# wolfecameron/GIST

Hardware: AMD Instinct MI355X
Metric: epochs/sec (higher is better)
Workload: dtype f32 (projection products from 3 bf16 pieces per operand = all 24 bits, 6 cross terms, fp32 accumulation)

## Files before the change

### gist_amd/_lib.py

```python
import ctypes
import os

_HERE = os.path.dirname(os.path.abspath(__file__))
LIB_PATH = os.environ.get('GIST_LIB_PATH') or os.path.join(_HERE, 'libgist_hip.so')

ABI_VERSION = 16


class GistLibraryError(RuntimeError):
    pass


class GistError(RuntimeError):
    """A gist_* entry point returned a negative code."""


_p = ctypes.c_void_p
_i64 = ctypes.c_int64
_i32 = ctypes.c_int32
_int = ctypes.c_int
_f = ctypes.c_float
_u64 = ctypes.c_uint64

SIGNATURES = {
    'gist_last_error': (ctypes.c_char_p, []),
    'gist_abi_version': (_int, []),
    'gist_device_count': (_int, []),
    'gist_in_degree_norm_f32': (_int, [_p, _i64, _p, _p]),
    'gist_spmm_csr_f32': (_int, [_p, _p, _p, _i64, _p, _i64, _i64, _i64, _p, _p, _int, _p]),
    'gist_partition_last_stats': (_int, [_p, _i32]),
    'gist_partition_graph': (_int, [_p, _p, _p, _p, _i64, _i32, _u64, _i32, _f, _p]),
    'gist_spmm_csr_blocked_f32': (_int, [_p, _p, _p, _i64, _p, _i64, _i64, _i64, _p, _p, _int, _p, _i64, _p]),
    'gist_spmm_blocks_bytes': (_i64, [_i64]),
    'gist_spmm_blocks_prepare': (_int, [_p, _p, _i64, _p, _i64, _p, _i64, _p]),
    'gist_spmm_csr_prepared_f32': (_int, [_p, _p, _p, _i64, _p, _i64, _i64, _i64, _p, _p, _int, _p, _i64, _p, _p]),
    'gist_gemm_workspace_bytes': (_i64, [_i64, _i64, _i64]),
    'gist_gemm_set_mode': (_int, [_int]),
    'gist_gemm_get_mode': (_int, []),
    'gist_tuning_set': (_int, [_int, ctypes.c_double]),
    'gist_tuning_get': (ctypes.c_double, [_int]),
    'gist_launch_count': (ctypes.c_uint64, []),
    'gist_empty_launches': (_int, [ctypes.c_int32, ctypes.c_int32, ctypes.c_int32, _p]),
    'gist_gemm_nt_f32': (_int, [_p, _i64, _p, _i64, _p, _p, _i64, _i64, _i64, _i64, _p, _i64, _p]),
    'gist_gemm_nn_f32': (_int, [_p, _i64, _p, _i64, _p, _i64, _i64, _i64, _i64, _p, _i64, _p]),
    'gist_gemm_tn_f32': (_int, [_p, _i64, _p, _i64, _p, _i64, _i64, _i64, _i64, _p, _i64, _p]),
    'gist_ln_relu_fwd_f32': (_int, [_p, _i64, _p, _i64, _p, _i64, _i64, _int, _int, _f, _p]),
    'gist_ln_relu_bwd_f32': (_int, [_p, _i64, _p, _i64, _p, _p, _i64, _i64, _i64, _int, _int, _p]),
    'gist_gemm_nn_dropout_f32': (_int, [_p, _i64, _p, _i64, _p, _i64, _i64, _i64, _i64, _f, _u64, _u64, _p, _i64, _p]),
    'gist_dropout_f32': (_int, [_p, _i64, _i64, _i64, _f, _u64, _u64, _p]),
    'gist_colsum_partials': (_i64, [_i64]),
    'gist_colsum_f32': (_int, [_p, _i64, _i64, _i64, _p, _p, _p]),
    'gist_softmax_xent_f32': (_int, [_p, _i64, _p, _p, _i64, _p, _p, _p, _i64, _i64, _i64, _p]),
    'gist_adam_f32': (_int, [_p, _p, _p, _p, _i64, _f, _f, _f, _f, _f, _i64, _p]),
    'gist_argmax_correct_i32': (_int, [_p, _i64, _p, _p, _p, _i64, _i64, _p]),
    'gist_induced_mark': (_int, [_p, _i64, _p, _p]),
    'gist_induced_unmark': (_int, [_p, _i64, _p, _p]),
    'gist_fill_i32': (_int, [_p, _i64, _i32, _p]),
    'gist_copy_i32': (_int, [_p, _p, _i64, _p]),
    'gist_publish_i64': (_int, [_p, _i64, _p, _p]),
    'gist_induced_rowptr': (_int, [_p, _p, _p, _i64, _p, _p, _p]),
    'gist_induced_fill': (_int, [_p, _p, _p, _i64, _p, _p, _p, _i64, _p]),
    'gist_extract_batch': (_int, [_p, _p, _p, _p, _p, _i64, _p, _p, _p, _p, _p, _i64, _p, _p, _i64, _i64, _p, _i64, _p, _p, _p]),
    'gist_gather_rows_f32': (_int, [_p, _i64, _p, _i64, _i64, _p, _i64, _p]),
    'gist_gather_i32': (_int, [_p, _p, _i64, _p, _p]),
    'gist_block_gather_f32': (_int, [_p, _i64, _p, _p, _i64, _i64, _p, _i64, _p]),
    'gist_block_scatter_f32': (_int, [_p, _i64, _p, _p, _i64, _i64, _p, _i64, _p]),
    'gist_mean_rows_f32': (_int, [_p, _i64, _i64, _i64, _p, _p]),
    'gist_standard_scaler_workspace_bytes': (_i64, [_i64, _i64]),
    'gist_standard_scaler_f32': (_int, [_p, _i64, _i64, _i64, _p, _i64, _p, _p, _p, _i64, _p]),
    'gist_timer_create': (_p, [_i64]),
    'gist_timer_destroy': (None, [_p]),
    'gist_timer_reset': (None, [_p]),
    'gist_timer_count': (_i64, [_p]),
    'gist_timer_read': (_int, [_p, _i64, _p, _p, _p, _p, _p]),
    'gist_step_h3_workspace_bytes': (_i64, [_p]),
    'gist_step_h3_workspace_bytes_mode': (_i64, [_p, _int]),
    'gist_step_fused_workspace_bytes': (_i64, [_p]),
    'gist_step_col_partials_floats': (_i64, [_p]),
    'gist_step_fused_slab_bytes': (_i64, [_p, _i32]),
    'gist_spmm_csr_drop_f32': (_int, [_p, _p, _p, _i64, _p, _i64, _i64, _i64, _p, _p, _int, _p, _i64, _int, _f,
                                      _u64, _u64, _u64, _i64, _p]),
    'gist_spmm_csr_drop_prepared_f32': (_int, [_p, _p, _p, _i64, _p, _i64, _i64, _i64, _p, _p, _int, _p, _i64, _int, _f,
                                               _u64, _u64, _u64, _i64, _p, _p]),
    'gist_spmm_csr_drop_lnbwd_f32': (_int, [_p, _p, _p, _i64, _p, _i64, _i64, _i64, _p, _p, _i64, _f, _u64, _u64, _u64, _i64,
                                            _p, _i64, _p, _p, _i64, _p, _i64, _int, _p]),
    'gist_spmm_lnb_units': (_i64, [_i64]),
    'gist_spmm_block_image_bytes': (_i64, []),
    'gist_spmm_pair_min_edges': (ctypes.c_int32, []),
    'gist_spmm_block_units_f32': (_int, [_p, _i64, _p, _p, _i64, _p, _i64, _i64, _i64, _p, _int, _p]),
    'gist_spmm_block_chains_f32': (_int, [_p, _i64, _p, _p, _p, _i64, _p, _i64, _i64, _i64, _p, _int, _p]),
    'gist_spmm_prepared_useful': (_int, [_i64, _i64, _i64, _p, _p]),
    'gist_spmm_drop_takes': (_int, [_int, _i64, _i64, _i64, _p, _p, _int]),
    'gist_gemm_dual_takes': (_int, [_i64, _i64, _i64, _i64, _i64, _i64, _i64, _p, _p, _p, _p]),
    'gist_gemm_nn_tn_dual_f32': (_int, [_p, _i64, _p, _i64, _p, _i64, _p, _i64, _p, _i64, _i64, _i64, _i64, _p, _i64, _p, _p]),
    'gist_gemm_slabs_f32': (_int, [_int, _p, _i64, _p, _i64, _p, _p, _i64, _i64, _i64, _i64, _p, _i64, _p, _p]),
    'gist_ln_relu_fwd_drop_f32': (_int, [_p, _i64, _p, _i64, _p, _i64, _p, _i64, _i64, _int, _int, _f, _f, _u64,
                                         _u64, _i64, _p]),
    'gist_ln_relu_fwd_slabs_f32': (_int, [_p, _i64, _p, _i64, _int, _p, _p, _i64, _p, _i64, _p, _i64, _i64, _int, _int,
                                          _f, _f, _u64, _u64, _i64, _p]),
    'gist_gemm_splits_operands': (_int, [_i64, _i64, _i64]),
    'gist_row_chunks16': (_i64, [_i64]),
    'gist_ln_relu_bwd_colsum_f32': (_int, [_p, _i64, _p, _i64, _p, _p, _i64, _i64, _i64, _int, _int, _p, _p]),
    'gist_colsum_chunks_f32': (_int, [_p, _i64, _i64, _p, _p]),
    'gist_class_layer_takes': (_int, [_i64, _i64, _i64, _i64, _i64, _p, _p]),
    'gist_class_layer_f32': (_int, [_p, _i64, _p, _i64, _p, _p, _i64, _p, _i64, _p, _i64, _p, _p, _i64, _f, _u64, _u64,
                                    _p, _i64, _i64, _i64, _p]),
    'gist_class_dw_slab_bytes': (_i64, [_i64, _i64, _i64]),
    'gist_class_dw_slabs_f32': (_int, [_p, _i64, _p, _i64, _p, _i64, _p, _i64, _i64, _i64, _p]),
    'gist_ln_relu_bwd_colsum_class_dw_f32': (_int, [_p, _i64, _p, _i64, _p, _p, _i64, _i64, _i64, _int, _int, _p,
                                                    _p, _i64, _p, _i64, _p, _i64, _p, _i64, _i64, _i64, _p]),
    'gist_gemm_nn_dropout_colsum_f32': (_int, [_p, _i64, _p, _i64, _p, _i64, _i64, _i64, _i64, _f, _u64, _u64,
                                               _p, _i64, _p, _p]),
    'gist_softmax_xent_slabs_f32': (_int, [_p, _i64, _p, _i64, _i64, _p, _p, _p, _i64, _p, _p, _p, _i64, _i64,
                                           _i64, _p]),
    'gist_adam_segments_f32': (_int, [_p, _p, _p, _p, _i64, _f, _f, _f, _f, _f, _i64, _p, _i64, _p, _i64, _i64,
                                      _p, _p]),
    'gist_grad_segments_finish_f32': (_int, [_p, _i64, _p, _i64, _p]),
    'gist_extract_batch_drop': (_int, [_p, _p, _p, _p, _p, _i64, _p, _p, _p, _p, _p, _i64, _p, _p, _i64, _i64, _p,
                                       _i64, _p, _p, _p, _i64, _f, _u64, _u64, _i64, _p]),
    'gist_extract_parts_scratch_bytes': (_i64, [_i64]),
    'gist_extract_parts_supported': (_int, [_i64]),
    'gist_extract_parts_batch': (_int, [_p, _p, _p, _p, _p, _i64, _i64, _p, _p, _i32, _p, _p, _p, _p, _i64,
                                        _p, _p, _i64, _i64, _p, _i64, _p, _p, _p, _i64, _f, _u64, _u64, _i64, _p,
                                        _p]),
    'gist_sage_step': (_int, [_p, _p, _i64, _u64, _f, _f, _f, _f, _f, _i64, _int, _p]),
    'gist_sage_step_extracts_next': (_int, [_p, _i64, _int]),
    'gist_extract_parts_desc_batch': (_int, [_p, _p]),
    'gist_adam_segments_extract_f32': (_int, [_p, _p, _p, _p, _i64, _f, _f, _f, _f, _f, _i64, _p, _i64, _p, _i64, _i64,
                                              _p, _p, _p]),
    'gist_gat_scores_f32': (_int, [_p, _i64, _p, _i64, _i64, _i64, _p, _p, _p]),
    'gist_gat_aggregate_f32': (_int, [_p, _p, _p, _i64, _p, _p, _i64, _i64, _i64, _int, _p, _i64, _p, _p, _p]),
    'gist_gat_backward_dst_f32': (_int, [_p, _p, _p, _i64, _p, _i64, _p, _i64, _p, _p, _p, _p, _i64, _i64, _i64, _int,
                                         _p, _i64, _p, _p, _p]),
    'gist_gat_backward_src_f32': (_int, [_p, _p, _p, _i64, _p, _i64, _p, _p, _p, _p, _p, _p, _p, _i64, _i64, _i64,
                                         _p, _i64, _p, _p]),
    'gist_gat_attn_grad_workspace_floats': (_i64, [_i64, _i64, _i64]),
    'gist_gat_attn_grad_f32': (_int, [_p, _i64, _p, _p, _i64, _i64, _i64, _p, _i64, _p, _p]),
}

GIST_MAX_LAYERS = 16
TUNE = {'h3_min_gflop': 0, 'h3_min_tiles': 1, 'h3_tm': 2, 'gemm_tile': 3, 'gemm_splits': 4,
        'spmm_chunk': 5, 'spmm_split': 6, 'spmm_kernel': 7, 'b3c': 8, 'class_fused': 9, 'gemm_dual': 10, 'host_threads': 11, 'lnb_fused': 12, 'b3c_splits': 13, 'b3_tail': 14,
        'b3_wide': 15}
GIST_STEP_EXTRACT = 1
GIST_STEP_TRAIN = 2
GIST_STEP_EXTRACT_NEXT = 4
GIST_STEP_PREEXTRACTED = 8
GIST_STEP_PHASE_FORWARD = 16
GIST_STEP_PHASE_BACKWARD = 32
GIST_STEP_PHASE_OPTIMIZER = 64
GIST_STEP_DLOGITS_GIVEN = 128


class LayerDesc(ctypes.Structure):
    _fields_ = [('n_in', _i64), ('n_out', _i64), ('W', _p), ('b', _p), ('dW', _p), ('db', _p),
                ('Z', _p), ('ldz', _i64), ('Y', _p), ('ldy', _i64), ('rstd', _p)]


class StepPlan(ctypes.Structure):
    _fields_ = [('n_layers', _i32), ('use_layernorm', _i32), ('p_drop', _f), ('seed', _u64),
                ('layer', LayerDesc * GIST_MAX_LAYERS),
                ('dlogits', _p), ('ldc', _i64), ('dZ', _p), ('partials', _p),
                ('row_loss', _p), ('loss', _p), ('workspace', _p), ('workspace_bytes', _i64),
                ('workspace2', _p), ('workspace2_bytes', _i64),
                ('params', _p), ('grads', _p), ('exp_avg', _p), ('exp_avg_sq', _p),
                ('n_params', _i64),
                ('g_rowptr', _p), ('g_col', _p), ('g_t_rowptr', _p), ('g_t_col', _p),
                ('feat', _p), ('ld_feat', _i64), ('labels_all', _p), ('remap', _p),
                ('rowptr', _p), ('col', _p), ('t_rowptr', _p), ('t_col', _p),
                ('col_capacity', _i64), ('norm', _p), ('labels', _p), ('timer', _p),
                ('n_max', _i64), ('feat_absmax', _f), ('h3_workspace', _p),
                ('h3_workspace_bytes', _i64), ('row_blocks', _p), ('n_row_blocks', _i64),
                ('spmm_prepared', _p), ('spmm_prepared_bytes', _i64),
                ('fuse', _i32), ('hsrc', _p * GIST_MAX_LAYERS), ('ld_hsrc', _i64 * GIST_MAX_LAYERS),
                ('col_partials', _p), ('fused_workspace', _p), ('fused_workspace_bytes', _i64),
                ('node_part', _p), ('part_slot', _p),
                ('batch_index', _i32), ('extract_scratch', _p),
                ('next_ids', _p), ('next_n', _i64), ('next_batch_index', _i32), ('next_drop_offset', _u64),
                ('feat_intra', _p), ('ld_feat_intra', _i64), ('sibling_parts', ctypes.c_int32)]


class ExtractPartsDesc(ctypes.Structure):
    _fields_ = [('g_rowptr', _p), ('g_col', _p), ('g_t_rowptr', _p), ('g_t_col', _p),
                ('ids', _p), ('n', _i64), ('n_max', _i64),
                ('node_part', _p), ('part_slot', _p), ('batch', _i32),
                ('rowptr', _p), ('col', _p), ('t_rowptr', _p), ('t_col', _p), ('col_capacity', _i64), ('norm', _p),
                ('feat', _p), ('ld_feat', _i64), ('n_feat', _i64), ('z0', _p), ('ldz0', _i64),
                ('labels_all', _p), ('labels', _p),
                ('x0', _p), ('ldx0', _i64), ('p', _f), ('seed', _u64), ('offset', _u64), ('mask_ld', _i64),
                ('scratch', _p), ('feat_intra', _p), ('ld_intra', _i64), ('ah', _p)]


class GradSegment(ctypes.Structure):
    _fields_ = [('begin', _i64), ('end', _i64), ('src', _p), ('stride', _i64), ('n_src', _i32)]


_lib = None


def load():
    global _lib
    if _lib is not None:
        return _lib
    if not os.path.exists(LIB_PATH):
        raise GistLibraryError(
            'gist_amd: %s is missing. Build it with `python gist_amd/build.py` '
            '(hipcc --offload-arch=gfx950). There is no CPU fallback.' % LIB_PATH)
    import torch
    try:
        lib = ctypes.CDLL(LIB_PATH)
    except OSError as e:
        raise GistLibraryError('gist_amd: cannot load %s: %s' % (LIB_PATH, e))
    for name, (res, args) in SIGNATURES.items():
        try:
            fn = getattr(lib, name)
        except AttributeError:
            raise GistLibraryError('gist_amd: %s does not export %s (stale build?)'
                                   % (LIB_PATH, name))
        fn.restype = res
        fn.argtypes = args
    if lib.gist_abi_version() != ABI_VERSION:
        raise GistLibraryError('gist_amd: ABI version mismatch: library %d, binding %d'
                               % (lib.gist_abi_version(), ABI_VERSION))
    _lib = lib
    return lib


def check(rc, name):
    if rc != 0:
        msg = load().gist_last_error()
        raise GistError('%s failed (%d): %s' % (name, rc, msg.decode() if msg else ''))
```

### gist_amd/csrc/adam_body.h

```cpp
#pragma once
#include "common.h"

namespace gist {

constexpr int kAdamMaxSegs = 2 * GIST_MAX_LAYERS;
struct AdamSegs {
    int n;
    int n_src[kAdamMaxSegs];
    int ded_first[kAdamMaxSegs];
    int n_ded;
    int fin_first[kAdamMaxSegs];
    int n_fin;
    int64_t begin[kAdamMaxSegs], end[kAdamMaxSegs], stride[kAdamMaxSegs];
    const float *src[kAdamMaxSegs];
};
struct AdamArgs {
    float *p, *g, *m, *v;
    int64_t n;
    float beta1, beta2, eps, wd, step_size, inv_bc2_sqrt;
    AdamSegs segs;
    const float *row_nll; int n_loss_rows; float inv_count; float *loss;
};
__host__ __device__ inline int64_t adam_arena_blocks(int64_t n) { return (n + 1023) / 1024; }

__device__ __forceinline__ float adam_wave_sum(float v) {
#pragma unroll
    for (int off = 32; off > 0; off >>= 1) v += __shfl_xor(v, off);
    return v;
}

__device__ __forceinline__ void loss_reduce_256(const float *__restrict__ row_nll, int n_rows,
                                                float inv_count, float *__restrict__ loss, float *red) {
    float s = 0.f;
    if (threadIdx.x < 256)
        for (int i = threadIdx.x; i < n_rows; i += 256) s += row_nll[i];
    s = adam_wave_sum(s);
    if (threadIdx.x < 256 && (threadIdx.x & 63) == 0) red[threadIdx.x >> 6] = s;
    __syncthreads();
    if (threadIdx.x == 0) loss[0] = (((red[0] + red[1]) + red[2]) + red[3]) * inv_count;
}

__device__ __forceinline__ float chunk_partial4(const float *__restrict__ src, int64_t stride, int n_src, int q) {
    float acc = 0.f;
    int k = q;
    for (; k + 28 < n_src; k += 32) {
        float t[8];
#pragma unroll
        for (int u = 0; u < 8; ++u) t[u] = src[(int64_t)(k + 4 * u) * stride];
#pragma unroll
        for (int u = 0; u < 8; ++u) acc += t[u];
    }
    for (; k < n_src; k += 4) acc += src[(int64_t)k * stride];
    return acc;
}

__device__ __forceinline__ void adam_update(float *__restrict__ p, float *__restrict__ m, float *__restrict__ v,
                                            int64_t i, float gv, float beta1, float beta2, float eps, float wd,
                                            float step_size, float inv_bc2_sqrt) {
    const float pv = p[i];
    if (wd != 0.f) gv = fmaf(wd, pv, gv);
    const float mv = m[i] + (1.f - beta1) * (gv - m[i]);
    const float vv = beta2 * v[i] + (1.f - beta2) * gv * gv;
    m[i] = mv;
    v[i] = vv;
    const float denom = sqrtf(vv) * inv_bc2_sqrt + eps;
    p[i] = pv - step_size * (mv / denom);
}

template <bool kUpdate = true>
__device__ __forceinline__ void adam_virtual_block(const AdamArgs &A, int64_t vb, int vt, int only_seg = -1) {
    const AdamSegs &segs = A.segs;
    const int64_t n_chunks = adam_arena_blocks(A.n);
    if (vb >= n_chunks) {
        const int idx = (int)(vb - n_chunks);
        if (idx >= segs.n_ded) return;
        int sg = -1;
        for (int s = 0; s < segs.n; ++s)
            if (segs.ded_first[s] >= 0 && segs.ded_first[s] <= idx &&
                (sg < 0 || segs.ded_first[s] > segs.ded_first[sg]))
                sg = s;
        if (sg < 0) return;
        const int lane = vt & 63, w = vt >> 6;
        const int e = 16 * w + (lane & 15), q = lane >> 4;
        const int64_t i = segs.begin[sg] + (int64_t)(idx - segs.ded_first[sg]) * 64 + e;
        const bool live = i < segs.end[sg];
        float acc = 0.f;
        if (live) acc = chunk_partial4(segs.src[sg] + (i - segs.begin[sg]), segs.stride[sg], segs.n_src[sg], q);
        const float a1 = __shfl(acc, (lane & 15) + 16), a2 = __shfl(acc, (lane & 15) + 32), a3 = __shfl(acc, (lane & 15) + 48);
        if (q == 0 && live) {
            const float gv = ((acc + a1) + a2) + a3;
            A.g[i] = gv;
            if (kUpdate) adam_update(A.p, A.m, A.v, i, gv, A.beta1, A.beta2, A.eps, A.wd, A.step_size, A.inv_bc2_sqrt);
        }
        return;
    }
    const int64_t lo = vb * 1024;
    const int64_t hi = lo + 1024 < A.n ? lo + 1024 : A.n;
    unsigned touch = 0;
    for (int s = 0; s < segs.n; ++s)
        if (segs.begin[s] < hi && segs.end[s] > lo && (only_seg < 0 || s == only_seg)) touch |= 1u << s;
#pragma unroll
    for (int u = 0; u < 4; ++u) {
        const int64_t i = lo + vt + 256 * u;
        if (i >= hi) break;
        float gv;
        int sg = -1;
        for (unsigned t = touch; t; t &= t - 1) {
            const int s = __builtin_ctz(t);
            if (i >= segs.begin[s] && i < segs.end[s]) sg = s;
        }
        if (sg >= 0) {
            if (segs.ded_first[sg] >= 0) continue;
            const float *src = segs.src[sg] + (i - segs.begin[sg]);
            const int64_t stride = segs.stride[sg];
            const int ns = segs.n_src[sg];
            float acc = 0.f;
            int k = 0;
            for (; k + 4 <= ns; k += 4) {
                const float t0 = src[(int64_t)k * stride], t1 = src[(int64_t)(k + 1) * stride];
                const float t2 = src[(int64_t)(k + 2) * stride], t3 = src[(int64_t)(k + 3) * stride];
                acc += t0; acc += t1; acc += t2; acc += t3;
            }
            for (; k < ns; ++k) acc += src[(int64_t)k * stride];
            gv = acc;
            A.g[i] = acc;
        } else {
            if (!kUpdate) continue;
            gv = A.g[i];
        }
        if (kUpdate) adam_update(A.p, A.m, A.v, i, gv, A.beta1, A.beta2, A.eps, A.wd, A.step_size, A.inv_bc2_sqrt);
    }
}

int adam_segments_args(const char *name, float *param, float *grad, float *exp_avg, float *exp_avg_sq, int64_t n, float lr,
                       float beta1, float beta2, float eps, float weight_decay, int64_t step,
                       const gist_grad_segment *segments, int64_t n_segments, const float *row_loss,
                       int64_t n_loss_rows, int64_t loss_count, float *loss, AdamArgs *out);

}
```

### gist_amd/csrc/common.h

```cpp
#pragma once
#include <hip/hip_runtime.h>
#include <stdint.h>
#include <stdio.h>
#include <stdlib.h>

#include <atomic>

#include "../../include/gist_hip.h"

namespace gist {

constexpr int kWave = 64;

void set_error(const char *fmt, ...);

static inline hipStream_t as_stream(gist_stream_t s) { return reinterpret_cast<hipStream_t>(s); }

extern std::atomic<uint64_t> g_launches;

static inline int launch_status(const char *what) {
    g_launches.fetch_add(1, std::memory_order_relaxed);
    hipError_t e = hipGetLastError();
    if (e != hipSuccess) {
        set_error("%s: %s", what, hipGetErrorString(e));
        return GIST_ELAUNCH;
    }
    return GIST_OK;
}

#define GIST_REQUIRE(cond, ...)            \
    do {                                   \
        if (!(cond)) {                     \
            gist::set_error(__VA_ARGS__);  \
            return GIST_EINVAL;            \
        }                                  \
    } while (0)

extern thread_local gist_timer *tl_timer;
int64_t timer_begin(gist_timer *t, int kind, int64_t m, int64_t n, int64_t k, hipStream_t s);
void timer_end(gist_timer *t, int64_t slot, hipStream_t s);

__device__ __forceinline__ uint64_t splitmix64(uint64_t z) {
    z = (z ^ (z >> 30)) * 0xBF58476D1CE4E5B9ULL;
    z = (z ^ (z >> 27)) * 0x94D049BB133111EBULL;
    return z ^ (z >> 31);
}

int64_t h3_kpad(int64_t k);
bool h3_eligible(int64_t m, int64_t n, int64_t k);
bool h3_eligible_kept(int64_t m, int64_t n, int64_t k);
struct H3Dual {
    const float *src; int64_t ld; int64_t rows, cols;
    float p; uint64_t seed, offset;
    int fixed_shift;
    const unsigned *amax;
    const float *rowmax, *colmax;
    uint32_t *dst_r; float *inv_r;
    uint32_t *dst_t; float *inv_t;
};
int h3_dual_split(const H3Dual &d, hipStream_t st);
int h3_split_rows(const float *src, int64_t ld, int64_t rows, int64_t k, uint32_t *dst, float *inv,
                  hipStream_t st);
int h3_absmax(const float *src, int64_t ld, int64_t rows, int64_t cols, unsigned *out, hipStream_t st);
int h3_gemm_presplit(const char *name, const uint32_t *sa, const float *inv_a, const uint32_t *sb,
                     const float *inv_b, const float *bias, float *c, int64_t ldc, int64_t m,
                     int64_t n, int64_t k, hipStream_t st);

int h3_mode();
int64_t b3_kpad(int64_t k);
bool b3_eligible(int64_t m, int64_t n, int64_t k);
bool b3_eligible_kept(int64_t m, int64_t n, int64_t k);
struct B3Dual {
    const float *src; int64_t ld; int64_t rows, cols;
    float p; uint64_t seed, offset;
    uint16_t *dst_r;
    uint16_t *dst_t;
    float *col_partials;
    bool vec4;
};
int b3_dual_split(const B3Dual &d, hipStream_t st);
int64_t b3_slab_bytes(int64_t m, int64_t n, int64_t k);
int b3_gemm_presplit(const char *name, const uint16_t *sa, const uint16_t *sb, const float *bias, float *c,
                     int64_t ldc, int64_t m, int64_t n, int64_t k, float *slabs, int64_t slab_bytes,
                     hipStream_t st, int *deferred = nullptr);
int gemm_slabs(int layout, const float *a, int64_t lda, const float *b, int64_t ldb, const float *bias, float *c,
               int64_t ldc, int64_t m, int64_t n, int64_t k, void *slabs, int64_t slab_bytes, int *n_slabs,
               hipStream_t st);
int64_t gemm_f32_slab_bytes(int64_t m, int64_t n, int64_t k, bool tn = false);
bool gemm_dual_takes(int64_t m, int64_t n1, int64_t k1, int64_t lddy, int64_t ldw, int64_t ldz, int64_t lddz,
                     const float *dy, const float *w, const float *z, const float *dz);
int gemm_dual_nn_tn(const char *name, const float *dy, int64_t lddy, const float *w, int64_t ldw, float *dz,
                    int64_t lddz, const float *z, int64_t ldz, float *dw, int64_t lddw, int64_t m, int64_t n1,
                    int64_t k1, void *slabs, int64_t slab_bytes, int *n_slabs, hipStream_t st);
int splitk_reduce(const char *name, const float *slabs, int64_t slab, int splits, const float *bias, float *c,
                  int64_t ldc, int64_t m, int64_t n, hipStream_t st);

struct SpmmDrop {
    int mode;
    float p, scale;
    uint64_t sm, y_base, src_base;
    int64_t ld;
};
struct SpmmLnBwd {
    const float *yhat; int64_t ldy;
    const float *rstd;
    float *dy; int64_t lddy;
    float *col_partials;
    int relu;
};
int spmm_drop(const int32_t *rowptr, const int32_t *col, const float *x, int64_t ldx, float *y, int64_t ldy,
              int64_t n_rows, int64_t d, const float *out_scale, const float *src_scale, int accumulate,
              const int32_t *row_blocks, int64_t n_row_blocks, const SpmmDrop &dr, hipStream_t st,
              const void *prepared = nullptr, bool pairs = true, const SpmmLnBwd *ln = nullptr);
int spmm_prepared(const int32_t *rowptr, const int32_t *col, const float *x, int64_t ldx, float *y, int64_t ldy,
                  int64_t n_rows, int64_t d, const float *out_scale, const float *src_scale, int accumulate,
                  const int32_t *row_blocks, int64_t n_row_blocks, const void *prepared, hipStream_t st, bool pairs);
bool spmm_lnb_takes(int64_t d, int64_t ldx, int64_t ldy, const float *x, const float *y, const int32_t *row_blocks,
                    const void *prepared);
int64_t spmm_lnb_units(int64_t n_row_blocks);
bool spmm_drop_takes(int mode, int64_t d, int64_t ldx, int64_t ldy, const float *x, const float *y,
                     const int32_t *row_blocks);
#ifdef __HIPCC__
template <int CTRL>
__device__ __forceinline__ float dpp_move(float v) {
    return __builtin_bit_cast(float, __builtin_amdgcn_update_dpp(0, __builtin_bit_cast(int, v), CTRL, 0xf, 0xf, true));
}
__device__ __forceinline__ float wave_sum(float v) {
    v += dpp_move<0xB1>(v);
    v += dpp_move<0x4E>(v);
    v += dpp_move<0x141>(v);
    v += dpp_move<0x140>(v);
    const float r0 = __builtin_bit_cast(float, __builtin_amdgcn_readlane(__builtin_bit_cast(int, v), 0));
    const float r1 = __builtin_bit_cast(float, __builtin_amdgcn_readlane(__builtin_bit_cast(int, v), 16));
    const float r2 = __builtin_bit_cast(float, __builtin_amdgcn_readlane(__builtin_bit_cast(int, v), 32));
    const float r3 = __builtin_bit_cast(float, __builtin_amdgcn_readlane(__builtin_bit_cast(int, v), 48));
    return (r0 + r1) + (r2 + r3);
}
__device__ __forceinline__ float drop_keep(uint64_t idx, uint64_t sm, float p, float scale) {
    const uint64_t h = splitmix64((idx >> 1) + sm);
    const uint32_t w = (idx & 1) ? (uint32_t)(h >> 32) : (uint32_t)h;
    return ((float)(w >> 8) * (1.0f / 16777216.0f) >= p) ? scale : 0.f;
}
template <int VEC>
__device__ __forceinline__ void drop_vec(float (&v)[VEC], uint64_t idx0, const SpmmDrop &dr) {
#pragma unroll
    for (int k = 0; k < VEC; ++k) v[k] *= drop_keep(idx0 + k, dr.sm, dr.p, dr.scale);
}
__device__ __forceinline__ void drop_f4(float4 &v, uint64_t idx0, const SpmmDrop &dr) {
    const float inv = 1.0f / 16777216.0f;
    if ((idx0 & 1) == 0) {
        const uint64_t pair = idx0 >> 1;
        const uint64_t h0 = splitmix64(pair + dr.sm), h1 = splitmix64(pair + 1 + dr.sm);
        v.x *= ((float)((uint32_t)h0 >> 8) * inv >= dr.p) ? dr.scale : 0.f;
        v.y *= ((float)((uint32_t)(h0 >> 32) >> 8) * inv >= dr.p) ? dr.scale : 0.f;
        v.z *= ((float)((uint32_t)h1 >> 8) * inv >= dr.p) ? dr.scale : 0.f;
        v.w *= ((float)((uint32_t)(h1 >> 32) >> 8) * inv >= dr.p) ? dr.scale : 0.f;
    } else {
        v.x *= drop_keep(idx0, dr.sm, dr.p, dr.scale); v.y *= drop_keep(idx0 + 1, dr.sm, dr.p, dr.scale);
        v.z *= drop_keep(idx0 + 2, dr.sm, dr.p, dr.scale); v.w *= drop_keep(idx0 + 3, dr.sm, dr.p, dr.scale);
    }
}

#endif
int launch_spmm_mfma(const int32_t *rowptr, const int32_t *col, const float *x, int64_t ldx, float *y,
                     int64_t ldy, int64_t n_rows, int64_t d, const float *out_scale, const float *src_scale,
                     int accumulate, const int32_t *row_blocks, int64_t n_row_blocks, const void *prepared,
                     hipStream_t st, const SpmmDrop *dr = nullptr, bool pairs = true);
int64_t spmm_blocks_bytes(int64_t n_blocks);
bool spmm_dense32_takes(int64_t d, int64_t ldx, int64_t ldy);
int launch_spmm_dense32(const int32_t *rowptr, const int32_t *col, const float *x, int64_t ldx, float *y,
                        int64_t ldy, int64_t n_rows, int64_t d, const float *out_scale, const float *src_scale,
                        int accumulate, const int32_t *row_blocks, int64_t n_row_blocks, const void *prepared,
                        hipStream_t st, const SpmmDrop *dr = nullptr);
bool spmm_prepared_takes(int64_t d, int64_t ldx, int64_t ldy, const float *x, const float *y);
int launch_spmm_blocks_prepare(const int32_t *rowptr, const int32_t *col, const int32_t *rowptr2,
                               const int32_t *col2, int64_t n_rows, const int32_t *row_blocks,
                               int64_t n_row_blocks, void *prepared, void *prepared2, hipStream_t st, bool pairs = true);

int ln_relu_bwd_ex(const float *d_out, int64_t ldg, const float *yhat, int64_t ldy, const float *rstd,
                   float *dy, int64_t lddy, int64_t n_rows, int64_t d, int use_lynorm, int relu,
                   float *rowmax, hipStream_t st);
int colsum_ex(const float *g, int64_t ldg, int64_t n_rows, int64_t d, float *partials, float *out,
              float *pmax, float *outmax, hipStream_t st);
int colsum_finish(const float *partials, int64_t chunks, int64_t d, float *out, hipStream_t st);
int ln_relu_bwd_colsum(const float *d_out, int64_t ldg, const float *yhat, int64_t ldy, const float *rstd,
                       float *dy, int64_t lddy, int64_t n_rows, int64_t d, int use_lynorm, int relu,
                       float *col_partials, hipStream_t st);
struct ClassDwArgs;
int ln_relu_bwd_colsum_class_dw(const float *d_out, int64_t ldg, const float *yhat, int64_t ldy, const float *rstd,
                                float *dy, int64_t lddy, int64_t n_rows, int64_t d, int use_lynorm, int relu,
                                float *col_partials, const ClassDwArgs &dw, hipStream_t st);
int gemm_nn_dropout_ex(const char *name, const float *g, int64_t ldg, const float *w, int64_t ldw, float *z,
                       int64_t ldz, int64_t m, int64_t n, int64_t k, float p, uint64_t seed, uint64_t offset,
                       void *workspace, int64_t workspace_bytes, float *dy_col_partials, hipStream_t st);
int softmax_xent_ex(const char *name, float *logits, int64_t ldl, const float *slabs, int64_t slab_stride,
                    int n_slabs, const float *bias, const int32_t *labels, const uint8_t *mask, int64_t count,
                    float *row_loss, float *loss, float *d_logits, int64_t ldg, int64_t n_rows,
                    int64_t n_classes, hipStream_t st);
int colsum_rows16(const float *g, int64_t ldg, int64_t n_rows, int64_t d, float *partials, bool interleaved,
// ... 24 lines not shown
```

### gist_amd/csrc/gemm_b3.hip

```cpp
#include <stdlib.h>
#include <string.h>

#include <type_traits>

#include "common.h"

namespace gist {

typedef __bf16 bf16x8 __attribute__((ext_vector_type(8)));
typedef float b3_f32x4 __attribute__((ext_vector_type(4)));

constexpr int B3_TM = 256, B3_TN = 128, B3_BK = 32;
constexpr int B3_THREADS = 512;
constexpr int B3_STAGES = 2;
constexpr int B3_SKEW = 16;
constexpr int B3_KT_BYTES = B3_BK * 6;
constexpr int B3_A_BYTES = B3_TM * B3_KT_BYTES;
constexpr int B3_B_BYTES = B3_TN * B3_KT_BYTES;
constexpr int B3_BUF_BYTES = B3_A_BYTES + B3_B_BYTES;

__device__ __forceinline__ uint32_t b3_pack(__bf16 lo, __bf16 hi) {
    return (uint32_t)__builtin_bit_cast(unsigned short, lo) |
           ((uint32_t)__builtin_bit_cast(unsigned short, hi) << 16);
}

__device__ __forceinline__ void b3_emit(const float (&v)[8], uint16_t *__restrict__ dst) {
    uint32_t w[3][4];
#pragma unroll
    for (int j = 0; j < 4; ++j) {
        __bf16 p[2][3];
#pragma unroll
        for (int h = 0; h < 2; ++h) {
            const float x = v[2 * j + h];
            p[h][0] = (__bf16)x;
            const float r1 = x - (float)p[h][0];
            p[h][1] = (__bf16)r1;
            const float r2 = r1 - (float)p[h][1];
            p[h][2] = (__bf16)r2;
        }
#pragma unroll
        for (int q = 0; q < 3; ++q) w[q][j] = b3_pack(p[0][q], p[1][q]);
    }
#pragma unroll
    for (int q = 0; q < 3; ++q)
        *reinterpret_cast<uint4 *>(dst + 8 * q) = make_uint4(w[q][0], w[q][1], w[q][2], w[q][3]);
}

__global__ __launch_bounds__(256) void b3_dual_split_kernel(B3Dual d, int64_t ldd_r, int64_t ldd_t,
                                                            float keep) {
    __shared__ float tile[64][65];
    const int c0 = blockIdx.x * 64, r0 = blockIdx.y * 64;
    const int t = threadIdx.x;
    const int c4 = (t & 15) * 4;
    const uint64_t sm = d.seed * 0x9E3779B97F4A7C15ULL;
    const float inv24 = 1.0f / 16777216.0f;
#pragma unroll
    for (int i = 0; i < 4; ++i) {
        const int rr = (t >> 4) + 16 * i;
        const int64_t r = r0 + rr;
        float v[4] = {0.f, 0.f, 0.f, 0.f};
        if (r < d.rows) {
            const float *p = d.src + r * d.ld + c0 + c4;
            if (c0 + c4 + 3 < d.cols && d.vec4) {
                const float4 q = *reinterpret_cast<const float4 *>(p);
                v[0] = q.x; v[1] = q.y; v[2] = q.z; v[3] = q.w;
            } else {
#pragma unroll
                for (int j = 0; j < 4; ++j)
                    if (c0 + c4 + j < d.cols) v[j] = p[j];
            }
            if (d.p > 0.f) {
                const uint64_t idx0 = d.offset + (uint64_t)r * (uint64_t)d.cols + (uint64_t)(c0 + c4);
#pragma unroll
                for (int j = 0; j < 4; ++j) {
                    const uint64_t idx = idx0 + j;
                    const uint64_t h = splitmix64((idx >> 1) + sm);
                    const uint32_t w = (idx & 1) ? (uint32_t)(h >> 32) : (uint32_t)h;
                    v[j] *= ((float)(w >> 8) * inv24 >= d.p) ? keep : 0.f;
                }
            }
        }
        tile[rr][c4 + 0] = v[0]; tile[rr][c4 + 1] = v[1];
        tile[rr][c4 + 2] = v[2]; tile[rr][c4 + 3] = v[3];
    }
    __syncthreads();
    if (d.col_partials != nullptr && t < 64 && c0 + t < d.cols && r0 < d.rows) {
        float s0 = 0.f, s1 = 0.f, s2 = 0.f, s3 = 0.f;
#pragma unroll
        for (int r = 0; r < 64; r += 4) {
            s0 += tile[r][t]; s1 += tile[r + 1][t]; s2 += tile[r + 2][t]; s3 += tile[r + 3][t];
        }
        d.col_partials[(int64_t)blockIdx.y * d.cols + c0 + t] = (s0 + s1) + (s2 + s3);
    }
    const int kb = t & 7;
#pragma unroll
    for (int i = 0; i < 2; ++i) {
        const int q = (t >> 3) + 32 * i;
        if (d.dst_r != nullptr && r0 + q < d.rows && c0 + kb * 8 < ldd_r) {
            float v[8];
#pragma unroll
            for (int j = 0; j < 8; ++j) v[j] = tile[q][kb * 8 + j];
            b3_emit(v, d.dst_r + ((int64_t)(r0 + q) * ldd_r + c0 + kb * 8) * 3);
        }
        if (d.dst_t != nullptr && c0 + q < d.cols && r0 + kb * 8 < ldd_t) {
            float v[8];
#pragma unroll
            for (int j = 0; j < 8; ++j) v[j] = tile[kb * 8 + j][q];
            b3_emit(v, d.dst_t + ((int64_t)(c0 + q) * ldd_t + r0 + kb * 8) * 3);
        }
    }
}

struct B3Args {
    const uint16_t *a; int64_t lda;
    const uint16_t *b; int64_t ldb;
    const float *bias;
    float *c; int64_t ldc;
    int m, n, kpad;
    int tiles_m, tiles_n;
    int kt_per_split;
    int64_t split_stride;
    int dp_tiles, tail_splits, tail_kt;
    float *tail_partials;
};

template <int NI>
__device__ __forceinline__ void b3_dma_offsets(int64_t ld, int rows, int row0, int first, int lane,
                                                uint32_t (&off)[NI]) {
#pragma unroll
    for (int jj = 0; jj < NI; ++jj) {
        const int inst = first + jj;
        const int slot = (inst % 3) * 64 + lane;
        const int rs = slot / 12;
        const int chunk = (slot % 12) ^ ((rs >> 3) << 1);
        const int r = (inst / 3) * 16 + rs;
        const int dr = min(r, rows - 1 - row0);
        off[jj] = (uint32_t)((int64_t)dr * ld * 6 + chunk * 16);
    }
}

__device__ __forceinline__ void b3_mfma(b3_f32x4 &acc, const bf16x8 &a, const bf16x8 &b) {
    asm volatile("v_mfma_f32_16x16x32_bf16 %0, %1, %2, %0" : "+v"(acc) : "v"(a), "v"(b));
}

template <int NI>
__device__ __forceinline__ void b3_dma_image(const char *base, const uint32_t (&off)[NI], char *image,
                                             int first) {
    __amdgpu_buffer_rsrc_t rsrc = __builtin_amdgcn_make_buffer_rsrc(
        const_cast<char *>(base), 0, 0x7fffffff, 0x00020000);
#pragma unroll
    for (int jj = 0; jj < NI; ++jj)
        __builtin_amdgcn_raw_ptr_buffer_load_lds(
            rsrc, (__attribute__((address_space(3))) void *)(image + (first + jj) * 1024), 16, off[jj],
            0, 0, 0);
}

__global__ __launch_bounds__(B3_THREADS, 2) void gemm_b3_kernel(B3Args g) {
    extern __shared__ __attribute__((aligned(16))) char b3_smem[];
    constexpr int NI = 4, NJ = 4;
    const int nwg = g.dp_tiles;
    const int orig = blockIdx.x;
    const bool tail = orig >= nwg;
    const int tail_tile = tail ? (orig - nwg) / g.tail_splits : 0;
    const int tail_slice = tail ? (orig - nwg) % g.tail_splits : 0;
    const int qd = nwg / kXcds, rm = nwg % kXcds, xcd = orig % kXcds;
    const int L = tail ? nwg + tail_tile
                       : (xcd < rm ? xcd * (qd + 1) : rm * (qd + 1) + (xcd - rm) * qd) + orig / kXcds;
    constexpr int GM = 8;
    const int width = GM * g.tiles_n;
    const int group = L / width;
    const int first_m = group * GM;
    const int gsz = min(g.tiles_m - first_m, GM);
    const int bm = first_m + (L % width) % gsz;
    const int bn = (L % width) / gsz;
    const int row0 = bm * B3_TM, col0 = bn * B3_TN;
    const int kt0 = tail ? tail_slice * g.tail_kt : (int)blockIdx.y * g.kt_per_split;
    const int n_kt = min(g.kpad / B3_BK - kt0, tail ? g.tail_kt : g.kt_per_split);

    const int lane = threadIdx.x & 63;
    const int wave = __builtin_amdgcn_readfirstlane(threadIdx.x >> 6);
    const int wm = wave >> 1, wn = wave & 1;
    const int rr = lane & 15, kg = lane >> 4;

    b3_f32x4 acc[NI][NJ];
#pragma unroll
    for (int i = 0; i < NI; ++i)
#pragma unroll
        for (int j = 0; j < NJ; ++j)
#pragma unroll
            for (int e = 0; e < 4; ++e) acc[i][j][e] = 0.f;

    constexpr int NWAVES = B3_THREADS / 64;
    constexpr int DA = B3_TM / 16 * 3 / NWAVES, DB = B3_TN / 16 * 3 / NWAVES;
    uint32_t offA[DA], offB[DB];
    b3_dma_offsets<DA>(g.lda, g.m, row0, DA * wave, lane, offA);
    b3_dma_offsets<DB>(g.ldb, g.n, col0, DB * wave, lane, offB);
    const char *originA = reinterpret_cast<const char *>(g.a) + (int64_t)row0 * g.lda * 6 + (int64_t)kt0 * B3_KT_BYTES;
    const char *originB = reinterpret_cast<const char *>(g.b) + (int64_t)col0 * g.ldb * 6 + (int64_t)kt0 * B3_KT_BYTES;
    auto dma = [&](int buf, int kt) {
        char *sa = b3_smem + buf * B3_BUF_BYTES;
        b3_dma_image<DA>(originA + (int64_t)kt * B3_KT_BYTES, offA, sa, DA * wave);
        b3_dma_image<DB>(originB + (int64_t)kt * B3_KT_BYTES, offB, sa + B3_A_BYTES, DB * wave);
    };

    const char *fa[B3_STAGES][3], *fb[B3_STAGES][3];
#pragma unroll
    for (int p = 0; p < 3; ++p) {
        const int c = 3 * kg + p;
        const int in_slab = (rr * 12 + (c ^ ((rr >> 3) << 1))) * 16;
#pragma unroll
        for (int st = 0; st < B3_STAGES; ++st) {
            fa[st][p] = b3_smem + st * B3_BUF_BYTES + wm * NI * 3072 + in_slab;
            fb[st][p] = b3_smem + st * B3_BUF_BYTES + B3_A_BYTES + wn * NJ * 3072 + in_slab;
        }
    }

    const bool live = __builtin_amdgcn_readfirstlane(row0 + wm * (16 * NI) < g.m);
    bf16x8 a[NI][3], b[NJ][3];
    auto read_head = [&](auto st_c) {
        constexpr int st = decltype(st_c)::value;
        if (!live) return;
#pragma unroll
        for (int j = 0; j < NJ; ++j) b[j][0] = *reinterpret_cast<const bf16x8 *>(fb[st][0] + j * 3072);
#pragma unroll
        for (int i = 0; i < NI; ++i) a[i][1] = *reinterpret_cast<const bf16x8 *>(fa[st][1] + i * 3072);
#pragma unroll
        for (int i = 0; i < NI; ++i) a[i][2] = *reinterpret_cast<const bf16x8 *>(fa[st][2] + i * 3072);
    };
    auto read_rest = [&](auto st_c) {
        constexpr int st = decltype(st_c)::value;
        if (!live) return;
#pragma unroll
        for (int j = 0; j < NJ; ++j) b[j][1] = *reinterpret_cast<const bf16x8 *>(fb[st][1] + j * 3072);
#pragma unroll
        for (int i = 0; i < NI; ++i) a[i][0] = *reinterpret_cast<const bf16x8 *>(fa[st][0] + i * 3072);
#pragma unroll
        for (int j = 0; j < NJ; ++j) b[j][2] = *reinterpret_cast<const bf16x8 *>(fb[st][2] + j * 3072);
    };
    constexpr int pa[6] = {1, 2, 1, 0, 0, 0};
    constexpr int pb[6] = {0, 0, 1, 0, 1, 2};
    constexpr int B3_MID = 4 * NI * NJ;

    dma(0, 0);
    __builtin_amdgcn_s_waitcnt(0x0f70);
    __syncthreads();
    dma(1, 1);
    read_head(std::integral_constant<int, 0>{});

    auto mfmas = [&](auto t0_c, auto t1_c) {
        constexpr int t0 = decltype(t0_c)::value, t1 = decltype(t1_c)::value;
        if (!live) return;
#pragma unroll
        for (int t = t0; t < t1; ++t) {
            const int term = t / (NI * NJ), i = (t % (NI * NJ)) / NJ, j = t % NJ;
            b3_mfma(acc[i][j], a[i][pa[term]], b[j][pb[term]]);
        }
    };
    const int last_kt = n_kt - 1;
    auto kstep = [&](auto cur_c, auto late_c, int kt) {
        constexpr int cur = decltype(cur_c)::value;
        constexpr int skew = decltype(late_c)::value * B3_SKEW;
        using I = std::integral_constant<int, 0>;
        __builtin_amdgcn_sched_barrier(0);
// ... 462 lines not shown
```

### gist_amd/csrc/rowops.hip

```cpp
#include <stdlib.h>

#include "common.h"
#include "class_dw_body.h"
#include "adam_body.h"

namespace gist {

template <int TPR>
__device__ __forceinline__ float row_sum(float v, float *red) {
    v = wave_sum(v);
    if constexpr (TPR == 64) {
        return v;
    } else {
        const int w = threadIdx.x >> 6;
        __syncthreads();
        if ((threadIdx.x & 63) == 0) red[w] = v;
        __syncthreads();
        return red[0] + red[1] + red[2] + red[3];
    }
}

__device__ __forceinline__ float keep_scale(uint64_t seed, uint64_t idx, float p, float scale) {
    const uint64_t h = splitmix64((idx >> 1) + seed * 0x9E3779B97F4A7C15ULL);
    const uint32_t w = (idx & 1) ? (uint32_t)(h >> 32) : (uint32_t)h;
// ... 553 lines not shown
            const uint64_t pair = (offset + (uint64_t)(r0 + r) * (uint64_t)n_cols + (uint64_t)c0) >> 1;
            const uint64_t h0 = splitmix64(pair + sm), h1 = splitmix64(pair + 1 + sm);
            v.x *= ((float)((uint32_t)h0 >> 8) * inv24 >= p) ? scale : 0.f;
            v.y *= ((float)((uint32_t)(h0 >> 32) >> 8) * inv24 >= p) ? scale : 0.f;
            v.z *= ((float)((uint32_t)h1 >> 8) * inv24 >= p) ? scale : 0.f;
            v.w *= ((float)((uint32_t)(h1 >> 32) >> 8) * inv24 >= p) ? scale : 0.f;
        }
        *reinterpret_cast<float4 *>(dz + (int64_t)(r0 + r) * lddz + c0) = v;
    }
}

constexpr int kColsumRows = 64;

template <bool WITH_MAX>
__global__ __launch_bounds__(256) void colsum_stage1_kernel(const float *__restrict__ g,
                                                            int64_t ldg, int n_rows, int d,
                                                            float *__restrict__ partials,
                                                            float *__restrict__ pmax) {
    __shared__ float red[3][64];
    __shared__ float redm[3][64];
    const int cl = threadIdx.x & 63, rl = threadIdx.x >> 6;
    const int c = blockIdx.x * 64 + cl;
    const int r0 = blockIdx.y * kColsumRows;
    const int r1 = min(n_rows, r0 + kColsumRows);
    float s0 = 0.f, s1 = 0.f, s2 = 0.f, s3 = 0.f, mx = 0.f;
    if (c < d) {
        const float *p = g + c;
        int r = r0 + rl;
        for (; r + 12 < r1; r += 16) {
            const float a0 = p[(int64_t)r * ldg], a1 = p[(int64_t)(r + 4) * ldg];
            const float a2 = p[(int64_t)(r + 8) * ldg], a3 = p[(int64_t)(r + 12) * ldg];
            s0 += a0; s1 += a1; s2 += a2; s3 += a3;
            if constexpr (WITH_MAX)
                mx = fmaxf(mx, fmaxf(fmaxf(fabsf(a0), fabsf(a1)), fmaxf(fabsf(a2), fabsf(a3))));
        }
        for (; r < r1; r += 4) {
            const float a0 = p[(int64_t)r * ldg];
            s0 += a0;
            if constexpr (WITH_MAX) mx = fmaxf(mx, fabsf(a0));
        }
    }
    const float s = (s0 + s1) + (s2 + s3);
    if (rl > 0) {
        red[rl - 1][cl] = s;
        if constexpr (WITH_MAX) redm[rl - 1][cl] = mx;
    }
    __syncthreads();
    if (rl == 0 && c < d) {
        partials[(int64_t)blockIdx.y * d + c] = ((s + red[0][cl]) + red[1][cl]) + red[2][cl];
        if constexpr (WITH_MAX)
            pmax[(int64_t)blockIdx.y * d + c] =
                fmaxf(fmaxf(mx, redm[0][cl]), fmaxf(redm[1][cl], redm[2][cl]));
    }
}

__global__ void colsum_stage2_kernel(const float *__restrict__ partials, int chunks, int d,
                                     float *__restrict__ out, const float *__restrict__ pmax,
                                     float *__restrict__ outmax) {
    const int c = blockIdx.x * blockDim.x + threadIdx.x;
    if (c >= d) return;
    if (outmax != nullptr) {
        float m0 = 0.f, m1 = 0.f, m2 = 0.f, m3 = 0.f;
        int k = 0;
        for (; k + 3 < chunks; k += 4) {
            m0 = fmaxf(m0, pmax[(int64_t)k * d + c]);
            m1 = fmaxf(m1, pmax[(int64_t)(k + 1) * d + c]);
            m2 = fmaxf(m2, pmax[(int64_t)(k + 2) * d + c]);
            m3 = fmaxf(m3, pmax[(int64_t)(k + 3) * d + c]);
        }
        for (; k < chunks; ++k) m0 = fmaxf(m0, pmax[(int64_t)k * d + c]);
        outmax[c] = fmaxf(fmaxf(m0, m1), fmaxf(m2, m3));
    }
    float s0 = 0.f, s1 = 0.f, s2 = 0.f, s3 = 0.f;
    int k = 0;
    for (; k + 3 < chunks; k += 4) {
        s0 += partials[(int64_t)k * d + c];
        s1 += partials[(int64_t)(k + 1) * d + c];
        s2 += partials[(int64_t)(k + 2) * d + c];
        s3 += partials[(int64_t)(k + 3) * d + c];
    }
    for (; k < chunks; ++k) s0 += partials[(int64_t)k * d + c];
    out[c] = (s0 + s1) + (s2 + s3);
}

__device__ __forceinline__ float wave_max(float v) {
#pragma unroll
    for (int off = 32; off > 0; off >>= 1) v = fmaxf(v, __shfl_xor(v, off));
    return v;
}

__global__ __launch_bounds__(256) void xent_grad_kernel(
    float *logits, int64_t ldl, const int32_t *__restrict__ labels,
    const uint8_t *__restrict__ mask, float inv_count, float *__restrict__ d_logits, int64_t ldg,
    float *__restrict__ row_nll, int n_rows, int n_classes, const float *__restrict__ slabs,
    int64_t slab_stride, int n_slabs, const float *__restrict__ bias) {
    const int row = blockIdx.x * 4 + (threadIdx.x >> 6);
    if (row >= n_rows) return;
    const int lane = threadIdx.x & 63;
    float *lr = logits + (int64_t)row * ldl;
    float *gr = d_logits + (int64_t)row * ldg;
    const bool on = mask ? mask[row] != 0 : true;
    if (slabs != nullptr) {
        for (int c = lane; c < n_classes; c += 64) {
            const int64_t i = (int64_t)row * n_classes + c;
            float sacc = 0.f;
            for (int k = 0; k < n_slabs; ++k) sacc += slabs[k * slab_stride + i];
            if (bias) sacc += bias[c];
            lr[c] = sacc;
        }
    }
    float mx = -INFINITY;
    for (int c = lane; c < n_classes; c += 64) mx = fmaxf(mx, lr[c]);
    mx = wave_max(mx);
    float se = 0.f;
    for (int c = lane; c < n_classes; c += 64) se += expf(lr[c] - mx);
    se = wave_sum(se);
    const int lab = labels[row];
    const float inv = 1.f / se;
    for (int c = lane; c < ldg; c += 64) {
        float gval = 0.f;
        if (on && c < n_classes) gval = (expf(lr[c] - mx) * inv - (c == lab ? 1.f : 0.f)) * inv_count;
        gr[c] = gval;
    }
    if (lane == 0) row_nll[row] = on ? -((lr[lab] - mx) - logf(se)) : 0.f;
}

__global__ __launch_bounds__(256) void xent_loss_kernel(const float *__restrict__ row_nll,
                                                        int n_rows, float inv_count,
                                                        float *__restrict__ loss) {
    __shared__ float red[4];
    loss_reduce_256(row_nll, n_rows, inv_count, loss, red);
}

__global__ void adam_kernel(float *__restrict__ p, const float *__restrict__ g,
                            float *__restrict__ m, float *__restrict__ v, int64_t n, float beta1,
                            float beta2, float eps, float wd, float step_size,
                            float inv_bc2_sqrt) {
    for (int64_t i = (int64_t)blockIdx.x * blockDim.x + threadIdx.x; i < n;
         i += (int64_t)gridDim.x * blockDim.x) {
        const float pv = p[i];
        float gv = g[i];
        if (wd != 0.f) gv = fmaf(wd, pv, gv);
        const float mv = m[i] + (1.f - beta1) * (gv - m[i]);
        const float vv = beta2 * v[i] + (1.f - beta2) * gv * gv;
        m[i] = mv;
        v[i] = vv;
        const float denom = sqrtf(vv) * inv_bc2_sqrt + eps;
        p[i] = pv - step_size * (mv / denom);
    }
}

__global__ __launch_bounds__(256) void adam_segments_kernel(AdamArgs A) {
    __shared__ float red[4];
    const int64_t n_blocks = adam_arena_blocks(A.n) + A.segs.n_ded;
    if ((int64_t)blockIdx.x >= n_blocks) {
        if (A.row_nll != nullptr) loss_reduce_256(A.row_nll, A.n_loss_rows, A.inv_count, A.loss, red);
        return;
    }
    adam_virtual_block(A, blockIdx.x, threadIdx.x);
}

__global__ __launch_bounds__(256) void grad_finish_kernel(AdamArgs A) {
    const int b = (int)blockIdx.x;
    if (b >= A.segs.n_fin) {
        adam_virtual_block<false>(A, adam_arena_blocks(A.n) + (b - A.segs.n_fin), threadIdx.x);
        return;
    }
    int sg = -1;
    for (int s = 0; s < A.segs.n; ++s)
        if (A.segs.fin_first[s] >= 0 && A.segs.fin_first[s] <= b && (sg < 0 || A.segs.fin_first[s] > A.segs.fin_first[sg]))
            sg = s;
    if (sg < 0) return;
    adam_virtual_block<false>(A, A.segs.begin[sg] / 1024 + (b - A.segs.fin_first[sg]), threadIdx.x, sg);
}

__global__ __launch_bounds__(256) void argmax_correct_kernel(
    const float *__restrict__ logits, int64_t ldl, const int32_t *__restrict__ labels,
    const uint8_t *__restrict__ mask, int32_t *__restrict__ correct, int n_rows, int n_classes) {
    const int row = blockIdx.x * 4 + (threadIdx.x >> 6);
    if (row >= n_rows) return;
    if (mask && !mask[row]) return;
    const int lane = threadIdx.x & 63;
    const float *lr = logits + (int64_t)row * ldl;
    float best = -INFINITY;
    int arg = 0x7fffffff;
    for (int c = lane; c < n_classes; c += 64) {
        const float v = lr[c];
        if (v > best) { best = v; arg = c; }
    }
#pragma unroll
    for (int off = 32; off > 0; off >>= 1) {
        const float ob = __shfl_xor(best, off);
        const int oa = __shfl_xor(arg, off);
        if (ob > best || (ob == best && oa < arg)) { best = ob; arg = oa; }
    }
    if (lane == 0 && arg == labels[row]) atomicAdd(correct, 1);
}

}

using namespace gist;

namespace gist {
static int ln_relu_fwd_ex(const char *name, float *y, int64_t ldy, float *out, int64_t ldo, float *rstd,
                          int64_t n_rows, int64_t d, int use_lynorm, int relu, float eps,
                          const DropOut *drop, hipStream_t st) {
    if (n_rows < 0 || d < 0) { set_error("%s: negative size", name); return GIST_EINVAL; }
    if (n_rows == 0 || d == 0) return GIST_OK;
    if (!y || !out) { set_error("%s: null pointer", name); return GIST_EINVAL; }
    if (ldy < d || ldo < d) { set_error("%s: leading dimension < d", name); return GIST_EINVAL; }
    if (n_rows >= (1LL << 31) || d >= (1LL << 31)) { set_error("%s: size >= 2^31", name); return GIST_EINVAL; }
    bool v4 = d % 4 == 0 && ldy % 4 == 0 && ldo % 4 == 0 && aligned16(y) && aligned16(out);
    DropOut dr{};
    const bool dropping = drop != nullptr && (drop->p > 0.f || drop->out2 != nullptr);
    if (drop != nullptr && drop->n_slabs > 0) {
        if (drop->slabs == nullptr || drop->slab_stride < n_rows * d) { set_error("%s: bad slabs", name); return GIST_EINVAL; }
        dr.slabs = drop->slabs; dr.slab_stride = drop->slab_stride; dr.n_slabs = drop->n_slabs; dr.bias = drop->bias;
        v4 = v4 && aligned16(drop->slabs) && drop->slab_stride % 4 == 0;
    }
    if (dropping) {
        const DropOut keep = dr;
        dr = *drop;
        dr.slabs = keep.slabs; dr.slab_stride = keep.slab_stride; dr.n_slabs = keep.n_slabs; dr.bias = keep.bias;
        if (dr.out2 != nullptr) {
            if (dr.ldo2 < d) { set_error("%s: leading dimension < d", name); return GIST_EINVAL; }
            v4 = v4 && dr.ldo2 % 4 == 0 && aligned16(dr.out2);
        }
    }
    const bool wide = d > 1024;
    const unsigned grid = (unsigned)(wide ? n_rows : ceil_div(n_rows, 4));
#define L(TPR, V)                                                                                   \
    do {                                                                                            \
        if (dropping)                                                                               \
            hipLaunchKernelGGL((ln_relu_fwd_kernel<TPR, V, true>), dim3(grid), dim3(256), 0, st, y, \
                               ldy, out, ldo, rstd, (int)n_rows, (int)d, use_lynorm, relu, eps, dr); \
        else                                                                                        \
            hipLaunchKernelGGL((ln_relu_fwd_kernel<TPR, V, false>), dim3(grid), dim3(256), 0, st, y, \
                               ldy, out, ldo, rstd, (int)n_rows, (int)d, use_lynorm, relu, eps, dr); \
    } while (0)
    if (wide) { if (v4) L(256, 4); else L(256, 1); }
    else { if (v4) L(64, 4); else L(64, 1); }
#undef L
    return launch_status(name);
}
}

extern "C" int gist_ln_relu_fwd_f32(float *y, int64_t ldy, float *out, int64_t ldo, float *rstd,
                                    int64_t n_rows, int64_t d, int use_lynorm, int relu,
                                    float eps, gist_stream_t stream) {
    return gist::ln_relu_fwd_ex("gist_ln_relu_fwd_f32", y, ldy, out, ldo, rstd, n_rows, d, use_lynorm, relu,
                                eps, nullptr, gist::as_stream(stream));
}

extern "C" int gist_ln_relu_fwd_drop_f32(float *y, int64_t ldy, float *out, int64_t ldo, float *out2,
                                         int64_t ldo2, float *rstd, int64_t n_rows, int64_t d,
                                         int use_lynorm, int relu, float eps, float p, uint64_t seed,
                                         uint64_t offset, int64_t mask_ld, gist_stream_t stream) {
    GIST_REQUIRE(p >= 0.f && p < 1.f, "gist_ln_relu_fwd_drop_f32: p must be in [0,1)");
    GIST_REQUIRE(mask_ld >= d || p == 0.f, "gist_ln_relu_fwd_drop_f32: mask_ld < d");
    gist::DropOut dr{};
    dr.out2 = out2; dr.ldo2 = ldo2; dr.p = p; dr.scale = p > 0.f ? 1.0f / (1.0f - p) : 1.f;
    dr.sm = seed * 0x9E3779B97F4A7C15ULL; dr.offset = offset; dr.mask_ld = mask_ld;
    return gist::ln_relu_fwd_ex("gist_ln_relu_fwd_drop_f32", y, ldy, out, ldo, rstd, n_rows, d, use_lynorm,
                                relu, eps, &dr, gist::as_stream(stream));
}

extern "C" int gist_ln_relu_fwd_slabs_f32(float *y, int64_t ldy, const float *slabs, int64_t slab_stride,
                                          int32_t n_slabs, const float *bias, float *out, int64_t ldo, float *out2,
                                          int64_t ldo2, float *rstd, int64_t n_rows, int64_t d, int use_lynorm,
                                          int relu, float eps, float p, uint64_t seed, uint64_t offset,
                                          int64_t mask_ld, gist_stream_t stream) {
    GIST_REQUIRE(p >= 0.f && p < 1.f, "gist_ln_relu_fwd_slabs_f32: p must be in [0,1)");
    GIST_REQUIRE(mask_ld >= d || p == 0.f, "gist_ln_relu_fwd_slabs_f32: mask_ld < d");
    GIST_REQUIRE(n_slabs >= 0 && n_slabs < 4096, "gist_ln_relu_fwd_slabs_f32: bad n_slabs");
    GIST_REQUIRE(n_slabs == 0 || slabs != nullptr, "gist_ln_relu_fwd_slabs_f32: null slabs");
    gist::DropOut dr{};
    dr.out2 = out2; dr.ldo2 = ldo2; dr.p = p; dr.scale = p > 0.f ? 1.0f / (1.0f - p) : 1.f;
    dr.sm = seed * 0x9E3779B97F4A7C15ULL; dr.offset = offset; dr.mask_ld = mask_ld;
    dr.slabs = slabs; dr.slab_stride = slab_stride; dr.n_slabs = n_slabs; dr.bias = n_slabs > 0 ? bias : nullptr;
    return gist::ln_relu_fwd_ex("gist_ln_relu_fwd_slabs_f32", y, ldy, out, ldo, rstd, n_rows, d, use_lynorm,
                                relu, eps, &dr, gist::as_stream(stream));
}

namespace gist {
int ln_relu_bwd_ex(const float *d_out, int64_t ldg, const float *yhat, int64_t ldy, const float *rstd,
                   float *dy, int64_t lddy, int64_t n_rows, int64_t d, int use_lynorm, int relu,
                   float *rowmax, hipStream_t st) {
    GIST_REQUIRE(n_rows >= 0 && d >= 0, "gist_ln_relu_bwd_f32: negative size");
    if (n_rows == 0 || d == 0) return GIST_OK;
    GIST_REQUIRE(d_out && yhat && dy, "gist_ln_relu_bwd_f32: null pointer");
    GIST_REQUIRE(!use_lynorm || rstd, "gist_ln_relu_bwd_f32: rstd is NULL with use_lynorm");
    GIST_REQUIRE(ldg >= d && ldy >= d && lddy >= d, "gist_ln_relu_bwd_f32: leading dimension < d");
    GIST_REQUIRE(n_rows < (1LL << 31) && d < (1LL << 31), "gist_ln_relu_bwd_f32: size >= 2^31");
    const bool v4 = d % 4 == 0 && ldg % 4 == 0 && ldy % 4 == 0 && lddy % 4 == 0 &&
                    aligned16(d_out) && aligned16(yhat) && aligned16(dy);
    const bool wide = d > 1024;
    const unsigned grid = (unsigned)(wide ? n_rows : ceil_div(n_rows, 4));
#define L(TPR, V)                                                                               \
    hipLaunchKernelGGL((ln_relu_bwd_kernel<TPR, V>), dim3(grid), dim3(256), 0, st, d_out, ldg,   \
                       yhat, ldy, rstd, dy, lddy, (int)n_rows, (int)d, use_lynorm, relu, rowmax)
    if (wide) { if (v4) L(256, 4); else L(256, 1); }
    else { if (v4) L(64, 4); else L(64, 1); }
#undef L
    return launch_status("gist_ln_relu_bwd_f32");
}
}

extern "C" int gist_ln_relu_bwd_f32(const float *d_out, int64_t ldg, const float *yhat,
                                    int64_t ldy, const float *rstd, float *dy, int64_t lddy,
                                    int64_t n_rows, int64_t d, int use_lynorm, int relu,
                                    gist_stream_t stream) {
    return gist::ln_relu_bwd_ex(d_out, ldg, yhat, ldy, rstd, dy, lddy, n_rows, d, use_lynorm, relu,
// ... 118 lines not shown
    GIST_REQUIRE(n_rows >= 0 && d >= 0, "gist_dropout_f32: negative size");
    GIST_REQUIRE(p >= 0.f && p < 1.f, "gist_dropout_f32: p must be in [0,1)");
    if (n_rows == 0 || d == 0 || p == 0.f) return GIST_OK;
    GIST_REQUIRE(z && ldz >= d, "gist_dropout_f32: bad buffer");
    const int64_t total = n_rows * d;
    if (d % 4 == 0 && ldz % 4 == 0 && aligned16(z) && (offset & 1) == 0) {
        const int64_t quads = total / 4;
        const unsigned grid = (unsigned)(ceil_div(quads, 256) < 16384 ? ceil_div(quads, 256) : 16384);
        hipLaunchKernelGGL(dropout_vec4_kernel, dim3(grid), dim3(256), 0, as_stream(stream), z, ldz,
                           n_rows, d, p, 1.0f / (1.0f - p), seed, offset);
        return launch_status("gist_dropout_f32");
    }
    const unsigned grid = (unsigned)(ceil_div(total, 256) < 8192 ? ceil_div(total, 256) : 8192);
    hipLaunchKernelGGL(dropout_kernel, dim3(grid), dim3(256), 0, as_stream(stream), z, ldz, n_rows,
                       d, p, 1.0f / (1.0f - p), seed, offset);
    return launch_status("gist_dropout_f32");
}

namespace gist {
int gemm_nn_dropout_ex(const char *name, const float *g, int64_t ldg, const float *w, int64_t ldw, float *z,
                       int64_t ldz, int64_t m, int64_t n, int64_t k, float p, uint64_t seed, uint64_t offset,
                       void *workspace, int64_t workspace_bytes, float *dy_col_partials, hipStream_t st) {
    if (!(p >= 0.f && p < 1.f)) { set_error("%s: p must be in [0,1)", name); return GIST_EINVAL; }
    if (m < 0 || n < 0 || k < 0) { set_error("%s: negative size", name); return GIST_EINVAL; }
    const bool narrow = k >= 1 && k <= 64 && m > 0 && n > 0 && g && w && z && n % 4 == 0 &&
                        ldw % 4 == 0 && ldz % 4 == 0 && aligned16(w) && aligned16(z) &&
                        (offset & 1) == 0 && ldg >= k && ldw >= n && ldz >= n &&
                        m < (1LL << 31) && n < (1LL << 31);
    if (!narrow) {
        int rc = gist_gemm_nn_f32(g, ldg, w, ldw, z, ldz, m, n, k, workspace, workspace_bytes, st);
        if (rc == GIST_OK && p != 0.f) rc = gist_dropout_f32(z, ldz, m, n, p, seed, offset, st);
        if (rc == GIST_OK && dy_col_partials != nullptr) rc = colsum_rows16(g, ldg, m, k, dy_col_partials, false, st);
        return rc;
    }
    hipLaunchKernelGGL(narrow_nn_drop_kernel, dim3((unsigned)ceil_div(n, 1024), (unsigned)ceil_div(m, 16)),
                       dim3(256), 0, st, g, ldg, w, ldw, z, ldz, (int)m, (int)n, (int)k, p,
                       p > 0.f ? 1.0f / (1.0f - p) : 1.0f, seed, offset, dy_col_partials);
    return launch_status(name);
}
}

extern "C" int gist_gemm_nn_dropout_f32(const float *g, int64_t ldg, const float *w, int64_t ldw,
                                        float *z, int64_t ldz, int64_t m, int64_t n, int64_t k,
                                        float p, uint64_t seed, uint64_t offset, void *workspace,
                                        int64_t workspace_bytes, gist_stream_t stream) {
    return gist::gemm_nn_dropout_ex("gist_gemm_nn_dropout_f32", g, ldg, w, ldw, z, ldz, m, n, k, p, seed,
                                    offset, workspace, workspace_bytes, nullptr, gist::as_stream(stream));
}

extern "C" int gist_gemm_nn_dropout_colsum_f32(const float *g, int64_t ldg, const float *w, int64_t ldw,
                                               float *z, int64_t ldz, int64_t m, int64_t n, int64_t k,
                                               float p, uint64_t seed, uint64_t offset, void *workspace,
                                               int64_t workspace_bytes, float *g_col_partials,
                                               gist_stream_t stream) {
    GIST_REQUIRE(g_col_partials != nullptr, "gist_gemm_nn_dropout_colsum_f32: null g_col_partials");
    return gist::gemm_nn_dropout_ex("gist_gemm_nn_dropout_colsum_f32", g, ldg, w, ldw, z, ldz, m, n, k, p,
                                    seed, offset, workspace, workspace_bytes, g_col_partials,
                                    gist::as_stream(stream));
}

extern "C" int64_t gist_colsum_partials(int64_t n_rows) {
    return n_rows <= 0 ? 0 : ceil_div(n_rows, kColsumRows);
}

namespace gist {
int colsum_ex(const float *g, int64_t ldg, int64_t n_rows, int64_t d, float *partials, float *out,
              float *pmax, float *outmax, hipStream_t st) {
    GIST_REQUIRE(n_rows >= 0 && d >= 0, "gist_colsum_f32: negative size");
    if (d == 0) return GIST_OK;
    GIST_REQUIRE(out, "gist_colsum_f32: null output");
    GIST_REQUIRE((pmax == nullptr) == (outmax == nullptr), "gist_colsum_f32: pmax/outmax mismatch");
    const int chunks = (int)gist_colsum_partials(n_rows);
    if (chunks > 0) {
        GIST_REQUIRE(g && partials && ldg >= d, "gist_colsum_f32: bad buffer");
        GIST_REQUIRE(chunks <= 65535, "gist_colsum_f32: too many rows");
        const dim3 grid((unsigned)ceil_div(d, 64), (unsigned)chunks);
        if (pmax)
            hipLaunchKernelGGL(colsum_stage1_kernel<true>, grid, dim3(256), 0, st, g, ldg,
                               (int)n_rows, (int)d, partials, pmax);
        else
            hipLaunchKernelGGL(colsum_stage1_kernel<false>, grid, dim3(256), 0, st, g, ldg,
                               (int)n_rows, (int)d, partials, pmax);
    }
    hipLaunchKernelGGL(colsum_stage2_kernel, dim3((unsigned)ceil_div(d, 64)), dim3(64), 0, st,
                       partials, chunks, (int)d, out, pmax, outmax);
    return launch_status("gist_colsum_f32");
}
}

namespace gist {
int colsum_finish(const float *partials, int64_t chunks, int64_t d, float *out, hipStream_t st) {
    if (d <= 0) return GIST_OK;
    hipLaunchKernelGGL(colsum_stage2_kernel, dim3((unsigned)ceil_div(d, 64)), dim3(64), 0, st, partials,
                       (int)chunks, (int)d, out, nullptr, nullptr);
    return launch_status("gist_colsum_f32");
}
}

extern "C" int gist_colsum_f32(const float *g, int64_t ldg, int64_t n_rows, int64_t d,
                               float *partials, float *out, gist_stream_t stream) {
    return gist::colsum_ex(g, ldg, n_rows, d, partials, out, nullptr, nullptr,
                           gist::as_stream(stream));
}

namespace gist {
int softmax_xent_ex(const char *name, float *logits, int64_t ldl, const float *slabs, int64_t slab_stride,
                    int n_slabs, const float *bias, const int32_t *labels, const uint8_t *mask, int64_t count,
                    float *row_loss, float *loss, float *d_logits, int64_t ldg, int64_t n_rows,
                    int64_t n_classes, hipStream_t st) {
    if (!(n_rows > 0 && n_classes > 0)) { set_error("%s: empty input", name); return GIST_EINVAL; }
    if (!(logits && labels && d_logits && row_loss)) { set_error("%s: null pointer", name); return GIST_EINVAL; }
    if (!(ldl >= n_classes && ldg >= n_classes)) { set_error("%s: leading dimension < n_classes", name); return GIST_EINVAL; }
    if (count <= 0) { set_error("%s: count must be > 0", name); return GIST_EINVAL; }
    if (!(n_rows < (1LL << 31) && ldg < (1LL << 31))) { set_error("%s: size >= 2^31", name); return GIST_EINVAL; }
    if (slabs != nullptr && n_slabs < 1) { set_error("%s: n_slabs < 1", name); return GIST_EINVAL; }
    const float inv = 1.0f / (float)count;
    hipLaunchKernelGGL(xent_grad_kernel, dim3((unsigned)ceil_div(n_rows, 4)), dim3(256), 0, st, logits, ldl,
                       labels, mask, inv, d_logits, ldg, row_loss, (int)n_rows, (int)n_classes, slabs,
                       slab_stride, n_slabs, bias);
    if (loss != nullptr)
        hipLaunchKernelGGL(xent_loss_kernel, dim3(1), dim3(256), 0, st, row_loss, (int)n_rows, inv, loss);
    return launch_status(name);
}
}

extern "C" int gist_softmax_xent_f32(const float *logits, int64_t ldl, const int32_t *labels,
                                     const uint8_t *mask, int64_t count, float *row_loss,
                                     float *loss, float *d_logits, int64_t ldg, int64_t n_rows,
                                     int64_t n_classes, gist_stream_t stream) {
    GIST_REQUIRE(loss != nullptr, "gist_softmax_xent_f32: null pointer");
    return gist::softmax_xent_ex("gist_softmax_xent_f32", const_cast<float *>(logits), ldl, nullptr, 0, 0,
                                 nullptr, labels, mask, count, row_loss, loss, d_logits, ldg, n_rows,
                                 n_classes, gist::as_stream(stream));
}

extern "C" int gist_softmax_xent_slabs_f32(float *logits, int64_t ldl, const float *slabs,
                                           int64_t slab_stride, int64_t n_slabs, const float *bias,
                                           const int32_t *labels, const uint8_t *mask, int64_t count,
                                           float *row_loss, float *loss, float *d_logits, int64_t ldg,
                                           int64_t n_rows, int64_t n_classes, gist_stream_t stream) {
    GIST_REQUIRE(n_slabs >= 0 && n_slabs < 4096, "gist_softmax_xent_slabs_f32: bad n_slabs");
    return gist::softmax_xent_ex("gist_softmax_xent_slabs_f32", logits, ldl, n_slabs > 0 ? slabs : nullptr,
                                 slab_stride, (int)n_slabs, bias, labels, mask, count, row_loss, loss,
                                 d_logits, ldg, n_rows, n_classes, gist::as_stream(stream));
}

extern "C" int gist_adam_f32(float *param, const float *grad, float *exp_avg, float *exp_avg_sq,
                             int64_t n, float lr, float beta1, float beta2, float eps,
                             float weight_decay, int64_t step, gist_stream_t stream) {
    GIST_REQUIRE(n >= 0, "gist_adam_f32: n < 0");
    if (n == 0) return GIST_OK;
    GIST_REQUIRE(param && grad && exp_avg && exp_avg_sq, "gist_adam_f32: null pointer");
    GIST_REQUIRE(step >= 1, "gist_adam_f32: step is 1-based");
    const double bc1 = 1.0 - pow((double)beta1, (double)step);
    const double bc2 = 1.0 - pow((double)beta2, (double)step);
    const float step_size = (float)((double)lr / bc1);
    const float inv_bc2_sqrt = (float)(1.0 / sqrt(bc2));
    const unsigned grid = (unsigned)(ceil_div(n, 256) < 16384 ? ceil_div(n, 256) : 16384);
    hipLaunchKernelGGL(adam_kernel, dim3(grid), dim3(256), 0, as_stream(stream), param, grad,
                       exp_avg, exp_avg_sq, n, beta1, beta2, eps, weight_decay, step_size,
                       inv_bc2_sqrt);
    return launch_status("gist_adam_f32");
}

namespace gist {
int adam_segments_args(const char *name, float *param, float *grad, float *exp_avg, float *exp_avg_sq, int64_t n, float lr,
                       float beta1, float beta2, float eps, float weight_decay, int64_t step,
                       const gist_grad_segment *segments, int64_t n_segments, const float *row_loss,
                       int64_t n_loss_rows, int64_t loss_count, float *loss, AdamArgs *out) {
    GIST_REQUIRE(n >= 0, "%s: n < 0", name);
    GIST_REQUIRE(n_segments >= 0 && n_segments <= kAdamMaxSegs, "%s: too many segments", name);
    GIST_REQUIRE(n_segments == 0 || segments != nullptr, "%s: null segments", name);
    GIST_REQUIRE(row_loss == nullptr || (loss != nullptr && loss_count > 0 && n_loss_rows >= 0 &&
                                         n_loss_rows < (1LL << 31)),
                 "%s: bad loss arguments", name);
    GIST_REQUIRE(n == 0 || (param && grad && exp_avg && exp_avg_sq), "%s: null pointer", name);
    GIST_REQUIRE(step >= 1, "%s: step is 1-based", name);
    AdamArgs A{};
    AdamSegs &sg = A.segs;
    for (int64_t i = 0; i < n_segments; ++i) {
        const gist_grad_segment &q = segments[i];
        if (q.src == nullptr || q.end <= q.begin) continue;
        GIST_REQUIRE(q.begin >= 0 && q.end <= n && q.n_src >= 1 && q.stride >= q.end - q.begin,
                     "%s: bad segment %d", name, (int)i);
        for (int j = 0; j < sg.n; ++j)
            GIST_REQUIRE(q.end <= sg.begin[j] || q.begin >= sg.end[j], "%s: overlapping segments", name);
        sg.begin[sg.n] = q.begin; sg.end[sg.n] = q.end; sg.stride[sg.n] = q.stride;
        sg.n_src[sg.n] = q.n_src; sg.src[sg.n] = q.src;
        sg.ded_first[sg.n] = -1;
        sg.fin_first[sg.n] = -1;
        if (q.n_src > 16 && q.end - q.begin <= 65536) {
            sg.ded_first[sg.n] = sg.n_ded;
            sg.n_ded += (int)ceil_div(q.end - q.begin, 64);
        } else {
            GIST_REQUIRE((q.end - 1) / 1024 - q.begin / 1024 + 1 + sg.n_fin < (1LL << 30), "%s: segment too large", name);
            sg.fin_first[sg.n] = sg.n_fin;
            sg.n_fin += (int)((q.end - 1) / 1024 - q.begin / 1024 + 1);
        }
        ++sg.n;
    }
    const double bc1 = 1.0 - pow((double)beta1, (double)step);
    const double bc2 = 1.0 - pow((double)beta2, (double)step);
    A.p = param; A.g = grad; A.m = exp_avg; A.v = exp_avg_sq; A.n = n;
    A.beta1 = beta1; A.beta2 = beta2; A.eps = eps; A.wd = weight_decay;
    A.step_size = (float)((double)lr / bc1);
    A.inv_bc2_sqrt = (float)(1.0 / sqrt(bc2));
    A.row_nll = row_loss; A.n_loss_rows = (int)n_loss_rows;
    A.inv_count = row_loss ? 1.0f / (float)loss_count : 0.f;
    A.loss = loss;
    GIST_REQUIRE(adam_arena_blocks(n) + sg.n_ded < (1LL << 31) - 2, "%s: arena too large", name);
    *out = A;
    return GIST_OK;
}
}

extern "C" int gist_adam_segments_f32(float *param, float *grad, float *exp_avg, float *exp_avg_sq,
                                      int64_t n, float lr, float beta1, float beta2, float eps,
                                      float weight_decay, int64_t step, const gist_grad_segment *segments,
                                      int64_t n_segments, const float *row_loss, int64_t n_loss_rows,
                                      int64_t loss_count, float *loss, gist_stream_t stream) {
    gist::AdamArgs A;
    const int rc = gist::adam_segments_args("gist_adam_segments_f32", param, grad, exp_avg, exp_avg_sq, n, lr, beta1, beta2,
                                            eps, weight_decay, step, segments, n_segments, row_loss, n_loss_rows,
                                            loss_count, loss, &A);
    if (rc != GIST_OK) return rc;
    if (n == 0 && row_loss == nullptr) return GIST_OK;
    const int64_t blocks = gist::adam_arena_blocks(n) + A.segs.n_ded + (row_loss ? 1 : 0);
    hipLaunchKernelGGL(gist::adam_segments_kernel, dim3((unsigned)blocks), dim3(256), 0, gist::as_stream(stream), A);
    return gist::launch_status("gist_adam_segments_f32");
}

extern "C" int gist_grad_segments_finish_f32(float *grad, int64_t n, const gist_grad_segment *segments,
                                             int64_t n_segments, gist_stream_t stream) {
    gist::AdamArgs A;
    const int rc = gist::adam_segments_args("gist_grad_segments_finish_f32", grad, grad, grad, grad, n, 0.f, 0.9f, 0.999f,
                                            1e-8f, 0.f, 1, segments, n_segments, nullptr, 0, 0, nullptr, &A);
    if (rc != GIST_OK) return rc;
    const int64_t blocks = (int64_t)A.segs.n_fin + A.segs.n_ded;
    if (blocks == 0) return GIST_OK;
    hipLaunchKernelGGL(gist::grad_finish_kernel, dim3((unsigned)blocks), dim3(256), 0, gist::as_stream(stream), A);
    return gist::launch_status("gist_grad_segments_finish_f32");
}

namespace gist {
int loss_finish(const float *row_loss, int64_t n_rows, int64_t count, float *loss, hipStream_t st) {
    hipLaunchKernelGGL(xent_loss_kernel, dim3(1), dim3(256), 0, st, row_loss, (int)n_rows, 1.0f / (float)count, loss);
    return launch_status("gist_sage_step");
}
}

extern "C" int gist_argmax_correct_i32(const float *logits, int64_t ldl, const int32_t *labels,
                                       const uint8_t *mask, int32_t *correct, int64_t n_rows,
                                       int64_t n_classes, gist_stream_t stream) {
    GIST_REQUIRE(n_rows >= 0 && n_classes > 0, "gist_argmax_correct_i32: bad size");
    if (n_rows == 0) return GIST_OK;
    GIST_REQUIRE(logits && labels && correct && ldl >= n_classes,
                 "gist_argmax_correct_i32: bad buffer");
    GIST_REQUIRE(n_rows < (1LL << 31), "gist_argmax_correct_i32: size >= 2^31");
    hipLaunchKernelGGL(argmax_correct_kernel, dim3((unsigned)ceil_div(n_rows, 4)), dim3(256), 0,
                       as_stream(stream), logits, ldl, labels, mask, correct, (int)n_rows,
                       (int)n_classes);
    return launch_status("gist_argmax_correct_i32");
}
```

### gist_amd/csrc/step.hip

```cpp
#include <math.h>

#include <new>

#include "common.h"
#include "class_dw_body.h"

using namespace gist;

#define GIST_TRY(expr)            \
    do {                          \
        int rc_ = (expr);         \
        if (rc_ != GIST_OK) return rc_; \
    } while (0)

static inline uint64_t round_up2(uint64_t x) { return x + (x & 1ULL); }

struct gist_timer {
    int64_t capacity, count;
    hipEvent_t *start, *stop;
    int32_t *kind;
    int64_t *m, *n, *k;
};

extern "C" gist_timer *gist_timer_create(int64_t capacity) {
    if (capacity <= 0) return nullptr;
    gist_timer *t = new (std::nothrow) gist_timer();
    if (!t) return nullptr;
    t->capacity = capacity;
    t->count = 0;
    t->start = new hipEvent_t[capacity];
    t->stop = new hipEvent_t[capacity];
    t->kind = new int32_t[capacity];
    t->m = new int64_t[capacity];
    t->n = new int64_t[capacity];
    t->k = new int64_t[capacity];
    for (int64_t i = 0; i < capacity; ++i) {
        if (hipEventCreate(&t->start[i]) != hipSuccess || hipEventCreate(&t->stop[i]) != hipSuccess) {
            set_error("gist_timer_create: hipEventCreate failed");
            t->capacity = i;
            break;
        }
    }
    return t;
}

extern "C" void gist_timer_destroy(gist_timer *t) {
    if (!t) return;
    for (int64_t i = 0; i < t->capacity; ++i) {
        (void)hipEventDestroy(t->start[i]);
        (void)hipEventDestroy(t->stop[i]);
    }
    delete[] t->start; delete[] t->stop; delete[] t->kind;
    delete[] t->m; delete[] t->n; delete[] t->k;
    delete t;
}

extern "C" void gist_timer_reset(gist_timer *t) { if (t) t->count = 0; }
extern "C" int64_t gist_timer_count(const gist_timer *t) { return t ? t->count : 0; }

extern "C" int gist_timer_read(gist_timer *t, int64_t i, float *ms, int32_t *kind, int64_t *m,
                               int64_t *n, int64_t *k) {
    GIST_REQUIRE(t && i >= 0 && i < t->count && ms, "gist_timer_read: bad index");
    hipError_t e = hipEventElapsedTime(ms, t->start[i], t->stop[i]);
    if (e != hipSuccess) { set_error("gist_timer_read: %s", hipGetErrorString(e)); return GIST_ELAUNCH; }
    if (kind) *kind = t->kind[i];
    if (m) *m = t->m[i];
    if (n) *n = t->n[i];
    if (k) *k = t->k[i];
    return GIST_OK;
}

namespace gist {
thread_local gist_timer *tl_timer = nullptr;

int64_t timer_begin(gist_timer *t, int kind, int64_t m, int64_t n, int64_t k, hipStream_t s) {
    if (!t || t->count >= t->capacity) return -1;
    const int64_t slot = t->count++;
    t->kind[slot] = kind; t->m[slot] = m; t->n[slot] = n; t->k[slot] = k;
    (void)hipEventRecord(t->start[slot], s);
    return slot;
}

void timer_end(gist_timer *t, int64_t slot, hipStream_t s) {
    if (t && slot >= 0) (void)hipEventRecord(t->stop[slot], s);
}
}

namespace {
struct Scope {
    gist_timer *t; int64_t slot; hipStream_t s;
    Scope(gist_timer *t_, int kind, int64_t m, int64_t n, int64_t k, hipStream_t s_)
        : t(t_), slot(timer_begin(t_, kind, m, n, k, s_)), s(s_) {}
    ~Scope() { timer_end(t, slot, s); }
};
struct ActiveTimer {
    explicit ActiveTimer(gist_timer *t) { tl_timer = t; }
    ~ActiveTimer() { tl_timer = nullptr; }
};
}

namespace {
struct H3Layer {
    bool on;
    int shift;
    uint32_t *Zs, *ZsT, *Ws, *WsT;
    float *inv_zr, *inv_zt, *inv_wr, *inv_wt;
};
struct H3Step {
    bool any;
    H3Layer layer[GIST_MAX_LAYERS];
    uint32_t *dYs, *dYsT;
    float *inv_dyr, *inv_dyt, *rowmax, *colmax, *pmax;
    unsigned *amax;
    int64_t bytes;
};

inline int bound_shift(double bound) {
    int e = 0;
    (void)frexp(bound, &e);
    const int s = 13 - e;
    return s < -60 ? -60 : (s > 60 ? 60 : s);
}

H3Step h3_layout(const gist_step_plan *p, char *base, int mode) {
    H3Step h{};
    const int L1 = p->n_layers;
    const int64_t n = p->n_max;
    if (mode != 1 || n <= 0) return h;
    int64_t off = 0;
    auto take = [&](int64_t bytes) {
        char *q = base ? base + off : nullptr;
        off += ceil_div(bytes, 256) * 256;
        return q;
    };
    int64_t max_out = 0;
    const double keep = p->p_drop > 0.f ? 1.0 / (1.0 - (double)p->p_drop) : 1.0;
    for (int k = 0; k < L1; ++k) {
        const gist_layer_desc &l = p->layer[k];
        const int64_t i2 = 2 * l.n_in, o = l.n_out;
        H3Layer &hl = h.layer[k];
        const double bound = k == 0 ? (double)p->feat_absmax * keep
                                    : (p->use_layernorm ? sqrt((double)(l.n_in > 1 ? l.n_in - 1 : 1)) * keep : 0.0);
        hl.on = k < L1 - 1 && bound > 0.0 && h3_eligible_kept(n, o, i2) && h3_eligible_kept(o, i2, n) &&
                (k == 0 || h3_eligible_kept(n, i2, o)) && l.ldz % 4 == 0 && l.ldy % 4 == 0 &&
                aligned16(l.W) && aligned16(l.Z) && aligned16(l.Y) && aligned16(l.dW);
        if (!hl.on) continue;
        h.any = true;
        hl.shift = bound_shift(bound);
        hl.Zs = reinterpret_cast<uint32_t *>(take(n * h3_kpad(i2) * 4));
        hl.ZsT = reinterpret_cast<uint32_t *>(take(i2 * h3_kpad(n) * 4));
        hl.Ws = reinterpret_cast<uint32_t *>(take(o * h3_kpad(i2) * 4));
        hl.WsT = k > 0 ? reinterpret_cast<uint32_t *>(take(i2 * h3_kpad(o) * 4)) : nullptr;
        hl.inv_zr = reinterpret_cast<float *>(take(n * 4));
        hl.inv_zt = reinterpret_cast<float *>(take(i2 * 4));
        hl.inv_wr = reinterpret_cast<float *>(take(o * 4));
        hl.inv_wt = k > 0 ? reinterpret_cast<float *>(take(i2 * 4)) : nullptr;
        max_out = o > max_out ? o : max_out;
    }
    if (!h.any) return h;
    h.dYs = reinterpret_cast<uint32_t *>(take(n * h3_kpad(max_out) * 4));
    h.dYsT = reinterpret_cast<uint32_t *>(take(max_out * h3_kpad(n) * 4));
    h.inv_dyr = reinterpret_cast<float *>(take(n * 4));
    h.inv_dyt = reinterpret_cast<float *>(take(max_out * 4));
    h.rowmax = reinterpret_cast<float *>(take(n * 4));
    h.colmax = reinterpret_cast<float *>(take(max_out * 4));
    h.pmax = reinterpret_cast<float *>(take(gist_colsum_partials(n) * max_out * 4));
    h.amax = reinterpret_cast<unsigned *>(take(GIST_MAX_LAYERS * 4));
    h.bytes = off;
    return h;
}

struct B3Layer {
    bool on;
    uint16_t *Zs, *ZsT, *Ws, *WsT;
};
struct B3Step {
    bool any;
    B3Layer layer[GIST_MAX_LAYERS];
    uint16_t *dYs, *dYsT;
    float *slabs; int64_t slab_bytes;
    int64_t bytes;
};

B3Step b3_layout(const gist_step_plan *p, char *base, int mode) {
    B3Step h{};
    const int L1 = p->n_layers;
    const int64_t n = p->n_max;
    if (mode != 2 || n <= 0) return h;
    int64_t off = 0;
    auto take = [&](int64_t bytes) {
        char *q = base ? base + off : nullptr;
        off += ceil_div(bytes, 256) * 256;
        return reinterpret_cast<uint16_t *>(q);
    };
    int64_t max_out = 0;
    for (int k = 0; k < L1; ++k) {
        const gist_layer_desc &l = p->layer[k];
        const int64_t i2 = 2 * l.n_in, o = l.n_out;
        B3Layer &hl = h.layer[k];
        hl.on = b3_eligible_kept(n, o, i2) && b3_eligible_kept(o, i2, n) &&
                (k == 0 || b3_eligible_kept(n, i2, o)) &&
                l.ldy < (1LL << 21) && i2 < (1LL << 21);
        if (!hl.on) continue;
        h.any = true;
        hl.Zs = take(n * b3_kpad(i2) * 6);
        hl.ZsT = take(i2 * b3_kpad(n) * 6);
        hl.Ws = take(o * b3_kpad(i2) * 6);
        hl.WsT = k > 0 ? take(i2 * b3_kpad(o) * 6) : nullptr;
        max_out = o > max_out ? o : max_out;
        int64_t sb = 0;
        for (int64_t rows = n; rows > 0; rows = (rows - 1) / 64 * 64) {
            const int64_t need[3] = {b3_slab_bytes(rows, o, i2), b3_slab_bytes(o, i2, rows),
                                     k > 0 ? b3_slab_bytes(rows, i2, o) : 0};
            for (int q = 0; q < 3; ++q) sb = need[q] > sb ? need[q] : sb;
        }
        if (sb > h.slab_bytes) h.slab_bytes = sb;
    }
    if (!h.any) return h;
    h.dYs = take(n * b3_kpad(max_out) * 6);
    h.dYsT = take(max_out * b3_kpad(n) * 6);
    h.slabs = h.slab_bytes > 0 ? reinterpret_cast<float *>(take(h.slab_bytes)) : nullptr;
    h.bytes = off;
    return h;
}
}

namespace {
constexpr int64_t kLnbMaxUnits = 256;
struct FusedLayout {
    float *dw_slabs[GIST_MAX_LAYERS]; int64_t dw_bytes[GIST_MAX_LAYERS];
    float *logit_slabs; int64_t logit_bytes;
    float *y_slabs; int64_t y_bytes;
    float *partials[GIST_MAX_LAYERS];
    int64_t partial_rows[GIST_MAX_LAYERS];
    int64_t bytes, partial_floats;
};

int64_t slab_need(int64_t m, int64_t n, int64_t k_max, bool k_is_rows) {
    struct Memo { int64_t m, n, k; int rows, mode; int64_t need; };
    static thread_local Memo memo[32];
    static thread_local int memo_n = 0;
    const int mode = gist_gemm_get_mode();
    const bool tuned = tune(GIST_TUNE_GEMM_TILE) != 0.0 || tune(GIST_TUNE_GEMM_SPLITS) != 0.0 || tune(GIST_TUNE_B3C) != 0.0 ||
                       tune(GIST_TUNE_B3C_SPLITS) != 0.0;
    for (int i = 0; i < memo_n && !tuned; ++i)
        if (memo[i].m == m && memo[i].n == n && memo[i].k == k_max && memo[i].rows == (int)k_is_rows && memo[i].mode == mode)
            return memo[i].need;
    int64_t need = 0;
    for (int64_t rows = k_max; rows > 0 && rows >= k_max / 2; rows -= 32) {
        const int64_t b = k_is_rows ? gemm_f32_slab_bytes(m, n, rows, true) : gemm_f32_slab_bytes(rows, n, m);
        need = b > need ? b : need;
    }
    if (!tuned) {
        static thread_local int memo_next = 0;
        if (memo_n < 32) memo[memo_n++] = Memo{m, n, k_max, (int)k_is_rows, mode, need};
        else { memo[memo_next] = Memo{m, n, k_max, (int)k_is_rows, mode, need}; memo_next = (memo_next + 1) % 32; }
    }
    return need;
}

FusedLayout fused_layout(const gist_step_plan *p, char *base, float *partials) {
    FusedLayout f{};
    const int L1 = p->n_layers;
    int64_t off = 0, poff = 0;
    auto take = [&](int64_t bytes) {
        char *q = base ? base + off : nullptr;
        off += ceil_div(bytes, 256) * 256;
        return reinterpret_cast<float *>(q);
    };
    const int64_t chunks = gist_row_chunks16(p->n_max);
    for (int k = 0; k < L1; ++k) {
        const gist_layer_desc &l = p->layer[k];
        f.dw_bytes[k] = slab_need(l.n_out, 2 * l.n_in, p->n_max, true);
        if (k == L1 - 1 && gist_class_layer_takes(p->n_max, l.n_out, 2 * l.n_in, 2 * l.n_in, 2 * l.n_in, nullptr, nullptr)) {
            const int64_t b = gist_class_dw_slab_bytes(p->n_max, l.n_out, 2 * l.n_in);
            f.dw_bytes[k] = b > f.dw_bytes[k] ? b : f.dw_bytes[k];
        }
        f.dw_slabs[k] = f.dw_bytes[k] > 0 ? take(f.dw_bytes[k]) : nullptr;
        f.partials[k] = partials ? partials + poff : nullptr;
        const int64_t rows = (k + 1 < L1 && l.n_out <= 256 && chunks < kLnbMaxUnits) ? kLnbMaxUnits : chunks;
        f.partial_rows[k] = rows;
        poff += ceil_div(rows * l.n_out, 64) * 64;
    }
    const gist_layer_desc &last = p->layer[L1 - 1];
    f.logit_bytes = slab_need(2 * last.n_in, last.n_out, p->n_max, false);
    f.logit_slabs = f.logit_bytes > 0 ? take(f.logit_bytes) : nullptr;
    f.y_bytes = 0;
    for (int k = 0; k + 1 < L1; ++k) {
        const int64_t b = slab_need(2 * p->layer[k].n_in, p->layer[k].n_out, p->n_max, false);
        f.y_bytes = b > f.y_bytes ? b : f.y_bytes;
    }
    f.y_slabs = f.y_bytes > 0 ? take(f.y_bytes) : nullptr;
    f.bytes = off;
    f.partial_floats = poff;
    return f;
}
}

extern "C" int64_t gist_step_fused_workspace_bytes(const gist_step_plan *plan) {
    if (!plan || plan->n_layers < 1 || plan->n_layers > GIST_MAX_LAYERS || plan->n_max <= 0) return 0;
    return fused_layout(plan, nullptr, nullptr).bytes;
}
extern "C" int64_t gist_step_fused_slab_bytes(const gist_step_plan *plan, int32_t k) {
    if (!plan || plan->n_layers < 1 || plan->n_layers > GIST_MAX_LAYERS || plan->n_max <= 0) return 0;
    if (k < 0 || k > plan->n_layers + 1) return 0;
    const FusedLayout f = fused_layout(plan, nullptr, nullptr);
    if (k == plan->n_layers + 1) return f.y_bytes;
    return k == plan->n_layers ? f.logit_bytes : f.dw_bytes[k];
}
extern "C" int64_t gist_step_col_partials_floats(const gist_step_plan *plan) {
    if (!plan || plan->n_layers < 1 || plan->n_layers > GIST_MAX_LAYERS || plan->n_max <= 0) return 0;
    return fused_layout(plan, nullptr, nullptr).partial_floats;
}

extern "C" int64_t gist_step_h3_workspace_bytes(const gist_step_plan *plan) {
    return gist_step_h3_workspace_bytes_mode(plan, gist_gemm_get_mode());
}

extern "C" int64_t gist_step_h3_workspace_bytes_mode(const gist_step_plan *plan, int mode) {
    if (!plan || plan->n_layers < 1 || plan->n_layers > GIST_MAX_LAYERS || mode < 0 || mode > 2) return 0;
    return mode == 2 ? b3_layout(plan, nullptr, mode).bytes : h3_layout(plan, nullptr, mode).bytes;
}

static int step_spmm(const gist_step_plan *p, const int32_t *rowptr, const int32_t *col, const float *x,
                     int64_t ldx, float *y, int64_t ldy, int64_t n, int64_t d, const float *out_scale,
                     const float *src_scale, int accumulate, const void *prepared, gist_stream_t s) {
    if (p->row_blocks != nullptr && p->n_row_blocks > 0) {
        if (prepared != nullptr)
            return spmm_prepared(rowptr, col, x, ldx, y, ldy, n, d, out_scale, src_scale, accumulate, p->row_blocks,
                                 p->n_row_blocks, prepared, as_stream(s), p->sibling_parts != 0);
        return gist_spmm_csr_blocked_f32(rowptr, col, x, ldx, y, ldy, n, d, out_scale, src_scale,
                                         accumulate, p->row_blocks, p->n_row_blocks, s);
    }
    return gist_spmm_csr_f32(rowptr, col, x, ldx, y, ldy, n, d, out_scale, src_scale, accumulate, s);
}

constexpr int64_t kPrefetchMaxParams = 12LL << 20;
static bool next_parts_ok(const gist_step_plan *p, bool fuse) {
    return fuse && p->node_part && p->part_slot && p->extract_scratch && p->next_ids && p->next_batch_index >= 0 &&
           p->next_n > 0 && p->next_n <= p->n_max && gist_extract_parts_supported(p->n_max) == 1;
}

extern "C" int gist_sage_step_extracts_next(const gist_step_plan *p, int64_t n, int flags) {
    if (p == nullptr || !(flags & GIST_STEP_TRAIN) || n <= 0) return 0;
    const bool fuse = p->fuse != 0 && n <= p->n_max;
    if (!fuse || p->col_partials == nullptr || !aligned16(p->col_partials)) return 0;
    const FusedLayout fl = fused_layout(p, static_cast<char *>(p->fused_workspace), p->col_partials);
    const bool defer = p->fused_workspace == nullptr ? fl.bytes == 0
                                                     : (aligned16(p->fused_workspace) && fl.bytes <= p->fused_workspace_bytes);
    if (p->n_params > kPrefetchMaxParams) return 0;
    return defer && next_parts_ok(p, fuse) ? 1 : 0;
}

extern "C" int gist_sage_step(const gist_step_plan *p, const int32_t *ids, int64_t n,
                              uint64_t drop_offset, float lr, float beta1, float beta2,
                              float eps, float weight_decay, int64_t adam_step, int flags,
                              gist_stream_t s) {
    GIST_REQUIRE(p != nullptr, "gist_sage_step: null plan");
    GIST_REQUIRE(p->n_layers >= 1 && p->n_layers <= GIST_MAX_LAYERS, "gist_sage_step: bad n_layers");
    GIST_REQUIRE(n > 0, "gist_sage_step: empty batch");
    GIST_REQUIRE(!((flags & GIST_STEP_EXTRACT) && (flags & GIST_STEP_PREEXTRACTED)),
                 "gist_sage_step: GIST_STEP_EXTRACT and GIST_STEP_PREEXTRACTED exclude each other");
    GIST_REQUIRE(!(flags & (GIST_STEP_EXTRACT_NEXT | GIST_STEP_PREEXTRACTED)) || (flags & GIST_STEP_TRAIN),
                 "gist_sage_step: GIST_STEP_EXTRACT_NEXT / GIST_STEP_PREEXTRACTED belong to training steps");
    const int L1 = p->n_layers;
    hipStream_t st = as_stream(s);
    ActiveTimer active(p->timer);
    const bool train = (flags & GIST_STEP_TRAIN) != 0;
    const bool drop = train && p->p_drop > 0.f;
    const int phase_bits = flags & (GIST_STEP_PHASE_FORWARD | GIST_STEP_PHASE_BACKWARD | GIST_STEP_PHASE_OPTIMIZER);
    GIST_REQUIRE(phase_bits == 0 || train, "gist_sage_step: GIST_STEP_PHASE_* belong to training steps");
    GIST_REQUIRE(!(flags & GIST_STEP_DLOGITS_GIVEN) || phase_bits == GIST_STEP_PHASE_BACKWARD,
                 "gist_sage_step: GIST_STEP_DLOGITS_GIVEN belongs to a GIST_STEP_PHASE_BACKWARD call");
    const bool do_fwd = phase_bits == 0 || (phase_bits & GIST_STEP_PHASE_FORWARD);
    const bool do_bwd = train && (phase_bits == 0 || (phase_bits & GIST_STEP_PHASE_BACKWARD));
    const bool do_opt = train && (phase_bits == 0 || (phase_bits & GIST_STEP_PHASE_OPTIMIZER));
    const bool split_phases = phase_bits != 0 && phase_bits != (GIST_STEP_PHASE_FORWARD | GIST_STEP_PHASE_BACKWARD |
                                                                GIST_STEP_PHASE_OPTIMIZER);
    GIST_REQUIRE(!split_phases || ((do_fwd ? 1 : 0) + (do_bwd ? 1 : 0) + (do_opt ? 1 : 0)) == 1,
                 "gist_sage_step: one GIST_STEP_PHASE_* per call (or none / all three)");
    const bool dlogits_given = (flags & GIST_STEP_DLOGITS_GIVEN) != 0;
    const bool blocked = p->row_blocks != nullptr && p->n_row_blocks > 0;
    const bool pairs = p->sibling_parts != 0;

    const int gemm_mode = gist_gemm_get_mode();
    H3Step h3{};
    if (p->h3_workspace != nullptr && aligned16(p->h3_workspace) && n <= p->n_max) {
        h3 = h3_layout(p, static_cast<char *>(p->h3_workspace), gemm_mode);
        if (h3.bytes > p->h3_workspace_bytes) h3 = H3Step{};
    }
    B3Step b3{};
    if (p->h3_workspace != nullptr && aligned16(p->h3_workspace) && n <= p->n_max) {
        b3 = b3_layout(p, static_cast<char *>(p->h3_workspace), gemm_mode);
        if (b3.bytes > p->h3_workspace_bytes) b3 = B3Step{};
    }

    const bool fuse = p->fuse != 0 && n <= p->n_max;
    FusedLayout fl{};
    bool defer = false;
    if (fuse && p->col_partials != nullptr && aligned16(p->col_partials)) {
        fl = fused_layout(p, static_cast<char *>(p->fused_workspace), p->col_partials);
        defer = p->fused_workspace == nullptr ? fl.bytes == 0
                                              : (aligned16(p->fused_workspace) && fl.bytes <= p->fused_workspace_bytes);
        if (!defer) fl = FusedLayout{};
    }
    uint64_t offs[GIST_MAX_LAYERS];
    {
        uint64_t off = drop_offset;
        for (int k = 0; k < L1; ++k) {
            offs[k] = off;
            if (drop) off += round_up2((uint64_t)n * 2 * p->layer[k].n_in);
        }
    }
    bool plain[GIST_MAX_LAYERS], fwd_fold[GIST_MAX_LAYERS], bwd_fold[GIST_MAX_LAYERS];
    for (int k = 0; k < L1; ++k) {
        const gist_layer_desc &l = p->layer[k];
        plain[k] = !h3.layer[k].on && !b3.layer[k].on;
        fwd_fold[k] = fuse && drop && plain[k] && p->hsrc[k] != nullptr && (offs[k] & 1) == 0 &&
                      (k > 0 || (flags & (GIST_STEP_EXTRACT | GIST_STEP_PREEXTRACTED))) &&
                      p->ld_hsrc[k] >= l.n_in &&
                      spmm_drop_takes(1, l.n_in, p->ld_hsrc[k], l.ldz, p->hsrc[k], l.Z + l.n_in, blocked ? p->row_blocks : nullptr);
        bwd_fold[k] = fuse && drop && plain[k] && k > 0 && k < L1 - 1 && (offs[k] & 1) == 0 &&
                      spmm_drop_takes(2, l.n_in, 2 * l.n_in, 2 * l.n_in, p->dZ + l.n_in, p->dZ, blocked ? p->row_blocks : nullptr);
    }
    const float keep = drop ? 1.0f / (1.0f - p->p_drop) : 1.f;
    const uint64_t sm = p->seed * 0x9E3779B97F4A7C15ULL;
    bool cls_fused = false;
    {
        const gist_layer_desc &l = p->layer[L1 - 1];
        cls_fused = train && defer && plain[L1 - 1] && p->ldc <= 64 && (offs[L1 - 1] & 1) == 0 &&
                    (int)tune(GIST_TUNE_CLASS_FUSED) != 1 &&
                    gist_class_layer_takes(n, l.n_out, 2 * l.n_in, l.ldz, 2 * l.n_in, l.Z, l.W) == 1 &&
                    fl.dw_slabs[L1 - 1] != nullptr &&
                    fl.dw_bytes[L1 - 1] >= gist_class_dw_slab_bytes(n, l.n_out, 2 * l.n_in);
    }
    bool bwd_fold_split[GIST_MAX_LAYERS];
    for (int k = 0; k < L1; ++k) {
        const gist_layer_desc &l = p->layer[k];
        bwd_fold_split[k] = fuse && drop && !plain[k] && k > 0 && k < L1 - 1 && (offs[k] & 1) == 0 &&
                            spmm_drop_takes(2, l.n_in, 2 * l.n_in, 2 * l.n_in, p->dZ + l.n_in, p->dZ,
                                            blocked ? p->row_blocks : nullptr);
    }

    if (b3.any && do_fwd) {
        Scope sc(p->timer, 3, 0, 0, 0, st);
        for (int k = 0; k < L1; ++k) {
            const B3Layer &hl = b3.layer[k];
            if (!hl.on) continue;
            const gist_layer_desc &l = p->layer[k];
            B3Dual d{};
            d.src = l.W; d.ld = 2 * l.n_in; d.rows = l.n_out; d.cols = 2 * l.n_in;
            d.dst_r = hl.Ws;
            d.dst_t = train ? hl.WsT : nullptr;
            GIST_TRY(b3_dual_split(d, st));
        }
    }
    if (h3.any && do_fwd) {
        Scope sc(p->timer, 3, 0, 0, 0, st);
        bool zeroed = false;
        for (int k = 0; k < L1; ++k) {
            const H3Layer &hl = h3.layer[k];
            if (!hl.on) continue;
            const gist_layer_desc &l = p->layer[k];
            if (k > 0 && train) {
                if (!zeroed) {
                    if (hipMemsetAsync(h3.amax, 0, GIST_MAX_LAYERS * 4, st) != hipSuccess) {
                        set_error("gist_sage_step: hipMemsetAsync failed");
                        return GIST_ELAUNCH;
                    }
                    zeroed = true;
                }
                GIST_TRY(h3_absmax(l.W, 2 * l.n_in, l.n_out, 2 * l.n_in, h3.amax + k, st));
                H3Dual d{};
                d.src = l.W; d.ld = 2 * l.n_in; d.rows = l.n_out; d.cols = 2 * l.n_in;
                d.amax = h3.amax + k;
                d.dst_r = hl.Ws; d.inv_r = hl.inv_wr; d.dst_t = hl.WsT; d.inv_t = hl.inv_wt;
                GIST_TRY(h3_dual_split(d, st));
            } else {
                GIST_TRY(h3_split_rows(l.W, 2 * l.n_in, l.n_out, 2 * l.n_in, hl.Ws, hl.inv_wr, st));
            }
        }
    }

    bool pre_ah = (flags & GIST_STEP_PREEXTRACTED) && p->feat_intra != nullptr;
    if ((flags & GIST_STEP_EXTRACT) && do_fwd) {
        GIST_REQUIRE(ids != nullptr, "gist_sage_step: null ids");
        const gist_layer_desc &l0 = p->layer[0];
        const bool by_parts = fuse && p->node_part && p->part_slot && p->extract_scratch && p->batch_index >= 0 && n <= p->n_max &&
                              gist_extract_parts_supported(p->n_max) == 1;
        if (by_parts) {
            gist_extract_parts_desc x{};
            x.g_rowptr = p->g_rowptr; x.g_col = p->g_col; x.g_t_rowptr = p->g_t_rowptr; x.g_t_col = p->g_t_col;
            x.ids = ids; x.n = n; x.n_max = p->n_max;
            x.node_part = p->node_part; x.part_slot = p->part_slot; x.batch = p->batch_index;
            x.rowptr = p->rowptr; x.col = p->col; x.t_rowptr = p->t_rowptr; x.t_col = p->t_col;
            x.col_capacity = p->col_capacity; x.norm = p->norm;
            x.feat = p->feat; x.ld_feat = p->ld_feat; x.n_feat = l0.n_in; x.z0 = l0.Z; x.ldz0 = l0.ldz;
            x.labels_all = p->labels_all; x.labels = p->labels;
            x.x0 = fwd_fold[0] ? p->hsrc[0] : nullptr; x.ldx0 = p->ld_hsrc[0]; x.p = p->p_drop; x.seed = p->seed;
            x.offset = offs[0]; x.mask_ld = 2 * l0.n_in; x.scratch = p->extract_scratch;
            if (p->feat_intra != nullptr) {
                x.feat_intra = p->feat_intra; x.ld_intra = p->ld_feat_intra; x.ah = l0.Z + l0.n_in;
                pre_ah = true;
            }
            GIST_TRY(gist_extract_parts_desc_batch(&x, s));
        } else if (fwd_fold[0])
            GIST_TRY(gist_extract_batch_drop(p->g_rowptr, p->g_col, p->g_t_rowptr, p->g_t_col, ids, n,
                                             p->remap, p->rowptr, p->col, p->t_rowptr, p->t_col,
                                             p->col_capacity, p->norm, p->feat, p->ld_feat, l0.n_in, l0.Z,
                                             l0.ldz, p->labels_all, p->labels, p->hsrc[0], p->ld_hsrc[0],
                                             p->p_drop, p->seed, offs[0], 2 * l0.n_in, s));
        else
            GIST_TRY(gist_extract_batch(p->g_rowptr, p->g_col, p->g_t_rowptr, p->g_t_col, ids, n,
                                        p->remap, p->rowptr, p->col, p->t_rowptr, p->t_col,
                                        p->col_capacity, p->norm, p->feat, p->ld_feat,
                                        l0.n_in, l0.Z, l0.ldz, p->labels_all, p->labels, s));
    }

    const void *prep_fwd = nullptr, *prep_bwd = nullptr;
    if (blocked && p->spmm_prepared != nullptr && aligned16(p->spmm_prepared)) {
        const int64_t one = gist_spmm_blocks_bytes(p->n_row_blocks);
        bool wide = false;
        for (int k = 0; k < L1; ++k)
            wide = wide || spmm_prepared_takes(p->layer[k].n_in, p->layer[k].ldz, p->layer[k].ldz,
                                               p->layer[k].Z, p->layer[k].Z + p->layer[k].n_in);
        if (wide && p->spmm_prepared_bytes >= (train ? 2 : 1) * one) {
            char *base = static_cast<char *>(p->spmm_prepared);
            if (do_fwd)
            GIST_TRY(launch_spmm_blocks_prepare(p->rowptr, p->col, train ? p->t_rowptr : nullptr,
                                                train ? p->t_col : nullptr, n, p->row_blocks, p->n_row_blocks,
                                                base, train ? base + one : nullptr, st, pairs));
            prep_fwd = base;
            prep_bwd = train ? base + one : nullptr;
        }
    }

    int logit_slabs = 0;
    for (int k = 0; k < L1 && do_fwd; ++k) {
        const gist_layer_desc &l = p->layer[k];
        int y_slabs_n = 1;
        const float *y_slabs = nullptr;
        if (!(k == 0 && pre_ah)) {
            Scope sc(p->timer, 0, n, n, l.n_in, st);
            if (fwd_fold[k]) {
                SpmmDrop dr{};
                dr.mode = 1; dr.p = p->p_drop; dr.scale = keep; dr.sm = sm;
                dr.y_base = offs[k] + (uint64_t)l.n_in; dr.src_base = 0; dr.ld = 2 * l.n_in;
                GIST_TRY(spmm_drop(p->rowptr, p->col, p->hsrc[k], p->ld_hsrc[k], l.Z + l.n_in, l.ldz, n, l.n_in,
                                   p->norm, nullptr, 0, blocked ? p->row_blocks : nullptr, p->n_row_blocks, dr, st,
                                   prep_fwd, pairs));
            } else {
                GIST_TRY(step_spmm(p, p->rowptr, p->col, l.Z, l.ldz, l.Z + l.n_in, l.ldz, n, l.n_in,
                                   p->norm, nullptr, 0, prep_fwd, s));
            }
        }
        if (h3.layer[k].on) {
            const H3Layer &hl = h3.layer[k];
            Scope sc(p->timer, 1, n, l.n_out, 2 * l.n_in, st);
            H3Dual d{};
            d.src = l.Z; d.ld = l.ldz; d.rows = n; d.cols = 2 * l.n_in;
            d.p = drop ? p->p_drop : 0.f; d.seed = p->seed; d.offset = offs[k];
            d.fixed_shift = hl.shift;
            d.dst_r = hl.Zs; d.inv_r = hl.inv_zr;
            d.dst_t = train ? hl.ZsT : nullptr; d.inv_t = hl.inv_zt;
            GIST_TRY(h3_dual_split(d, st));
            GIST_TRY(h3_gemm_presplit("gist_sage_step", hl.Zs, hl.inv_zr, hl.Ws, hl.inv_wr, l.b, l.Y,
                                      l.ldy, n, l.n_out, 2 * l.n_in, st));
        } else if (b3.layer[k].on) {
            const B3Layer &hl = b3.layer[k];
            Scope sc(p->timer, 1, n, l.n_out, 2 * l.n_in, st);
            B3Dual d{};
            d.src = l.Z; d.ld = l.ldz; d.rows = n; d.cols = 2 * l.n_in;
            d.p = drop ? p->p_drop : 0.f; d.seed = p->seed; d.offset = offs[k];
            d.dst_r = hl.Zs;
            d.dst_t = train ? hl.ZsT : nullptr;
            GIST_TRY(b3_dual_split(d, st));
            const bool to_ln = defer && k + 1 < L1;
            GIST_TRY(b3_gemm_presplit("gist_sage_step", hl.Zs, hl.Ws, l.b, l.Y, l.ldy, n, l.n_out,
                                      2 * l.n_in, b3.slabs, b3.slab_bytes, st, to_ln ? &y_slabs_n : nullptr));
            if (to_ln) y_slabs = b3.slabs;
        } else {
            if (drop && !fwd_fold[k])
                GIST_TRY(gist_dropout_f32(l.Z, l.ldz, n, 2 * l.n_in, p->p_drop, p->seed, offs[k], s));
            if (cls_fused && k == L1 - 1) continue;
            Scope sc(p->timer, 1, n, l.n_out, 2 * l.n_in, st);
            if (defer && k == L1 - 1 && fl.logit_slabs != nullptr) {
                GIST_TRY(gemm_slabs(0, l.Z, l.ldz, l.W, 2 * l.n_in, l.b, l.Y, l.ldy, n, l.n_out, 2 * l.n_in,
                                    fl.logit_slabs, fl.logit_bytes, &logit_slabs, st));
            } else if (defer && k + 1 < L1 && fl.y_slabs != nullptr && !h3_eligible(n, l.n_out, 2 * l.n_in) &&
                       !b3_eligible(n, l.n_out, 2 * l.n_in)) {
                GIST_TRY(gemm_slabs(0, l.Z, l.ldz, l.W, 2 * l.n_in, l.b, l.Y, l.ldy, n, l.n_out, 2 * l.n_in,
                                    fl.y_slabs, fl.y_bytes, &y_slabs_n, st));
                y_slabs = fl.y_slabs;
            } else {
                GIST_TRY(gist_gemm_nt_f32(l.Z, l.ldz, l.W, 2 * l.n_in, l.b, l.Y, l.ldy, n, l.n_out,
                                          2 * l.n_in, p->workspace, p->workspace_bytes, s));
            }
        }
        if (k + 1 < L1) {
            const gist_layer_desc &nx = p->layer[k + 1];
            if (y_slabs_n > 1)
// ... 122 lines not shown
        }
        if (b3.layer[k].on) {
            const B3Layer &hl = b3.layer[k];
            {
                Scope sc(p->timer, 3, 0, 0, 0, st);
                B3Dual d{};
                d.src = dy; d.ld = lddy; d.rows = n; d.cols = l.n_out;
                d.dst_r = k > 0 ? b3.dYs : nullptr;
                d.dst_t = b3.dYsT;
                d.col_partials = defer && fl.partials[k] != nullptr ? fl.partials[k] : p->partials;
                GIST_TRY(b3_dual_split(d, st));
            }
            if (defer && fl.partials[k] != nullptr) {
                gist_grad_segment &g = segs[n_segs++];
                g.begin = l.db - p->grads; g.end = g.begin + l.n_out;
                g.src = fl.partials[k]; g.stride = l.n_out; g.n_src = (int32_t)gist_colsum_partials(n);
            } else {
                GIST_TRY(colsum_finish(p->partials, gist_colsum_partials(n), l.n_out, l.db, st));
            }
            if (k > 0) {
                Scope sc(p->timer, 1, n, 2 * l.n_in, l.n_out, st);
                GIST_TRY(b3_gemm_presplit("gist_sage_step", b3.dYs, hl.WsT, nullptr, p->dZ, 2 * l.n_in, n,
                                          2 * l.n_in, l.n_out, b3.slabs, b3.slab_bytes, st));
            }
            {
                Scope sc(p->timer, 1, l.n_out, 2 * l.n_in, n, st);
                int ns = 1;
                GIST_TRY(b3_gemm_presplit("gist_sage_step", b3.dYsT, hl.ZsT, nullptr, l.dW, 2 * l.n_in,
                                          l.n_out, 2 * l.n_in, n, b3.slabs, b3.slab_bytes, st,
                                          defer && k == 0 ? &ns : nullptr));
                if (ns > 1) {
                    gist_grad_segment &g = segs[n_segs++];
                    g.begin = l.dW - p->grads; g.end = g.begin + l.n_out * 2 * l.n_in;
                    g.src = b3.slabs; g.stride = l.n_out * 2 * l.n_in; g.n_src = ns;
                }
            }
            if (k > 0) {
                if (bwd_fold_split[k]) {
                    Scope sc(p->timer, 0, n, n, l.n_in, st);
                    SpmmDrop dr{};
                    dr.mode = 2; dr.p = p->p_drop; dr.scale = keep; dr.sm = sm;
                    dr.y_base = offs[k]; dr.src_base = offs[k] + (uint64_t)l.n_in; dr.ld = 2 * l.n_in;
                    GIST_TRY(spmm_drop(p->t_rowptr, p->t_col, p->dZ + l.n_in, 2 * l.n_in, p->dZ, 2 * l.n_in, n,
                                       l.n_in, nullptr, p->norm, 1, p->row_blocks, p->n_row_blocks, dr, st, prep_bwd,
                                       pairs));
                } else {
                    if (drop)
                        GIST_TRY(gist_dropout_f32(p->dZ, 2 * l.n_in, n, 2 * l.n_in, p->p_drop, p->seed,
                                                  offs[k], s));
                    Scope sc(p->timer, 0, n, n, l.n_in, st);
                    GIST_TRY(step_spmm(p, p->t_rowptr, p->t_col, p->dZ + l.n_in, 2 * l.n_in, p->dZ,
                                       2 * l.n_in, n, l.n_in, nullptr, p->norm, 1, prep_bwd, s));
                }
            }
            continue;
        }
        bool dual_done = false;
        if (defer && k > 0 && k < L1 - 1 && db_done && (!drop || bwd_fold[k]) &&
            gemm_dual_takes(n, 2 * l.n_in, l.n_out, lddy, 2 * l.n_in, l.ldz, 2 * l.n_in, dy, l.W, l.Z, p->dZ)) {
            Scope sc(p->timer, 1, n, 4 * l.n_in, l.n_out, st);
            int ns = 1;
            GIST_TRY(gemm_dual_nn_tn("gist_sage_step", dy, lddy, l.W, 2 * l.n_in, p->dZ, 2 * l.n_in, l.Z, l.ldz, l.dW,
                                     2 * l.n_in, n, 2 * l.n_in, l.n_out, fl.dw_slabs[k], fl.dw_bytes[k], &ns, st));
            if (ns > 1) {
                gist_grad_segment &g = segs[n_segs++];
                g.begin = l.dW - p->grads; g.end = g.begin + l.n_out * 2 * l.n_in;
                g.src = fl.dw_slabs[k]; g.stride = l.n_out * 2 * l.n_in; g.n_src = ns;
            }
            dual_done = true;
        }
        if (dual_done) {
        } else if (cls_dz_done && k == L1 - 1) {
            db_done = true;
        } else if (k > 0) {
            Scope sc(p->timer, 1, n, 2 * l.n_in, l.n_out, st);
            const bool chunk_db = defer && k == L1 - 1;
            GIST_TRY(gemm_nn_dropout_ex("gist_sage_step", dy, lddy, l.W, 2 * l.n_in, p->dZ, 2 * l.n_in, n,
                                        2 * l.n_in, l.n_out, (drop && !bwd_fold[k]) ? p->p_drop : 0.f, p->seed,
                                        offs[k], p->workspace, p->workspace_bytes,
                                        chunk_db ? fl.partials[k] : nullptr, st));
            db_done = db_done || chunk_db;
        }
        if (!dual_done) {
            const bool dw_with_ln = cls_fused && k == L1 - 1 && L1 >= 2 && defer && plain[L1 - 2] &&
                                    (int)tune(GIST_TUNE_CLASS_FUSED) != 2;
            Scope sc(dw_with_ln ? nullptr : p->timer, 1, l.n_out, 2 * l.n_in, n, st);
            if (cls_fused && k == L1 - 1) {
                int32_t ns = 1;
                if (dw_with_ln) {
                    GIST_TRY(class_dw_args("gist_sage_step", dy, lddy, l.Z, l.ldz, fl.dw_slabs[k], fl.dw_bytes[k], n, l.n_out,
                                           2 * l.n_in, &dw_args, &ns));
                    dw_pending = true;
                } else {
                    GIST_TRY(gist_class_dw_slabs_f32(dy, lddy, l.Z, l.ldz, fl.dw_slabs[k], fl.dw_bytes[k], &ns, n, l.n_out,
                                                     2 * l.n_in, s));
                }
                gist_grad_segment &g = segs[n_segs++];
                g.begin = l.dW - p->grads; g.end = g.begin + l.n_out * 2 * l.n_in;
                g.src = fl.dw_slabs[k]; g.stride = l.n_out * 2 * l.n_in; g.n_src = ns;
            } else if (defer && fl.dw_slabs[k] != nullptr) {
                int ns = 1;
                GIST_TRY(gemm_slabs(2, dy, lddy, l.Z, l.ldz, nullptr, l.dW, 2 * l.n_in, l.n_out, 2 * l.n_in, n,
                                    fl.dw_slabs[k], fl.dw_bytes[k], &ns, st));
                if (ns > 1) {
                    gist_grad_segment &g = segs[n_segs++];
                    g.begin = l.dW - p->grads; g.end = g.begin + l.n_out * 2 * l.n_in;
                    g.src = fl.dw_slabs[k]; g.stride = l.n_out * 2 * l.n_in; g.n_src = ns;
                }
            } else {
                GIST_TRY(gist_gemm_tn_f32(dy, lddy, l.Z, l.ldz, l.dW, 2 * l.n_in, l.n_out,
                                          2 * l.n_in, n, p->workspace, p->workspace_bytes, s));
            }
        }
        if (defer) {
            if (!db_done)
                GIST_TRY(colsum_rows16(dy, lddy, n, l.n_out, fl.partials[k], k == L1 - 1 ? false : true, st));
            bias_segment(k, db_rows);
        } else {
            GIST_TRY(gist_colsum_f32(dy, lddy, n, l.n_out, p->partials, l.db, s));
        }
        if (k > 0) {
            Scope sc(p->timer, 0, n, n, l.n_in, st);
            if (bwd_fold[k]) {
                SpmmDrop dr{};
                dr.mode = 2; dr.p = p->p_drop; dr.scale = keep; dr.sm = sm;
                dr.y_base = offs[k]; dr.src_base = offs[k] + (uint64_t)l.n_in; dr.ld = 2 * l.n_in;
                const gist_layer_desc &lo = p->layer[k - 1];
                SpmmLnBwd ln{};
                const int64_t units = blocked ? spmm_lnb_units(p->n_row_blocks) : 0;
                const bool with_ln = defer && plain[k - 1] && !dw_pending && (int)tune(GIST_TUNE_LNB_FUSED) != 1 &&
                                     units > 0 && units <= fl.partial_rows[k - 1] && lo.ldy % 4 == 0 && aligned16(lo.Y) &&
                                     (!p->use_layernorm || lo.rstd != nullptr) &&
                                     spmm_lnb_takes(l.n_in, 2 * l.n_in, 2 * l.n_in, p->dZ + l.n_in, p->dZ, p->row_blocks, prep_bwd);
                if (with_ln) {
                    ln.yhat = lo.Y; ln.ldy = lo.ldy; ln.rstd = p->use_layernorm ? lo.rstd : nullptr;
                    ln.dy = lo.Y; ln.lddy = lo.ldy; ln.col_partials = fl.partials[k - 1]; ln.relu = 1;
                    lnb_rows = units;
                }
                GIST_TRY(spmm_drop(p->t_rowptr, p->t_col, p->dZ + l.n_in, 2 * l.n_in, p->dZ, 2 * l.n_in, n,
                                   l.n_in, nullptr, p->norm, 1, p->row_blocks, p->n_row_blocks, dr, st, prep_bwd,
                                   pairs, with_ln ? &ln : nullptr));
            } else {
                GIST_TRY(step_spmm(p, p->t_rowptr, p->t_col, p->dZ + l.n_in, 2 * l.n_in, p->dZ,
                                   2 * l.n_in, n, l.n_in, nullptr, p->norm, 1, prep_bwd, s));
            }
        }
    }
    GIST_REQUIRE(!dw_pending, "gist_sage_step: internal error (class-layer weight gradient not launched)");
    if (do_bwd && !do_opt) {
        if (defer && n_segs > 0) GIST_TRY(gist_grad_segments_finish_f32(p->grads, p->n_params, segs, n_segs, s));
        return GIST_OK;
    }
    if (!do_opt) return GIST_OK;
    if (!do_bwd) n_segs = 0;
    const float *opt_row_loss = do_bwd || !split_phases ? p->row_loss : nullptr;
    if (defer && (flags & GIST_STEP_EXTRACT_NEXT) && next_parts_ok(p, fuse) && p->n_params <= kPrefetchMaxParams) {
        const gist_layer_desc &l0 = p->layer[0];
        const bool fold0 = fuse && drop && plain[0] && p->hsrc[0] != nullptr && (p->next_drop_offset & 1) == 0 &&
                           p->ld_hsrc[0] >= l0.n_in &&
                           spmm_drop_takes(1, l0.n_in, p->ld_hsrc[0], l0.ldz, p->hsrc[0], l0.Z + l0.n_in,
                                           blocked ? p->row_blocks : nullptr);
        gist_extract_parts_desc x{};
        x.g_rowptr = p->g_rowptr; x.g_col = p->g_col; x.g_t_rowptr = p->g_t_rowptr; x.g_t_col = p->g_t_col;
        x.ids = p->next_ids; x.n = p->next_n; x.n_max = p->n_max;
        x.node_part = p->node_part; x.part_slot = p->part_slot; x.batch = p->next_batch_index;
        x.rowptr = p->rowptr; x.col = p->col; x.t_rowptr = p->t_rowptr; x.t_col = p->t_col;
        x.col_capacity = p->col_capacity; x.norm = p->norm;
        x.feat = p->feat; x.ld_feat = p->ld_feat; x.n_feat = l0.n_in; x.z0 = l0.Z; x.ldz0 = l0.ldz;
        x.labels_all = p->labels_all; x.labels = p->labels;
        x.x0 = fold0 ? p->hsrc[0] : nullptr; x.ldx0 = p->ld_hsrc[0]; x.p = p->p_drop; x.seed = p->seed;
        x.offset = p->next_drop_offset; x.mask_ld = 2 * l0.n_in; x.scratch = p->extract_scratch;
        if (p->feat_intra != nullptr) { x.feat_intra = p->feat_intra; x.ld_intra = p->ld_feat_intra; x.ah = l0.Z + l0.n_in; }
        GIST_TRY(gist_adam_segments_extract_f32(p->params, p->grads, p->exp_avg, p->exp_avg_sq, p->n_params, lr, beta1,
                                                beta2, eps, weight_decay, adam_step, segs, n_segs, opt_row_loss, n, n,
                                                p->loss, &x, s));
    } else if (defer)
        GIST_TRY(gist_adam_segments_f32(p->params, p->grads, p->exp_avg, p->exp_avg_sq, p->n_params, lr, beta1,
                                        beta2, eps, weight_decay, adam_step, segs, n_segs, opt_row_loss, n, n,
                                        p->loss, s));
    else
        GIST_TRY(gist_adam_f32(p->params, p->grads, p->exp_avg, p->exp_avg_sq, p->n_params, lr, beta1,
                               beta2, eps, weight_decay, adam_step, s));
    return GIST_OK;
}
```

### gist_amd/csrc/subgraph.hip

```cpp
#include "common.h"
#include "adam_body.h"

namespace gist {

__global__ void mark_kernel(const int32_t *__restrict__ ids, int64_t n, int32_t *__restrict__ remap,
                            int unmark) {
    const int64_t i = (int64_t)blockIdx.x * blockDim.x + threadIdx.x;
    if (i < n) remap[ids[i]] = unmark ? -1 : (int32_t)i;
}

__global__ void fill_i32_kernel(int32_t *__restrict__ p, int64_t n, int32_t v) {
    for (int64_t i = (int64_t)blockIdx.x * blockDim.x + threadIdx.x; i < n;
         i += (int64_t)gridDim.x * blockDim.x)
        p[i] = v;
}

__global__ __launch_bounds__(256) void induced_count_kernel(
    const int32_t *__restrict__ rowptr, const int32_t *__restrict__ col,
    const int32_t *__restrict__ ids, int n_ids, const int32_t *__restrict__ remap,
    int32_t *__restrict__ out) {
    const int i = blockIdx.x * 4 + (threadIdx.x >> 6);
    if (i >= n_ids) return;
    const int lane = threadIdx.x & 63;
    const int v = ids[i];
// ... 610 lines not shown
    float tail = 0.f;
    const int m = n_src < kMax ? n_src : kMax;
    for (int k = 0; k < kMax; ++k) v[k] = k < m ? src[(int64_t)k * stride + j] : 0.f;
    for (int k = kMax; k < n_src; ++k) tail += src[(int64_t)k * stride + j];
#pragma unroll
    for (int w = 1; w < kMax; w <<= 1)
#pragma unroll
        for (int k = 0; k + w < kMax; k += 2 * w) v[k] += v[k + w];
    out[j] = (v[0] + tail) / (float)n_src;
}

}

using namespace gist;

static int mark_impl(const char *name, const int32_t *ids, int64_t n_ids, int32_t *remap, int unmark,
                     gist_stream_t stream) {
    if (n_ids < 0) { set_error("%s: n_ids < 0", name); return GIST_EINVAL; }
    if (n_ids == 0) return GIST_OK;
    if (!ids || !remap) { set_error("%s: null pointer", name); return GIST_EINVAL; }
    hipLaunchKernelGGL(mark_kernel, dim3((unsigned)ceil_div(n_ids, 256)), dim3(256), 0,
                       as_stream(stream), ids, n_ids, remap, unmark);
    return launch_status(name);
}

extern "C" int gist_induced_mark(const int32_t *ids, int64_t n_ids, int32_t *remap,
                                 gist_stream_t stream) {
    return mark_impl("gist_induced_mark", ids, n_ids, remap, 0, stream);
}

extern "C" int gist_induced_unmark(const int32_t *ids, int64_t n_ids, int32_t *remap,
                                   gist_stream_t stream) {
    return mark_impl("gist_induced_unmark", ids, n_ids, remap, 1, stream);
}

extern "C" int gist_fill_i32(int32_t *p, int64_t n, int32_t value, gist_stream_t stream) {
    GIST_REQUIRE(n >= 0, "gist_fill_i32: n < 0");
    if (n == 0) return GIST_OK;
    GIST_REQUIRE(p, "gist_fill_i32: null pointer");
    const unsigned grid = (unsigned)(ceil_div(n, 256) < 4096 ? ceil_div(n, 256) : 4096);
    hipLaunchKernelGGL(fill_i32_kernel, dim3(grid), dim3(256), 0, as_stream(stream), p, n, value);
    return launch_status("gist_fill_i32");
}

__global__ void copy_i32_kernel(const int32_t *__restrict__ src, int32_t *__restrict__ dst, int64_t n) {
    for (int64_t i = (int64_t)blockIdx.x * blockDim.x + threadIdx.x; i < n; i += (int64_t)gridDim.x * blockDim.x)
        dst[i] = src[i];
}

extern "C" int gist_copy_i32(const int32_t *src, int32_t *dst, int64_t n, gist_stream_t stream) {
    GIST_REQUIRE(n >= 0, "gist_copy_i32: n < 0");
    if (n == 0) return GIST_OK;
    GIST_REQUIRE(src && dst, "gist_copy_i32: null pointer");
    const unsigned grid = (unsigned)(ceil_div(n, 256) < 1024 ? ceil_div(n, 256) : 1024);
    hipLaunchKernelGGL(copy_i32_kernel, dim3(grid), dim3(256), 0, as_stream(stream), src, dst, n);
    return launch_status("gist_copy_i32");
}

__global__ void publish_i64_kernel(const int64_t *__restrict__ device_word, int64_t tag, volatile int64_t *host_word) {
    host_word[0] = device_word ? *device_word : 0;
    __threadfence_system();
    host_word[1] = tag;
    __threadfence_system();
}

extern "C" int gist_publish_i64(const int64_t *device_word, int64_t tag, int64_t *host_word, gist_stream_t stream) {
    GIST_REQUIRE(host_word, "gist_publish_i64: null pointer");
    hipLaunchKernelGGL(publish_i64_kernel, dim3(1), dim3(1), 0, as_stream(stream), device_word, tag, host_word);
    return launch_status("gist_publish_i64");
}

extern "C" int gist_induced_rowptr(const int32_t *rowptr, const int32_t *col, const int32_t *ids,
                                   int64_t n_ids, const int32_t *remap, int32_t *sub_rowptr,
                                   gist_stream_t stream) {
    GIST_REQUIRE(n_ids >= 0 && n_ids < (1LL << 31) - 8, "gist_induced_rowptr: bad n_ids");
    GIST_REQUIRE(sub_rowptr, "gist_induced_rowptr: null sub_rowptr");
    hipStream_t st = as_stream(stream);
    if (n_ids > 0) {
        GIST_REQUIRE(rowptr && col && ids && remap, "gist_induced_rowptr: null pointer");
        hipLaunchKernelGGL(induced_count_kernel, dim3((unsigned)ceil_div(n_ids, 4)), dim3(256), 0, st,
                           rowptr, col, ids, (int)n_ids, remap, sub_rowptr);
    }
    hipLaunchKernelGGL(scan_rowptr_kernel, dim3(1), dim3(1024), 0, st, sub_rowptr, (int)n_ids);
    return launch_status("gist_induced_rowptr");
}

extern "C" int gist_induced_fill(const int32_t *rowptr, const int32_t *col, const int32_t *ids,
                                 int64_t n_ids, const int32_t *remap, const int32_t *sub_rowptr,
                                 int32_t *sub_col, int64_t sub_col_capacity, gist_stream_t stream) {
    GIST_REQUIRE(n_ids >= 0 && n_ids < (1LL << 31) - 8, "gist_induced_fill: bad n_ids");
    GIST_REQUIRE(sub_col_capacity >= 0, "gist_induced_fill: negative capacity");
    if (n_ids == 0) return GIST_OK;
    GIST_REQUIRE(rowptr && col && ids && remap && sub_rowptr, "gist_induced_fill: null pointer");
    GIST_REQUIRE(sub_col || sub_col_capacity == 0, "gist_induced_fill: null sub_col");
    hipLaunchKernelGGL(induced_fill_kernel, dim3((unsigned)ceil_div(n_ids, 4)), dim3(256), 0,
                       as_stream(stream), rowptr, col, ids, (int)n_ids, remap, sub_rowptr, sub_col,
                       sub_col_capacity);
    return launch_status("gist_induced_fill");
}

extern "C" int gist_gather_rows_f32(const float *src, int64_t lds_, const int32_t *ids,
                                    int64_t n_ids, int64_t d, float *dst, int64_t ldd,
                                    gist_stream_t stream) {
    GIST_REQUIRE(n_ids >= 0 && d >= 0, "gist_gather_rows_f32: negative size");
    if (n_ids == 0 || d == 0) return GIST_OK;
    GIST_REQUIRE(src && ids && dst, "gist_gather_rows_f32: null pointer");
    GIST_REQUIRE(lds_ >= d && ldd >= d, "gist_gather_rows_f32: leading dimension < d");
    GIST_REQUIRE(n_ids < (1LL << 31) - 8 && d < (1LL << 31), "gist_gather_rows_f32: size >= 2^31");
    hipStream_t st = as_stream(stream);
    const dim3 grid((unsigned)ceil_div(n_ids, 4));
    if (d % 4 == 0 && lds_ % 4 == 0 && ldd % 4 == 0 && aligned16(src) && aligned16(dst))
        hipLaunchKernelGGL(gather_rows_kernel<4>, grid, dim3(256), 0, st, src, lds_, ids, (int)n_ids,
                           (int)d, dst, ldd);
    else if (d % 2 == 0 && lds_ % 2 == 0 && ldd % 2 == 0 && aligned8(src) && aligned8(dst))
        hipLaunchKernelGGL(gather_rows_kernel<2>, grid, dim3(256), 0, st, src, lds_, ids, (int)n_ids,
                           (int)d, dst, ldd);
    else
        hipLaunchKernelGGL(gather_rows_kernel<1>, grid, dim3(256), 0, st, src, lds_, ids, (int)n_ids,
                           (int)d, dst, ldd);
    return launch_status("gist_gather_rows_f32");
}

extern "C" int gist_gather_i32(const int32_t *src, const int32_t *ids, int64_t n_ids, int32_t *dst,
                               gist_stream_t stream) {
    GIST_REQUIRE(n_ids >= 0, "gist_gather_i32: n_ids < 0");
    if (n_ids == 0) return GIST_OK;
    GIST_REQUIRE(src && ids && dst, "gist_gather_i32: null pointer");
    hipLaunchKernelGGL(gather_i32_kernel, dim3((unsigned)ceil_div(n_ids, 256)), dim3(256), 0,
                       as_stream(stream), src, ids, n_ids, dst);
    return launch_status("gist_gather_i32");
}

static int block_move(const char *name, bool scatter, const float *src, int64_t lds_,
                      const int32_t *row_idx, const int32_t *col_idx, int64_t n_rows,
                      int64_t n_cols, float *dst, int64_t ldd, gist_stream_t stream) {
    if (n_rows < 0 || n_cols < 0) { set_error("%s: negative size", name); return GIST_EINVAL; }
    if (n_rows == 0 || n_cols == 0) return GIST_OK;
    if (!src || !dst) { set_error("%s: null pointer", name); return GIST_EINVAL; }
    if (n_rows >= (1LL << 31) || n_cols >= (1LL << 31)) { set_error("%s: size >= 2^31", name); return GIST_EINVAL; }
    const unsigned gx = (unsigned)(ceil_div(n_cols, 256) < 64 ? ceil_div(n_cols, 256) : 64);
    const unsigned gy = (unsigned)(n_rows < 8192 ? n_rows : 8192);
    if (scatter)
        hipLaunchKernelGGL(block_move_kernel<true>, dim3(gx, gy), dim3(256), 0, as_stream(stream), src,
                           lds_, row_idx, col_idx, (int)n_rows, (int)n_cols, dst, ldd);
    else
        hipLaunchKernelGGL(block_move_kernel<false>, dim3(gx, gy), dim3(256), 0, as_stream(stream), src,
                           lds_, row_idx, col_idx, (int)n_rows, (int)n_cols, dst, ldd);
    return launch_status(name);
}

extern "C" int gist_block_gather_f32(const float *src, int64_t lds_, const int32_t *row_idx,
                                     const int32_t *col_idx, int64_t n_rows, int64_t n_cols,
                                     float *dst, int64_t ldd, gist_stream_t stream) {
    return block_move("gist_block_gather_f32", false, src, lds_, row_idx, col_idx, n_rows, n_cols,
                      dst, ldd, stream);
}

extern "C" int gist_block_scatter_f32(const float *src, int64_t lds_, const int32_t *row_idx,
                                      const int32_t *col_idx, int64_t n_rows, int64_t n_cols,
                                      float *dst, int64_t ldd, gist_stream_t stream) {
    return block_move("gist_block_scatter_f32", true, src, lds_, row_idx, col_idx, n_rows, n_cols,
                      dst, ldd, stream);
}

extern "C" int gist_mean_rows_f32(const float *src, int64_t stride, int64_t n_src, int64_t n,
                                  float *out, gist_stream_t stream) {
    GIST_REQUIRE(n_src > 0 && n >= 0, "gist_mean_rows_f32: bad size");
    if (n == 0) return GIST_OK;
    GIST_REQUIRE(src && out, "gist_mean_rows_f32: null pointer");
    hipLaunchKernelGGL(mean_rows_kernel, dim3((unsigned)ceil_div(n, 256)), dim3(256), 0,
                       as_stream(stream), src, stride, (int)n_src, n, out);
    return launch_status("gist_mean_rows_f32");
}

static int extract_impl(const int32_t *g_rowptr, const int32_t *g_col,
                                  const int32_t *g_t_rowptr, const int32_t *g_t_col,
                                  const int32_t *ids, int64_t n, int32_t *remap, int32_t *rowptr,
                                  int32_t *col, int32_t *t_rowptr, int32_t *t_col,
                                  int64_t col_capacity, float *norm, const float *feat,
                                  int64_t ld_feat, int64_t n_feat, float *z0, int64_t ldz0,
                                  const int32_t *labels_all, int32_t *labels, const GatherDrop *drop,
                                  gist_stream_t stream) {
    GIST_REQUIRE(n > 0 && n < (1LL << 31) - 8, "gist_extract_batch: bad n");
    GIST_REQUIRE(g_rowptr && g_col && g_t_rowptr && g_t_col && ids && remap && rowptr && col &&
                     t_rowptr && t_col && norm && feat && z0,
                 "gist_extract_batch: null pointer");
    GIST_REQUIRE(n_feat > 0 && ld_feat >= n_feat && ldz0 >= n_feat && n_feat < (1LL << 31),
                 "gist_extract_batch: bad feature shape");
    GIST_REQUIRE(col_capacity >= 0, "gist_extract_batch: negative capacity");
    hipStream_t st = as_stream(stream);
    CsrPair p;
    p.rowptr[0] = g_rowptr; p.col[0] = g_col; p.sub_rowptr[0] = rowptr; p.sub_col[0] = col;
    p.rowptr[1] = g_t_rowptr; p.col[1] = g_t_col; p.sub_rowptr[1] = t_rowptr; p.sub_col[1] = t_col;
    const unsigned nb4 = (unsigned)ceil_div(n, 4);
    hipLaunchKernelGGL(mark_kernel, dim3((unsigned)ceil_div(n, 256)), dim3(256), 0, st, ids, n, remap, 0);
    hipLaunchKernelGGL(induced_count2_kernel, dim3(nb4, 2), dim3(256), 0, st, p, ids, (int)n, remap, norm);
    hipLaunchKernelGGL(scan_rowptr2_kernel, dim3(2), dim3(1024), 0, st, rowptr, t_rowptr, (int)n);
    hipLaunchKernelGGL(induced_fill2_kernel, dim3(nb4, 2), dim3(256), 0, st, p, ids, (int)n, remap,
                       col_capacity);
    GatherDrop gd{};
    if (drop != nullptr) {
        gd = *drop;
        GIST_REQUIRE(gd.x0 != nullptr && gd.ldx0 >= n_feat && gd.mask_ld >= n_feat && gd.p >= 0.f && gd.p < 1.f,
                     "gist_extract_batch_drop: bad dropout arguments");
        if (n_feat % 2 == 0)
            hipLaunchKernelGGL((gather_batch_kernel<2, true>), dim3(nb4), dim3(256), 0, st, feat, ld_feat, ids,
                               (int)n, (int)n_feat, z0, ldz0, labels_all, labels, remap, gd);
        else
            hipLaunchKernelGGL((gather_batch_kernel<1, true>), dim3(nb4), dim3(256), 0, st, feat, ld_feat, ids,
                               (int)n, (int)n_feat, z0, ldz0, labels_all, labels, remap, gd);
        return launch_status("gist_extract_batch_drop");
    }
    if (n_feat % 4 == 0 && ld_feat % 4 == 0 && ldz0 % 4 == 0 && aligned16(feat) && aligned16(z0))
        hipLaunchKernelGGL(gather_batch_kernel<4>, dim3(nb4), dim3(256), 0, st, feat, ld_feat, ids,
                           (int)n, (int)n_feat, z0, ldz0, labels_all, labels, remap, gd);
    else if (n_feat % 2 == 0 && ld_feat % 2 == 0 && ldz0 % 2 == 0 && aligned8(feat) && aligned8(z0))
        hipLaunchKernelGGL(gather_batch_kernel<2>, dim3(nb4), dim3(256), 0, st, feat, ld_feat, ids,
                           (int)n, (int)n_feat, z0, ldz0, labels_all, labels, remap, gd);
    else
        hipLaunchKernelGGL(gather_batch_kernel<1>, dim3(nb4), dim3(256), 0, st, feat, ld_feat, ids,
                           (int)n, (int)n_feat, z0, ldz0, labels_all, labels, remap, gd);
    return launch_status("gist_extract_batch");
}

extern "C" int gist_extract_batch(const int32_t *g_rowptr, const int32_t *g_col,
                                  const int32_t *g_t_rowptr, const int32_t *g_t_col,
                                  const int32_t *ids, int64_t n, int32_t *remap, int32_t *rowptr,
                                  int32_t *col, int32_t *t_rowptr, int32_t *t_col,
                                  int64_t col_capacity, float *norm, const float *feat,
                                  int64_t ld_feat, int64_t n_feat, float *z0, int64_t ldz0,
                                  const int32_t *labels_all, int32_t *labels,
                                  gist_stream_t stream) {
    return extract_impl(g_rowptr, g_col, g_t_rowptr, g_t_col, ids, n, remap, rowptr, col, t_rowptr, t_col,
                        col_capacity, norm, feat, ld_feat, n_feat, z0, ldz0, labels_all, labels, nullptr,
                        stream);
}

extern "C" int gist_extract_batch_drop(const int32_t *g_rowptr, const int32_t *g_col,
                                       const int32_t *g_t_rowptr, const int32_t *g_t_col,
                                       const int32_t *ids, int64_t n, int32_t *remap, int32_t *rowptr,
                                       int32_t *col, int32_t *t_rowptr, int32_t *t_col,
                                       int64_t col_capacity, float *norm, const float *feat,
                                       int64_t ld_feat, int64_t n_feat, float *z0, int64_t ldz0,
                                       const int32_t *labels_all, int32_t *labels, float *x0, int64_t ldx0,
                                       float p, uint64_t seed, uint64_t offset, int64_t mask_ld,
                                       gist_stream_t stream) {
    GatherDrop gd{};
    gd.x0 = x0; gd.ldx0 = ldx0; gd.p = p; gd.scale = (p > 0.f && p < 1.f) ? 1.0f / (1.0f - p) : 1.f;
    gd.sm = seed * 0x9E3779B97F4A7C15ULL; gd.offset = offset; gd.mask_ld = mask_ld;
    return extract_impl(g_rowptr, g_col, g_t_rowptr, g_t_col, ids, n, remap, rowptr, col, t_rowptr, t_col,
                        col_capacity, norm, feat, ld_feat, n_feat, z0, ldz0, labels_all, labels, &gd, stream);
}


extern "C" int64_t gist_extract_parts_scratch_bytes(int64_t n_max) {
    return n_max <= 0 ? 0 : 32 + 16 * ceil_div(n_max, kPartsWaves);
}

extern "C" int gist_extract_parts_supported(int64_t n_max) {
    return n_max > 0 && n_max < (1LL << 31) - 64 ? 1 : 0;
}

static int parts_args(const char *name, const gist_extract_parts_desc &x, PartsArgs *out) {
    GIST_REQUIRE(x.n > 0 && x.n <= x.n_max && x.n_max < (1LL << 31) - 8, "%s: bad n", name);
    GIST_REQUIRE(x.g_rowptr && x.g_col && x.g_t_rowptr && x.g_t_col && x.ids && x.node_part && x.part_slot && x.rowptr &&
                     x.col && x.t_rowptr && x.t_col && x.norm && x.feat && x.z0 && x.scratch,
                 "%s: null pointer", name);
    GIST_REQUIRE(aligned8(x.node_part) && aligned8(x.part_slot), "%s: tables must be 8-byte aligned", name);
    GIST_REQUIRE(x.n_feat > 0 && x.ld_feat >= x.n_feat && x.ldz0 >= x.n_feat && x.n_feat < (1LL << 31),
                 "%s: bad feature shape", name);
    GIST_REQUIRE(x.col_capacity >= 0 && x.batch >= 0, "%s: bad capacity / batch index", name);
    GIST_REQUIRE(aligned8(x.scratch), "%s: scratch must be 8-byte aligned", name);
    GIST_REQUIRE(gist_extract_parts_supported(x.n_max) == 1, "%s: bad n_max", name);
    static std::atomic<unsigned long long> g_epoch{0};
    const unsigned long long epoch = (g_epoch.fetch_add(1, std::memory_order_relaxed) + 1) & ((1ULL << 33) - 1);
    GIST_REQUIRE(epoch != 0, "%s: launch counter exhausted", name);
    PartsArgs a{};
    a.p.rowptr[0] = x.g_rowptr; a.p.col[0] = x.g_col; a.p.sub_rowptr[0] = x.rowptr; a.p.sub_col[0] = x.col;
    a.p.rowptr[1] = x.g_t_rowptr; a.p.col[1] = x.g_t_col; a.p.sub_rowptr[1] = x.t_rowptr; a.p.sub_col[1] = x.t_col;
    a.ids = x.ids; a.n = (int)x.n; a.n_max = (int)x.n_max;
    a.node_part = x.node_part; a.part_slot = x.part_slot;
    a.batch = x.batch; a.capacity = x.col_capacity; a.norm = x.norm;
    a.error = static_cast<unsigned long long *>(x.scratch) + 1;
    a.tickets = static_cast<unsigned long long *>(x.scratch) + 2;
    a.slots = static_cast<unsigned long long *>(x.scratch) + 4;
    a.epoch = epoch;
    a.feat = x.feat; a.ld_feat = x.ld_feat; a.d = (int)x.n_feat; a.z0 = x.z0; a.ldz0 = x.ldz0;
    a.labels_all = x.labels_all; a.labels = x.labels;
    a.drop = 0;
    if (x.x0 != nullptr) {
        GIST_REQUIRE(x.ldx0 >= x.n_feat && x.mask_ld >= x.n_feat && x.p >= 0.f && x.p < 1.f, "%s: bad dropout arguments", name);
        a.drop = 1;
        a.gd.x0 = x.x0; a.gd.ldx0 = x.ldx0; a.gd.p = x.p; a.gd.scale = x.p > 0.f ? 1.0f / (1.0f - x.p) : 1.f;
        a.gd.sm = x.seed * 0x9E3779B97F4A7C15ULL; a.gd.offset = x.offset; a.gd.mask_ld = x.mask_ld;
    }
    if (x.ah != nullptr) {
        GIST_REQUIRE(x.feat_intra != nullptr && x.ld_intra >= x.n_feat, "%s: bad feat_intra", name);
        GIST_REQUIRE(x.x0 == nullptr || x.mask_ld >= 2 * x.n_feat, "%s: mask pitch below 2 n_feat with ah", name);
        a.feat_intra = x.feat_intra; a.ld_intra = x.ld_intra; a.ah = x.ah;
        a.gd.offset = x.offset; a.gd.mask_ld = x.mask_ld;
    }
    *out = a;
    return GIST_OK;
}

extern "C" int gist_extract_parts_desc_batch(const gist_extract_parts_desc *desc, gist_stream_t stream) {
    GIST_REQUIRE(desc != nullptr, "gist_extract_parts_desc_batch: null descriptor");
    PartsArgs a;
    const int rc = parts_args("gist_extract_parts_desc_batch", *desc, &a);
    if (rc != GIST_OK) return rc;
    hipLaunchKernelGGL(extract_parts_kernel, dim3((unsigned)ceil_div(desc->n, kPartsWaves), 3),
                       dim3(64 * kPartsWaves), 0, as_stream(stream), a);
    return launch_status("gist_extract_parts_desc_batch");
}

extern "C" int gist_extract_parts_batch(const int32_t *g_rowptr, const int32_t *g_col,
                                        const int32_t *g_t_rowptr, const int32_t *g_t_col,
                                        const int32_t *ids, int64_t n, int64_t n_max,
                                        const int32_t *node_part, const int32_t *part_slot, int32_t batch,
                                        int32_t *rowptr, int32_t *col, int32_t *t_rowptr, int32_t *t_col,
                                        int64_t col_capacity, float *norm, const float *feat, int64_t ld_feat,
                                        int64_t n_feat, float *z0, int64_t ldz0, const int32_t *labels_all,
                                        int32_t *labels, float *x0, int64_t ldx0, float p, uint64_t seed,
                                        uint64_t offset, int64_t mask_ld, void *scratch, gist_stream_t stream) {
    gist_extract_parts_desc x{};
    x.g_rowptr = g_rowptr; x.g_col = g_col; x.g_t_rowptr = g_t_rowptr; x.g_t_col = g_t_col;
    x.ids = ids; x.n = n; x.n_max = n_max; x.node_part = node_part; x.part_slot = part_slot; x.batch = batch;
    x.rowptr = rowptr; x.col = col; x.t_rowptr = t_rowptr; x.t_col = t_col; x.col_capacity = col_capacity; x.norm = norm;
    x.feat = feat; x.ld_feat = ld_feat; x.n_feat = n_feat; x.z0 = z0; x.ldz0 = ldz0;
    x.labels_all = labels_all; x.labels = labels;
    x.x0 = x0; x.ldx0 = ldx0; x.p = p; x.seed = seed; x.offset = offset; x.mask_ld = mask_ld; x.scratch = scratch;
    PartsArgs a;
    const int rc = parts_args("gist_extract_parts_batch", x, &a);
    if (rc != GIST_OK) return rc;
    hipLaunchKernelGGL(extract_parts_kernel, dim3((unsigned)ceil_div(n, kPartsWaves), 3),
                       dim3(64 * kPartsWaves), 0, as_stream(stream), a);
    return launch_status("gist_extract_parts_batch");
}

extern "C" int gist_adam_segments_extract_f32(float *param, float *grad, float *exp_avg, float *exp_avg_sq,
                                              int64_t n, float lr, float beta1, float beta2, float eps,
                                              float weight_decay, int64_t step, const gist_grad_segment *segments,
                                              int64_t n_segments, const float *row_loss, int64_t n_loss_rows,
                                              int64_t loss_count, float *loss, const gist_extract_parts_desc *next,
                                              gist_stream_t stream) {
    GIST_REQUIRE(next != nullptr, "gist_adam_segments_extract_f32: null descriptor");
    gist::AdamArgs A;
    int rc = gist::adam_segments_args("gist_adam_segments_extract_f32", param, grad, exp_avg, exp_avg_sq, n, lr, beta1,
                                      beta2, eps, weight_decay, step, segments, n_segments, row_loss, n_loss_rows,
                                      loss_count, loss, &A);
    if (rc != GIST_OK) return rc;
    PartsArgs a;
    rc = parts_args("gist_adam_segments_extract_f32", *next, &a);
    if (rc != GIST_OK) return rc;
    const int64_t gx = ceil_div(next->n, kPartsWaves);
    const int64_t blocks = 3 * gx + ceil_div((int64_t)A.segs.n_ded, 4) + (row_loss ? 1 : 0) +
                           ceil_div(gist::adam_arena_blocks(n), 4);
    GIST_REQUIRE(blocks < (1LL << 31), "gist_adam_segments_extract_f32: grid too large");
    hipLaunchKernelGGL(adam_extract_kernel, dim3((unsigned)blocks), dim3(64 * kPartsWaves), 0, as_stream(stream), a, (int)gx, A);
    return launch_status("gist_adam_segments_extract_f32");
}
```

### gist_amd/engine.py

```python
import os
import weakref

import numpy as np
import torch

from . import hip


def _round_up(x, m):
    return (x + m - 1) // m * m


class ParamArena(object):

    def __init__(self, dims, device, with_grads=True):
        self.dims = list(dims)
        self.offsets = []
        off = 0
        for (i, o) in self.dims:
            self.offsets.append((off, off + o * 2 * i))
            off += o * 2 * i + o
        self.numel = off
        self.device = device
        self.params = torch.zeros(off, dtype=torch.float32, device=device)
        self.W, self.b, self.dW, self.db = [], [], [], []
        for (i, o), (w0, b0) in zip(self.dims, self.offsets):
            self.W.append(self.params[w0:b0].view(o, 2 * i))
            self.b.append(self.params[b0:b0 + o])
        self.grads = self.exp_avg = self.exp_avg_sq = None
        if with_grads:
            self.grads = torch.zeros(off, dtype=torch.float32, device=device)
            self.exp_avg = torch.zeros(off, dtype=torch.float32, device=device)
            self.exp_avg_sq = torch.zeros(off, dtype=torch.float32, device=device)
            for (i, o), (w0, b0) in zip(self.dims, self.offsets):
                self.dW.append(self.grads[w0:b0].view(o, 2 * i))
                self.db.append(self.grads[b0:b0 + o])
        self.step = 0

    def reset_optimizer(self):
        self.exp_avg.zero_()
        self.exp_avg_sq.zero_()
        self.step = 0

    def load(self, params):
        for k, (W, b) in enumerate(params):
            self.W[k].copy_(torch.as_tensor(W).to(self.device))
            self.b[k].copy_(torch.as_tensor(b).to(self.device))

    def export(self):
        return [(W.detach().cpu().numpy().copy(), b.detach().cpu().numpy().copy())
                for W, b in zip(self.W, self.b)]

    def adopt_module(self, gcn):
        for k, layer in enumerate(gcn.layers):
            self.W[k].copy_(layer.linear.weight.data.to(self.device))
            self.b[k].copy_(layer.linear.bias.data.to(self.device))
            layer.linear.weight.data = self.W[k]
            layer.linear.bias.data = self.b[k]

    def bind_module(self, gcn):
        gcn.__dict__['_gist_arena'] = weakref.ref(self)


class Batch(object):
    __slots__ = ('n', 'rowptr', 'col', 't_rowptr', 't_col', 'norm', 'labels', 'ids', 'ready',
                 'row_blocks', 'batcher', 'parts', 'z0_dropped', 'next_info', 'ah_owner', 'siblings')

    def __init__(self):
        self.ready = True
        self.z0_dropped = False
        self.row_blocks = None
        self.batcher = None
        self.parts = None
        self.next_info = None
        self.siblings = True
        self.ah_owner = None


class ClusterBatcher(object):

    def __init__(self, graph, feat, labels, n_max, nnz_max):
        dev = graph.device
        assert dev.type == 'cuda', 'ClusterBatcher needs the training graph on the GPU'
        self.g, self.feat, self.labels = graph, feat, labels
        self.n_max, self.nnz_max = int(n_max), int(max(nnz_max, 1))
        i32 = dict(dtype=torch.int32, device=dev)
        self.remap = torch.empty(graph.number_of_nodes(), **i32)
        hip.fill_i32_(self.remap, -1)
        self.rowptr = torch.zeros(self.n_max + 1, **i32)
        self.t_rowptr = torch.zeros(self.n_max + 1, **i32)
        self.col = torch.zeros(self.nnz_max, **i32)
        self.t_col = torch.zeros(self.nnz_max, **i32)
        self.norm = torch.zeros(self.n_max, dtype=torch.float32, device=dev)
        self.lab = torch.zeros(self.n_max, **i32)
        self.feat_intra = None
        self.prefetched = None

    def lazy(self, ids):
        n = ids.numel()
        if n > self.n_max:
            raise ValueError('gist_amd: batch of %d rows exceeds n_max=%d' % (n, self.n_max))
        b = Batch()
        b.n, b.rowptr, b.col = n, self.rowptr[:n + 1], self.col
        b.t_rowptr, b.t_col = self.t_rowptr[:n + 1], self.t_col
        b.norm, b.labels, b.ids = self.norm[:n], self.lab[:n], ids
        b.ready = False
        b.batcher = self
        return b

    def extract(self, ids, z0_left, drop=None):
        n = ids.numel()
        if n > self.n_max:
            raise ValueError('gist_amd: batch of %d rows exceeds n_max=%d' % (n, self.n_max))
        self.prefetched = None
        g = self.g
        rp, trp = self.rowptr[:n + 1], self.t_rowptr[:n + 1]
        if drop is not None:
            hip.extract_batch_drop(g, ids, self.remap, rp, self.col, trp, self.t_col, self.norm, self.feat,
                                   z0_left, self.labels, self.lab, *drop)
        else:
            hip.extract_batch(g, ids, self.remap, rp, self.col, trp, self.t_col, self.norm, self.feat,
                              z0_left, self.labels, self.lab)
        b = Batch()
        b.n, b.rowptr, b.col, b.t_rowptr, b.t_col = n, rp, self.col, trp, self.t_col
        b.norm, b.labels, b.ids = self.norm[:n], self.lab[:n], ids
        return b


class SageEngine(object):
    def __init__(self, dims, use_layernorm, dropout, n_max, device, seed=0, arena=None):
        self.dims = [(int(i), int(o)) for i, o in dims]
        self.L1 = len(self.dims)
        self.use_layernorm = bool(use_layernorm)
        self.p_drop = float(dropout) if dropout else 0.0
        self.n_max = int(n_max)
        self.device = device
        self.seed = int(seed)
        self.drop_calls = 0
        self.arena = arena if arena is not None else ParamArena(self.dims, device)
        f32 = dict(dtype=torch.float32, device=device)
        self.Z = [torch.zeros(self.n_max, 2 * i, **f32) for (i, o) in self.dims]
        self.n_classes = self.dims[-1][1]
        self.ldc = _round_up(self.n_classes, 4)
        self.Y = [torch.zeros(self.n_max, o, **f32) for (i, o) in self.dims[:-1]]
        self.Y.append(torch.zeros(self.n_max, self.ldc, **f32))
        self.dlogits = torch.zeros(self.n_max, self.ldc, **f32)
        self.rstd = [torch.zeros(self.n_max, **f32) for _ in self.dims[:-1]]
        wide = max([2 * i for (i, o) in self.dims[1:]] + [4])
        self.dZ = torch.zeros(self.n_max * wide, **f32)
        max_out = max(o for (i, o) in self.dims)
        self.partials = torch.zeros(
            max(1, hip._lib.load().gist_colsum_partials(self.n_max)) * max_out, **f32)
        self.row_loss = torch.zeros(self.n_max, **f32)
        self.loss = torch.zeros(1, **f32)
        self.correct = torch.zeros(1, dtype=torch.int32, device=device)
        need = 0
        L = hip._lib.load()
        for (i, o) in self.dims:
            for (m, n, k) in ((self.n_max, o, 2 * i), (self.n_max, 2 * i, o), (o, 2 * i, self.n_max)):
                need = max(need, L.gist_gemm_workspace_bytes(m, n, k))
        self._ws = hip.workspace(need, device)
        self._ws2 = torch.empty(max(int(need), 1 << 20), dtype=torch.uint8, device=device)
        self._drop_offsets = []
        self.fuse = os.environ.get('GIST_STEP_FUSE', '1') != '0'
        self.H = [None] * self.L1
        if self.fuse and self.p_drop > 0.0:
            for k, (i, o) in enumerate(self.dims):
                ld = i if i % 4 == 0 else _round_up(i + 2, 4)
                self.H[k] = torch.zeros(self.n_max, ld, **f32)
        self._fused = None
        self._extract_scratch = None
        self.prefetch = False
        self._prefetch_refused = None
        self._segments = []
        self._logit_slabs_n = 1
        self.plan = None
        self._spmm_prep = None
        self._plan_keep = None

    def attach_batcher(self, batcher):
        from . import _lib
        A = self.arena
        if A.grads is None:
            raise ValueError('gist_amd: the native step needs an arena with gradients')
        if self.L1 > _lib.GIST_MAX_LAYERS:
            return None
        P = _lib.StepPlan()
        P.n_layers = self.L1
        P.use_layernorm = int(self.use_layernorm)
        P.p_drop = self.p_drop
        P.seed = self.seed
        for k, (i, o) in enumerate(self.dims):
            l = P.layer[k]
            l.n_in, l.n_out = i, o
            l.W, l.b = A.W[k].data_ptr(), A.b[k].data_ptr()
            l.dW, l.db = A.dW[k].data_ptr(), A.db[k].data_ptr()
            l.Z, l.ldz = self.Z[k].data_ptr(), 2 * i
            l.Y, l.ldy = self.Y[k].data_ptr(), self.Y[k].shape[1]
            l.rstd = self.rstd[k].data_ptr() if k < self.L1 - 1 else None
        P.dlogits, P.ldc = self.dlogits.data_ptr(), self.ldc
        P.dZ, P.partials = self.dZ.data_ptr(), self.partials.data_ptr()
        P.row_loss, P.loss = self.row_loss.data_ptr(), self.loss.data_ptr()
        P.workspace, P.workspace_bytes = self._ws.data_ptr(), self._ws.numel()
        P.workspace2, P.workspace2_bytes = self._ws2.data_ptr(), self._ws2.numel()
        P.params, P.grads = A.params.data_ptr(), A.grads.data_ptr()
        P.exp_avg, P.exp_avg_sq = A.exp_avg.data_ptr(), A.exp_avg_sq.data_ptr()
        P.n_params = A.numel
        g = batcher.g
        P.g_rowptr, P.g_col = g.rowptr.data_ptr(), g.col.data_ptr()
        P.g_t_rowptr, P.g_t_col = g.t_rowptr.data_ptr(), g.t_col.data_ptr()
        P.feat, P.ld_feat = batcher.feat.data_ptr(), batcher.feat.stride(0)
        fi = getattr(batcher, 'feat_intra', None)
        if fi is not None and self.fuse:
            P.feat_intra, P.ld_feat_intra = fi.data_ptr(), fi.stride(0)
        else:
            P.feat_intra, P.ld_feat_intra = None, 0
        P.labels_all, P.remap = batcher.labels.data_ptr(), batcher.remap.data_ptr()
        P.rowptr, P.col = batcher.rowptr.data_ptr(), batcher.col.data_ptr()
        P.t_rowptr, P.t_col = batcher.t_rowptr.data_ptr(), batcher.t_col.data_ptr()
        P.col_capacity = batcher.col.numel()
        P.norm, P.labels = batcher.norm.data_ptr(), batcher.lab.data_ptr()
        P.n_max = self.n_max
        P.feat_absmax = float(batcher.feat.abs().max().item()) if batcher.feat.numel() else 0.0
        import ctypes
        L_ = _lib.load()
        cur = L_.gist_gemm_get_mode()
        need = 0
        for m_ in ((1, 2) if cur != 0 else ()):
            need = max(need, L_.gist_step_h3_workspace_bytes_mode(ctypes.byref(P), m_))
        self._h3_ws = None
        if need > 0 and os.environ.get('GIST_STEP_H3', '1') != '0':
            self._h3_ws = torch.empty(need, dtype=torch.uint8, device=self.device)
            P.h3_workspace, P.h3_workspace_bytes = self._h3_ws.data_ptr(), need
        if self._spmm_prep is not None:
            P.spmm_prepared, P.spmm_prepared_bytes = self._spmm_prep.data_ptr(), self._spmm_prep.numel()
        P.fuse = int(self.fuse)
        self._fused_ws = self._col_partials = None
        if self.fuse:
            for k in range(self.L1):
                if self.H[k] is not None:
                    P.hsrc[k], P.ld_hsrc[k] = self.H[k].data_ptr(), self.H[k].stride(0)
            nf = L_.gist_step_col_partials_floats(ctypes.byref(P))
            self._col_partials = torch.zeros(max(int(nf), 4), dtype=torch.float32, device=self.device)
            P.col_partials = self._col_partials.data_ptr()
            nb = L_.gist_step_fused_workspace_bytes(ctypes.byref(P))
            if nb > 0:
                self._fused_ws = torch.empty(int(nb), dtype=torch.uint8, device=self.device)
                P.fused_workspace, P.fused_workspace_bytes = self._fused_ws.data_ptr(), int(nb)
        self.plan = P
        self._plan_keep = (batcher, g, self._ws, self._ws2, self._h3_ws, self._fused_ws,
                           self._col_partials)
        return P

    def check_extract(self):
        if self._extract_scratch is not None and int(self._extract_scratch[1].item()) != 0:
            raise RuntimeError('gist_amd: gist_extract_parts_batch timed out at its grid barrier; '
                               'the batches extracted since the last check are invalid')

    def check_extract_deferred(self):
        if self._extract_scratch is None:
            return
        import time
        if getattr(self, '_mark', None) is None:
            self._mark = torch.zeros(2, dtype=torch.int64, pin_memory=True)
            self._mark_np = self._mark.numpy()
            self._mark_tag = 0
        prev = self._mark_tag
        if prev > 0:
            deadline = None
            while int(self._mark_np[1]) < prev:
                if deadline is None:
                    deadline = time.time() + 600.0
                elif time.time() > deadline:
                    raise RuntimeError('gist_amd: the GPU never reached the progress mark of the previous epoch')
                time.sleep(5e-5)
            if int(self._mark_np[0]) != 0:
                raise RuntimeError('gist_amd: gist_extract_parts_batch timed out at its grid barrier; '
                                   'the batches extracted since the last check are invalid')
        self._mark_tag = prev + 1
        hip.publish_i64_raw(self._extract_scratch[1:2].data_ptr(), self._mark_tag, self._mark.data_ptr())

    def enable_timer(self, capacity):
        from . import _lib
        L = _lib.load()
        if self.plan is None:
            raise RuntimeError('gist_amd: enable_timer needs attach_batcher first')
        self.disable_timer()
        self._timer = L.gist_timer_create(int(capacity))
        self.plan.timer = self._timer
        return self._timer

    def disable_timer(self):
        from . import _lib
        if getattr(self, '_timer', None):
            _lib.load().gist_timer_destroy(self._timer)
        self._timer = None
        if self.plan is not None:
            self.plan.timer = None

    def read_timer(self):
        import ctypes
        from . import _lib
        L = _lib.load()
        torch.cuda.synchronize(self.device)
        out = []
        ms, kind = ctypes.c_float(), ctypes.c_int32()
        m, n, k = ctypes.c_int64(), ctypes.c_int64(), ctypes.c_int64()
        for i in range(L.gist_timer_count(self._timer)):
            _lib.check(L.gist_timer_read(self._timer, i, ctypes.byref(ms), ctypes.byref(kind),
                                         ctypes.byref(m), ctypes.byref(n), ctypes.byref(k)),
                       'gist_timer_read')
            out.append((ms.value, kind.value, m.value, n.value, k.value))
        return out

    def _native_step(self, b, lr, weight_decay, train, betas=(0.9, 0.999), eps=1e-8, phase=0, given=False,
                     adam_step=None):
        import ctypes
        from . import _lib
        L = _lib.load()
        P = self.plan
        if phase in (_lib.GIST_STEP_PHASE_BACKWARD, _lib.GIST_STEP_PHASE_OPTIMIZER):
            cb, off, flags, ids_ptr = self._phase_ctx
            if cb is not b:
                raise RuntimeError('gist_amd: backward / optimiser phase of a batch that is not the last one forwarded')
            batcher = b.batcher
            nxt = None
            if phase == _lib.GIST_STEP_PHASE_OPTIMIZER:
                nxt, flags = self._plan_next(b, batcher, flags)
                self.arena.step += 1
            elif given:
                flags |= _lib.GIST_STEP_DLOGITS_GIVEN
            rc = L.gist_sage_step(ctypes.byref(P), ids_ptr, b.n, off, lr, betas[0], betas[1], eps, weight_decay,
                                  max(adam_step if adam_step is not None else self.arena.step, 1), flags | phase,
                                  hip._stream())
            _lib.check(rc, 'gist_sage_step')
            if phase == _lib.GIST_STEP_PHASE_OPTIMIZER and batcher is not None:
                batcher.prefetched = nxt
            return self.loss
        off = self.drop_calls
        ids_ptr = b.ids.data_ptr() if b.ids is not None else None
        batcher = b.batcher
        pre = batcher.prefetched if batcher is not None else None
        if batcher is not None:
            batcher.prefetched = None
        pre_ok = (pre is not None and train and not b.ready and b.parts is not None and
                  pre == (b.parts[1].data_ptr(), int(b.parts[2]), b.n, ids_ptr, off, L.gist_gemm_get_mode(), id(self)))
        flags = (_lib.GIST_STEP_TRAIN if train else 0)
        if pre_ok:
            flags |= _lib.GIST_STEP_PREEXTRACTED
        elif not b.ready:
            flags |= _lib.GIST_STEP_EXTRACT
        if train and self.p_drop > 0.0:
            for (i, o) in self.dims:
                numel = b.n * 2 * i
                self.drop_calls += numel + (numel & 1)
        if train and phase == 0:
            self.arena.step += 1
        rb = b.row_blocks
        P.sibling_parts = 1 if b.siblings else 0
        if rb is not None and rb.numel() > 1:
            P.row_blocks, P.n_row_blocks = rb.data_ptr(), rb.numel() - 1
            need = 2 * L.gist_spmm_blocks_bytes(rb.numel() - 1)
            if self._spmm_prep is None or self._spmm_prep.numel() < need:
                self._spmm_prep = torch.empty(need + need // 4, dtype=torch.uint8, device=self.device)
                P.spmm_prepared = self._spmm_prep.data_ptr()
                P.spmm_prepared_bytes = self._spmm_prep.numel()
        else:
            P.row_blocks, P.n_row_blocks = None, 0
        if b.parts is not None and not b.ready and self.fuse and L.gist_extract_parts_supported(self.n_max):
            node_part, tab, j = b.parts
            if self._extract_scratch is None:
                self._extract_scratch = torch.zeros(int(L.gist_extract_parts_scratch_bytes(self.n_max)) // 8 + 1,
                                                    dtype=torch.int64, device=self.device)
            P.node_part, P.part_slot = node_part.data_ptr(), tab.data_ptr()
            P.batch_index, P.extract_scratch = int(j), self._extract_scratch.data_ptr()
        else:
            P.node_part = P.part_slot = P.extract_scratch = None
            P.batch_index = -1
        P.next_ids, P.next_n, P.next_batch_index, P.next_drop_offset = None, 0, -1, 0
        nxt = None
        if phase == 0:
            nxt, flags = self._plan_next(b, batcher, flags)
        else:
            self._phase_ctx = (b, off, flags, ids_ptr)
        rc = L.gist_sage_step(ctypes.byref(P), ids_ptr, b.n, off, lr, betas[0], betas[1],
                              eps, weight_decay, max(adam_step if adam_step is not None else self.arena.step, 1),
                              flags | phase, hip._stream())
        _lib.check(rc, 'gist_sage_step')
        if batcher is not None:
            batcher.prefetched = nxt
        if not b.ready and train and self.fuse and self.p_drop > 0.0 and self.H[0] is not None:
            b.z0_dropped = True
        b.ready = True
        return self.loss

    def _plan_next(self, b, batcher, flags):
        import ctypes
        from . import _lib
        L = _lib.load()
        P = self.plan
        nxt = None
        P.next_ids, P.next_n, P.next_batch_index, P.next_drop_offset = None, 0, -1, 0
        if (self.prefetch and self._prefetch_refused is not True and (flags & _lib.GIST_STEP_TRAIN) and batcher is not None
                and b.next_info is not None and P.node_part is not None and b.row_blocks is not None):
            nids, nj = b.next_info
            P.next_ids, P.next_n, P.next_batch_index = nids.data_ptr(), nids.numel(), int(nj)
            P.next_drop_offset = self.drop_calls
            if L.gist_sage_step_extracts_next(ctypes.byref(P), b.n, flags):
                flags |= _lib.GIST_STEP_EXTRACT_NEXT
                nxt = (P.part_slot, int(nj), nids.numel(), nids.data_ptr(), self.drop_calls, L.gist_gemm_get_mode(),
                       id(self))
            else:
                self._prefetch_refused = True
        return nxt, flags

    def z0_left(self, n):
        return self.Z[0][:n, :self.dims[0][0]]

    def logits(self, n):
        return self.Y[-1][:n, :self.n_classes]

    def _drop_offset(self, numel):
        off = self.drop_calls
        self.drop_calls += numel + (numel & 1)
        return off

    def _fused_buffers(self):
        if self._fused is not None:
            return self._fused
        import ctypes
        from . import _lib
        L = _lib.load()
        P = _lib.StepPlan()
        P.n_layers, P.n_max = self.L1, self.n_max
        for k, (i, o) in enumerate(self.dims):
            P.layer[k].n_in, P.layer[k].n_out = i, o
        u8 = dict(dtype=torch.uint8, device=self.device)
        f32 = dict(dtype=torch.float32, device=self.device)
        chunks = int(L.gist_row_chunks16(self.n_max))
        fb = {'dw': [], 'partials': []}
        for k, (i, o) in enumerate(self.dims):
            nb = int(L.gist_step_fused_slab_bytes(ctypes.byref(P), k))
            fb['dw'].append(torch.empty(nb, **u8) if nb > 0 else None)
            fb['partials'].append(torch.zeros(max(chunks * o, 4), **f32))
        nb = int(L.gist_step_fused_slab_bytes(ctypes.byref(P), self.L1))
        fb['logits'] = torch.empty(nb, **u8) if nb > 0 else None
        nb = int(L.gist_step_fused_slab_bytes(ctypes.byref(P), self.L1 + 1))
        fb['y'] = torch.empty(nb, **u8) if nb > 0 else None
        self._fused = fb
        return fb

    def _offsets(self, n, training):
        offs = []
        if training and self.p_drop > 0.0:
            for (i, o) in self.dims:
                offs.append(self._drop_offset(n * 2 * i))
        return offs

    def forward(self, b, training, _step=False):
        n = b.n
        A = self.arena
        drop = training and self.p_drop > 0.0
        blocked = b.row_blocks is not None and b.row_blocks.numel() > 1
        rb = b.row_blocks if blocked else None
        self._drop_offsets = offs = self._offsets(n, training)
        fold = [False] * self.L1
        if self.fuse and drop:
            for k, (i, o) in enumerate(self.dims):
                fold[k] = (self.H[k] is not None and (k > 0 or (_step and not b.ready)) and
                           hip.spmm_drop_takes(1, i, self.H[k][:n, :i], self.Z[k][:n, i:], blocked))
        self._fwd_fold = fold
        self._pre_ah = False
        if not b.ready:
            if b.batcher is None:
                raise RuntimeError('gist_amd: lazy batch without a batcher')
            i0 = self.dims[0][0]
            dr = (self.H[0][:n, :i0], self.p_drop, self.seed, offs[0], 2 * i0) if fold[0] else None
            fi = getattr(b.batcher, 'feat_intra', None)
            if (fi is not None and b.parts is not None and self.fuse and self.plan is not None and self.plan.feat_intra
                    and hip._lib.load().gist_extract_parts_supported(self.n_max)):
                bt = b.batcher
                if self._extract_scratch is None:
                    self._extract_scratch = torch.zeros(
                        int(hip._lib.load().gist_extract_parts_scratch_bytes(self.n_max)) // 8 + 1,
                        dtype=torch.int64, device=self.device)
                bt.prefetched = None
                hip.extract_parts(bt.g, b.ids, self.n_max, b.parts[0], b.parts[1], b.parts[2], bt.rowptr[:n + 1], bt.col,
                                  bt.t_rowptr[:n + 1], bt.t_col, bt.norm, bt.feat, self.z0_left(n), bt.labels, bt.lab,
                                  self._extract_scratch, drop=dr, feat_intra=fi, ah=self.Z[0][:n, i0:])
                self._pre_ah = True
            else:
                b.batcher.extract(b.ids, self.z0_left(n), drop=dr)
            b.ready = True
            b.z0_dropped = dr is not None
        self._logit_slabs_n = 1
        self._prep_fwd = self._prep_bwd = None
        if blocked and any(hip.spmm_prepared_useful(self.Z[k][:n, :i], self.Z[k][:n, i:])
                           for k, (i, o) in enumerate(self.dims)):
            self._prep_fwd = hip.spmm_prepare(b.rowptr, b.col, rb)
            if training:
                self._prep_bwd = hip.spmm_prepare(b.t_rowptr, b.t_col, rb)
        pf = self._prep_fwd
        for k, (i, o) in enumerate(self.dims):
            z = self.Z[k][:n]
            if not training and o < i and k == self.L1 - 1:
                W = A.W[k]
                p_buf = self.dlogits[:n, :o]
                hip.gemm_nt(z[:, :i], W[:, i:], None, p_buf)
                hip.gemm_nt(z[:, :i], W[:, :i], A.b[k], self.Y[k][:n, :o])
                hip.spmm(b.rowptr, b.col, p_buf, self.Y[k][:n, :o], out_scale=b.norm,
                         accumulate=True)
                continue
            if k == 0 and (self._pre_ah or b.ah_owner is self):
                if drop and not fold[0]:
                    hip.dropout_(z, self.p_drop, self.seed, offs[k])
                    b.ah_owner = None
            elif fold[k]:
                hip.spmm_drop(b.rowptr, b.col, self.H[k][:n, :i], z[:, i:], 1, self.p_drop, self.seed,
                              offs[k] + i, 0, 2 * i, out_scale=b.norm, row_blocks=rb, prepared=pf)
            else:
                hip.spmm(b.rowptr, b.col, z[:, :i], z[:, i:], out_scale=b.norm, row_blocks=b.row_blocks,
                         prepared=pf if blocked else None)
                if drop:
                    hip.dropout_(z, self.p_drop, self.seed, offs[k])
            last = k == self.L1 - 1
            if last:
                self._cls_fused = False
                if self.fuse and training and _step:
                    fb = self._fused_buffers()
                    L_ = hip._lib.load()
                    if (fb['dw'][k] is not None and self.ldc <= 64 and (not offs or offs[k] % 2 == 0) and
                            int(hip.tuning('class_fused')) != 1 and hip.class_layer_takes(z, A.W[k], o) and
                            fb['dw'][k].numel() >= L_.gist_class_dw_slab_bytes(n, o, 2 * i)):
                        self._cls_fused = True
                        continue
                    if fb['logits'] is not None:
                        self._logit_slabs_n = hip.gemm_slabs('nt', z, A.W[k], A.b[k], self.Y[k][:n, :o],
                                                             fb['logits'])
                        continue
                hip.gemm_nt(z, A.W[k], A.b[k], self.Y[k][:n, :o])
            else:
                y = self.Y[k][:n]
                i_next = self.dims[k + 1][0]
                rstd = self.rstd[k][:n] if self.use_layernorm else None
                if (self.fuse and training and _step and self._fused_buffers()['y'] is not None and
                        not hip.gemm_splits_own_operands(n, o, 2 * i)):
                    ys = self._fused_buffers()['y']
# ... 165 lines not shown
```

### include/gist_hip.h

```cpp
#ifndef GIST_HIP_H_
#define GIST_HIP_H_

#include <stdint.h>

#ifdef __cplusplus
extern "C" {
#endif

typedef void *gist_stream_t;

#define GIST_OK 0
#define GIST_EINVAL (-1)
#define GIST_ELAUNCH (-2)
#define GIST_ENOSPACE (-3)

const char *gist_last_error(void);
int gist_abi_version(void);
int gist_device_count(void);


int gist_in_degree_norm_f32(const int32_t *rowptr, int64_t n_rows, float *norm,
                            gist_stream_t stream);

int gist_spmm_csr_f32(const int32_t *rowptr, const int32_t *col,
// ... 232 lines not shown
int gist_extract_batch(const int32_t *g_rowptr, const int32_t *g_col,
                       const int32_t *g_t_rowptr, const int32_t *g_t_col,
                       const int32_t *ids, int64_t n, int32_t *remap,
                       int32_t *rowptr, int32_t *col, int32_t *t_rowptr, int32_t *t_col,
                       int64_t col_capacity, float *norm,
                       const float *feat, int64_t ld_feat, int64_t n_feat,
                       float *z0, int64_t ldz0,
                       const int32_t *labels_all, int32_t *labels, gist_stream_t stream);

int gist_extract_batch_drop(const int32_t *g_rowptr, const int32_t *g_col,
                            const int32_t *g_t_rowptr, const int32_t *g_t_col,
                            const int32_t *ids, int64_t n, int32_t *remap,
                            int32_t *rowptr, int32_t *col, int32_t *t_rowptr, int32_t *t_col,
                            int64_t col_capacity, float *norm,
                            const float *feat, int64_t ld_feat, int64_t n_feat,
                            float *z0, int64_t ldz0,
                            const int32_t *labels_all, int32_t *labels,
                            float *x0, int64_t ldx0, float p, uint64_t seed, uint64_t offset,
                            int64_t mask_ld, gist_stream_t stream);

int64_t gist_extract_parts_scratch_bytes(int64_t n_max);
int gist_extract_parts_supported(int64_t n_max);
int gist_extract_parts_batch(const int32_t *g_rowptr, const int32_t *g_col,
                             const int32_t *g_t_rowptr, const int32_t *g_t_col,
                             const int32_t *ids, int64_t n, int64_t n_max,
                             const int32_t *node_part, const int32_t *part_slot, int32_t batch,
                             int32_t *rowptr, int32_t *col, int32_t *t_rowptr, int32_t *t_col,
                             int64_t col_capacity, float *norm,
                             const float *feat, int64_t ld_feat, int64_t n_feat,
                             float *z0, int64_t ldz0,
                             const int32_t *labels_all, int32_t *labels,
                             float *x0, int64_t ldx0, float p, uint64_t seed, uint64_t offset,
                             int64_t mask_ld, void *scratch, gist_stream_t stream);

typedef struct gist_extract_parts_desc {
    const int32_t *g_rowptr, *g_col, *g_t_rowptr, *g_t_col;
    const int32_t *ids; int64_t n, n_max;
    const int32_t *node_part, *part_slot; int32_t batch;
    int32_t *rowptr, *col, *t_rowptr, *t_col; int64_t col_capacity; float *norm;
    const float *feat; int64_t ld_feat, n_feat; float *z0; int64_t ldz0;
    const int32_t *labels_all; int32_t *labels;
    float *x0; int64_t ldx0; float p; uint64_t seed, offset; int64_t mask_ld;
    void *scratch;
    const float *feat_intra; int64_t ld_intra;
    float *ah;
} gist_extract_parts_desc;
int gist_extract_parts_desc_batch(const gist_extract_parts_desc *desc, gist_stream_t stream);
int gist_adam_segments_extract_f32(float *param, float *grad, float *exp_avg, float *exp_avg_sq,
                                   int64_t n, float lr, float beta1, float beta2, float eps,
                                   float weight_decay, int64_t step,
                                   const struct gist_grad_segment *segments, int64_t n_segments,
                                   const float *row_loss, int64_t n_loss_rows, int64_t loss_count, float *loss,
                                   const gist_extract_parts_desc *next, gist_stream_t stream);

int gist_gather_rows_f32(const float *src, int64_t lds, const int32_t *ids, int64_t n_ids,
                         int64_t d, float *dst, int64_t ldd, gist_stream_t stream);
int gist_gather_i32(const int32_t *src, const int32_t *ids, int64_t n_ids, int32_t *dst,
                    gist_stream_t stream);


int gist_block_gather_f32(const float *src, int64_t lds, const int32_t *row_idx,
                          const int32_t *col_idx, int64_t n_rows, int64_t n_cols,
                          float *dst, int64_t ldd, gist_stream_t stream);

int gist_block_scatter_f32(const float *src, int64_t lds, const int32_t *row_idx,
                           const int32_t *col_idx, int64_t n_rows, int64_t n_cols,
                           float *dst, int64_t ldd, gist_stream_t stream);

int gist_mean_rows_f32(const float *src, int64_t stride, int64_t n_src, int64_t n,
                       float *out, gist_stream_t stream);



int64_t gist_standard_scaler_workspace_bytes(int64_t n_fit_rows, int64_t d);
int gist_standard_scaler_f32(float *x, int64_t ld, int64_t n_rows, int64_t d,
                             const int32_t *fit_rows, int64_t n_fit_rows, double *mean, double *var,
                             void *workspace, int64_t workspace_bytes, gist_stream_t stream);

#define GIST_MAX_LAYERS 16

typedef struct gist_layer_desc {
    int64_t n_in, n_out;
    float *W, *b;
    float *dW, *db;
    float *Z; int64_t ldz;
    float *Y; int64_t ldy;
    float *rstd;
} gist_layer_desc;

struct gist_timer;
typedef struct gist_step_plan {
    int32_t n_layers;
    int32_t use_layernorm;
    float p_drop;
    uint64_t seed;
    gist_layer_desc layer[GIST_MAX_LAYERS];
    float *dlogits; int64_t ldc;
    float *dZ;
    float *partials;
    float *row_loss, *loss;
    void *workspace; int64_t workspace_bytes;
    void *workspace2; int64_t workspace2_bytes;
    float *params, *grads, *exp_avg, *exp_avg_sq; int64_t n_params;
    const int32_t *g_rowptr, *g_col, *g_t_rowptr, *g_t_col;
    const float *feat; int64_t ld_feat;
    const int32_t *labels_all;
    int32_t *remap;
    int32_t *rowptr, *col, *t_rowptr, *t_col; int64_t col_capacity;
    float *norm; int32_t *labels;
    struct gist_timer *timer;
    int64_t n_max;
    float feat_absmax;
    void *h3_workspace; int64_t h3_workspace_bytes;
    const int32_t *row_blocks; int64_t n_row_blocks;
    void *spmm_prepared; int64_t spmm_prepared_bytes;
    int32_t fuse;
    float *hsrc[GIST_MAX_LAYERS]; int64_t ld_hsrc[GIST_MAX_LAYERS];
    float *col_partials;
    void *fused_workspace; int64_t fused_workspace_bytes;
    const int32_t *node_part, *part_slot;
    int32_t batch_index;
    void *extract_scratch;
    const int32_t *next_ids;
    int64_t next_n;
    int32_t next_batch_index;
    uint64_t next_drop_offset;
    const float *feat_intra; int64_t ld_feat_intra;
    int32_t sibling_parts;
} gist_step_plan;

int64_t gist_step_fused_workspace_bytes(const gist_step_plan *plan);
int64_t gist_step_col_partials_floats(const gist_step_plan *plan);
int64_t gist_step_fused_slab_bytes(const gist_step_plan *plan, int32_t k);

int64_t gist_step_h3_workspace_bytes(const gist_step_plan *plan);
int64_t gist_step_h3_workspace_bytes_mode(const gist_step_plan *plan, int mode);

typedef struct gist_timer gist_timer;
gist_timer *gist_timer_create(int64_t capacity);
void gist_timer_destroy(gist_timer *t);
void gist_timer_reset(gist_timer *t);
int64_t gist_timer_count(const gist_timer *t);
int gist_timer_read(gist_timer *t, int64_t i, float *ms, int32_t *kind, int64_t *m, int64_t *n,
                    int64_t *k);

#define GIST_STEP_EXTRACT 1
#define GIST_STEP_TRAIN 2
#define GIST_STEP_EXTRACT_NEXT 4
#define GIST_STEP_PREEXTRACTED 8
#define GIST_STEP_PHASE_FORWARD 16
#define GIST_STEP_PHASE_BACKWARD 32
#define GIST_STEP_PHASE_OPTIMIZER 64
#define GIST_STEP_DLOGITS_GIVEN 128

int gist_sage_step(const gist_step_plan *plan, const int32_t *ids, int64_t n,
                   uint64_t drop_offset, float lr, float beta1, float beta2, float eps,
                   float weight_decay, int64_t adam_step, int flags, gist_stream_t stream);
int gist_sage_step_extracts_next(const gist_step_plan *plan, int64_t n, int flags);


int gist_gat_scores_f32(const float *Z, int64_t ldz, const float *A, int64_t n_rows, int64_t heads,
                        int64_t out_dim, float *s_src, float *s_dst, gist_stream_t stream);

int gist_gat_aggregate_f32(const int32_t *rowptr, const int32_t *col, const float *Z, int64_t ldz,
                           const float *s_src, const float *s_dst, int64_t n_rows, int64_t heads,
                           int64_t out_dim, int elu, float *out, int64_t ldo, float *M, float *L,
                           gist_stream_t stream);

int gist_gat_backward_dst_f32(const int32_t *rowptr, const int32_t *col, const float *Z, int64_t ldz,
                              const float *out, int64_t ldo, const float *d_out, int64_t ldg,
                              const float *s_src, const float *s_dst, const float *M, const float *L,
                              int64_t n_rows, int64_t heads, int64_t out_dim, int elu, float *G,
                              int64_t ldgm, float *ds_dst, float *D, gist_stream_t stream);

int gist_gat_backward_src_f32(const int32_t *t_rowptr, const int32_t *t_col, const float *Z, int64_t ldz,
                              const float *G, int64_t ldgm, const float *A, const float *s_src,
                              const float *s_dst, const float *M, const float *L, const float *D,
                              const float *ds_dst, int64_t n_rows, int64_t heads, int64_t out_dim,
                              float *dZ, int64_t lddz, float *ds_src, gist_stream_t stream);

int64_t gist_gat_attn_grad_workspace_floats(int64_t n_rows, int64_t heads, int64_t out_dim);
int gist_gat_attn_grad_f32(const float *Z, int64_t ldz, const float *ds_src, const float *ds_dst,
                           int64_t n_rows, int64_t heads, int64_t out_dim, float *partials,
                           int64_t partial_floats, float *dA, gist_stream_t stream);

#ifdef __cplusplus
}
#endif
#endif
```

Before: 5.327.

## Fuse bf16x3 weight-piece emission into the Adam update and skip forward re-split

The Adam kernel gains tiled blocks that update weight matrices and directly write their three-piece bf16 split, both row-major and transposed, into the b3 workspace. A host-side record tracks which layers' pieces are current. When Python reports, via the tensor version counter, that params have not changed since the last step, the next forward pass skips the separate weight-splitting pass. This removes one read of the weights and one kernel pass per layer, at the cost of global cache-invalidation bookkeeping and extra LDS use in the Adam kernel.

```diff
diff --git a/gist_amd/_lib.py b/gist_amd/_lib.py
--- a/gist_amd/_lib.py
+++ b/gist_amd/_lib.py
@@ -150,6 +150,7 @@
 GIST_STEP_PHASE_BACKWARD = 32
 GIST_STEP_PHASE_OPTIMIZER = 64
 GIST_STEP_DLOGITS_GIVEN = 128
+GIST_STEP_PARAMS_UNCHANGED = 256
 
 
 class LayerDesc(ctypes.Structure):
diff --git a/gist_amd/csrc/adam_body.h b/gist_amd/csrc/adam_body.h
--- a/gist_amd/csrc/adam_body.h
+++ b/gist_amd/csrc/adam_body.h
@@ -1,4 +1,5 @@
 #pragma once
+#include "b3_pieces.h"
 #include "common.h"
 
 namespace gist {
@@ -14,11 +15,25 @@
     int64_t begin[kAdamMaxSegs], end[kAdamMaxSegs], stride[kAdamMaxSegs];
     const float *src[kAdamMaxSegs];
 };
+constexpr int kAdamMaxPieces = 4;
+struct AdamPieces {
+    int n;
+    int n_blocks;
+    int first[kAdamMaxPieces];
+    int gx[kAdamMaxPieces];
+    int seg[kAdamMaxPieces];
+    int64_t begin[kAdamMaxPieces];
+    int64_t rows[kAdamMaxPieces], cols[kAdamMaxPieces];
+    int64_t ldd_r[kAdamMaxPieces], ldd_t[kAdamMaxPieces];
+    uint16_t *dst_r[kAdamMaxPieces], *dst_t[kAdamMaxPieces];
+    int64_t skip_lo[kAdamMaxPieces], skip_hi[kAdamMaxPieces];
+};
 struct AdamArgs {
     float *p, *g, *m, *v;
     int64_t n;
     float beta1, beta2, eps, wd, step_size, inv_bc2_sqrt;
     AdamSegs segs;
+    AdamPieces pc;
     const float *row_nll; int n_loss_rows; float inv_count; float *loss;
 };
 __host__ __device__ inline int64_t adam_arena_blocks(int64_t n) { return (n + 1023) / 1024; }
@@ -99,10 +114,19 @@
     unsigned touch = 0;
     for (int s = 0; s < segs.n; ++s)
         if (segs.begin[s] < hi && segs.end[s] > lo && (only_seg < 0 || s == only_seg)) touch |= 1u << s;
+    unsigned ptouch = 0;
+    for (int s = 0; s < A.pc.n; ++s)
+        if (A.pc.begin[s] < hi && A.pc.begin[s] + A.pc.rows[s] * A.pc.cols[s] > lo) ptouch |= 1u << s;
 #pragma unroll
     for (int u = 0; u < 4; ++u) {
         const int64_t i = lo + vt + 256 * u;
         if (i >= hi) break;
+        bool piece = false;
+        for (unsigned t = ptouch; t; t &= t - 1) {
+            const int s = __builtin_ctz(t);
+            piece = piece || (i >= A.pc.begin[s] && i < A.pc.begin[s] + A.pc.rows[s] * A.pc.cols[s]);
+        }
+        if (piece) continue;
         float gv;
         int sg = -1;
         for (unsigned t = touch; t; t &= t - 1) {
@@ -132,6 +156,55 @@
     }
 }
 
+__device__ __forceinline__ void adam_piece_block(const AdamArgs &A, int idx, int t, float (*tile)[65]) {
+    const AdamPieces &pc = A.pc;
+    int s = 0;
+    for (int q = 1; q < pc.n; ++q)
+        if (pc.first[q] <= idx) s = q;
+    const int local = idx - pc.first[s];
+    const int64_t c0 = (int64_t)(local % pc.gx[s]) * 64, r0 = (int64_t)(local / pc.gx[s]) * 64;
+    const int64_t rows = pc.rows[s], cols = pc.cols[s];
+    const int sg = pc.seg[s];
+    const int cc = t & 63;
+    const int64_t c = c0 + cc;
+#pragma unroll 4
+    for (int u = 0; u < 16; ++u) {
+        const int rr = (t >> 6) + 4 * u;
+        const int64_t r = r0 + rr;
+        float out = 0.f;
+        if (r < rows && c < cols) {
+            const int64_t e = r * cols + c;
+            const int64_t i = pc.begin[s] + e;
+            float gv;
+            if (sg >= 0) {
+                const float *src = A.segs.src[sg] + e;
+                const int64_t stride = A.segs.stride[sg];
+                const int ns = A.segs.n_src[sg];
+                float acc = 0.f;
+                int k = 0;
+                for (; k + 4 <= ns; k += 4) {
+                    const float t0 = src[(int64_t)k * stride], t1 = src[(int64_t)(k + 1) * stride];
+                    const float t2 = src[(int64_t)(k + 2) * stride], t3 = src[(int64_t)(k + 3) * stride];
+                    acc += t0; acc += t1; acc += t2; acc += t3;
+                }
+                for (; k < ns; ++k) acc += src[(int64_t)k * stride];
+                gv = acc;
+                A.g[i] = acc;
+            } else {
+                gv = A.g[i];
+            }
+            adam_update(A.p, A.m, A.v, i, gv, A.beta1, A.beta2, A.eps, A.wd, A.step_size, A.inv_bc2_sqrt);
+            out = A.p[i];
+        }
+        tile[rr][cc] = out;
+    }
+    __syncthreads();
+    b3_store_tile(tile, t, r0, c0, rows, cols, pc.dst_r[s], pc.ldd_r[s], pc.dst_t[s], pc.ldd_t[s]);
+}
+
+struct AdamPieceRange { const float *W; int64_t rows, cols; uint16_t *dst_r, *dst_t; };
+int adam_segments_launch(AdamArgs A, const AdamPieceRange *pieces, int n_pieces, hipStream_t st, unsigned *taken = nullptr);
+
 int adam_segments_args(const char *name, float *param, float *grad, float *exp_avg, float *exp_avg_sq, int64_t n, float lr,
                        float beta1, float beta2, float eps, float weight_decay, int64_t step,
                        const gist_grad_segment *segments, int64_t n_segments, const float *row_loss,
diff --git a/gist_amd/csrc/b3_pieces.h b/gist_amd/csrc/b3_pieces.h
--- /dev/null
+++ b/gist_amd/csrc/b3_pieces.h
@@ -0,0 +1,55 @@
+#pragma once
+#include "common.h"
+
+namespace gist {
+
+__device__ __forceinline__ uint32_t b3_pack(__bf16 lo, __bf16 hi) {
+    return (uint32_t)__builtin_bit_cast(unsigned short, lo) |
+           ((uint32_t)__builtin_bit_cast(unsigned short, hi) << 16);
+}
+
+__device__ __forceinline__ void b3_emit(const float (&v)[8], uint16_t *__restrict__ dst) {
+    uint32_t w[3][4];
+#pragma unroll
+    for (int j = 0; j < 4; ++j) {
+        __bf16 p[2][3];
+#pragma unroll
+        for (int h = 0; h < 2; ++h) {
+            const float x = v[2 * j + h];
+            p[h][0] = (__bf16)x;
+            const float r1 = x - (float)p[h][0];
+            p[h][1] = (__bf16)r1;
+            const float r2 = r1 - (float)p[h][1];
+            p[h][2] = (__bf16)r2;
+        }
+#pragma unroll
+        for (int q = 0; q < 3; ++q) w[q][j] = b3_pack(p[0][q], p[1][q]);
+    }
+#pragma unroll
+    for (int q = 0; q < 3; ++q)
+        *reinterpret_cast<uint4 *>(dst + 8 * q) = make_uint4(w[q][0], w[q][1], w[q][2], w[q][3]);
+}
+
+__device__ __forceinline__ void b3_store_tile(const float (*tile)[65], int t, int64_t r0, int64_t c0, int64_t rows,
+                                              int64_t cols, uint16_t *__restrict__ dst_r, int64_t ldd_r,
+                                              uint16_t *__restrict__ dst_t, int64_t ldd_t) {
+    const int kb = t & 7;
+#pragma unroll
+    for (int i = 0; i < 2; ++i) {
+        const int q = (t >> 3) + 32 * i;
+        if (dst_r != nullptr && r0 + q < rows && c0 + kb * 8 < ldd_r) {
+            float v[8];
+#pragma unroll
+            for (int j = 0; j < 8; ++j) v[j] = tile[q][kb * 8 + j];
+            b3_emit(v, dst_r + ((r0 + q) * ldd_r + c0 + kb * 8) * 3);
+        }
+        if (dst_t != nullptr && c0 + q < cols && r0 + kb * 8 < ldd_t) {
+            float v[8];
+#pragma unroll
+            for (int j = 0; j < 8; ++j) v[j] = tile[kb * 8 + j][q];
+            b3_emit(v, dst_t + ((c0 + q) * ldd_t + r0 + kb * 8) * 3);
+        }
+    }
+}
+
+}
diff --git a/gist_amd/csrc/common.h b/gist_amd/csrc/common.h
--- a/gist_amd/csrc/common.h
+++ b/gist_amd/csrc/common.h
@@ -45,6 +45,8 @@
     z = (z ^ (z >> 27)) * 0x94D049BB133111EBULL;
     return z ^ (z >> 31);
 }
+
+void weight_pieces_forget(const float *params);
 
 int64_t h3_kpad(int64_t k);
 bool h3_eligible(int64_t m, int64_t n, int64_t k);
diff --git a/gist_amd/csrc/gemm_b3.hip b/gist_amd/csrc/gemm_b3.hip
--- a/gist_amd/csrc/gemm_b3.hip
+++ b/gist_amd/csrc/gemm_b3.hip
@@ -3,6 +3,7 @@
 
 #include <type_traits>
 
+#include "b3_pieces.h"
 #include "common.h"
 
 namespace gist {
@@ -18,33 +19,6 @@
 constexpr int B3_A_BYTES = B3_TM * B3_KT_BYTES;
 constexpr int B3_B_BYTES = B3_TN * B3_KT_BYTES;
 constexpr int B3_BUF_BYTES = B3_A_BYTES + B3_B_BYTES;
-
-__device__ __forceinline__ uint32_t b3_pack(__bf16 lo, __bf16 hi) {
-    return (uint32_t)__builtin_bit_cast(unsigned short, lo) |
-           ((uint32_t)__builtin_bit_cast(unsigned short, hi) << 16);
-}
-
-__device__ __forceinline__ void b3_emit(const float (&v)[8], uint16_t *__restrict__ dst) {
-    uint32_t w[3][4];
-#pragma unroll
-    for (int j = 0; j < 4; ++j) {
-        __bf16 p[2][3];
-#pragma unroll
-        for (int h = 0; h < 2; ++h) {
-            const float x = v[2 * j + h];
-            p[h][0] = (__bf16)x;
-            const float r1 = x - (float)p[h][0];
-            p[h][1] = (__bf16)r1;
-            const float r2 = r1 - (float)p[h][1];
-            p[h][2] = (__bf16)r2;
-        }
-#pragma unroll
-        for (int q = 0; q < 3; ++q) w[q][j] = b3_pack(p[0][q], p[1][q]);
-    }
-#pragma unroll
-    for (int q = 0; q < 3; ++q)
-        *reinterpret_cast<uint4 *>(dst + 8 * q) = make_uint4(w[q][0], w[q][1], w[q][2], w[q][3]);
-}
 
 __global__ __launch_bounds__(256) void b3_dual_split_kernel(B3Dual d, int64_t ldd_r, int64_t ldd_t,
                                                             float keep) {
@@ -92,23 +66,7 @@
         }
         d.col_partials[(int64_t)blockIdx.y * d.cols + c0 + t] = (s0 + s1) + (s2 + s3);
     }
-    const int kb = t & 7;
-#pragma unroll
-    for (int i = 0; i < 2; ++i) {
-        const int q = (t >> 3) + 32 * i;
-        if (d.dst_r != nullptr && r0 + q < d.rows && c0 + kb * 8 < ldd_r) {
-            float v[8];
-#pragma unroll
-            for (int j = 0; j < 8; ++j) v[j] = tile[q][kb * 8 + j];
-            b3_emit(v, d.dst_r + ((int64_t)(r0 + q) * ldd_r + c0 + kb * 8) * 3);
-        }
-        if (d.dst_t != nullptr && c0 + q < d.cols && r0 + kb * 8 < ldd_t) {
-            float v[8];
-#pragma unroll
-            for (int j = 0; j < 8; ++j) v[j] = tile[kb * 8 + j][q];
-            b3_emit(v, d.dst_t + ((int64_t)(c0 + q) * ldd_t + r0 + kb * 8) * 3);
-        }
-    }
+    b3_store_tile(tile, t, r0, c0, d.rows, d.cols, d.dst_r, ldd_r, d.dst_t, ldd_t);
 }
 
 struct B3Args {
diff --git a/gist_amd/csrc/rowops.hip b/gist_amd/csrc/rowops.hip
--- a/gist_amd/csrc/rowops.hip
+++ b/gist_amd/csrc/rowops.hip
@@ -729,12 +729,26 @@
 
 __global__ __launch_bounds__(256) void adam_segments_kernel(AdamArgs A) {
     __shared__ float red[4];
-    const int64_t n_blocks = adam_arena_blocks(A.n) + A.segs.n_ded;
-    if ((int64_t)blockIdx.x >= n_blocks) {
+    __shared__ float tile[64][65];
+    int64_t b = blockIdx.x;
+    if (b < A.pc.n_blocks) {
+        adam_piece_block(A, (int)b, threadIdx.x, tile);
+        return;
+    }
+    b -= A.pc.n_blocks;
+    int64_t n_arena = adam_arena_blocks(A.n);
+    for (int s = 0; s < A.pc.n; ++s) n_arena -= A.pc.skip_hi[s] - A.pc.skip_lo[s];
+    if (b >= n_arena + A.segs.n_ded) {
         if (A.row_nll != nullptr) loss_reduce_256(A.row_nll, A.n_loss_rows, A.inv_count, A.loss, red);
         return;
     }
-    adam_virtual_block(A, blockIdx.x, threadIdx.x);
+    if (b < n_arena) {
+        for (int s = 0; s < A.pc.n; ++s)
+            if (b >= A.pc.skip_lo[s]) b += A.pc.skip_hi[s] - A.pc.skip_lo[s];
+    } else {
+        b += adam_arena_blocks(A.n) - n_arena;
+    }
+    adam_virtual_block(A, b, threadIdx.x);
 }
 
 __global__ __launch_bounds__(256) void grad_finish_kernel(AdamArgs A) {
@@ -1159,6 +1173,7 @@
     if (n == 0) return GIST_OK;
     GIST_REQUIRE(param && grad && exp_avg && exp_avg_sq, "gist_adam_f32: null pointer");
     GIST_REQUIRE(step >= 1, "gist_adam_f32: step is 1-based");
+    weight_pieces_forget(nullptr);
     const double bc1 = 1.0 - pow((double)beta1, (double)step);
     const double bc2 = 1.0 - pow((double)beta2, (double)step);
     const float step_size = (float)((double)lr / bc1);
@@ -1219,6 +1234,47 @@
     *out = A;
     return GIST_OK;
 }
+
+int adam_segments_launch(AdamArgs A, const AdamPieceRange *pieces, int n_pieces, hipStream_t st, unsigned *taken) {
+    if (taken) *taken = 0;
+    AdamPieces &pc = A.pc;
+    pc = AdamPieces{};
+    int64_t prev_end = 0, blocks = 0;
+    for (int k = 0; k < n_pieces && pc.n < kAdamMaxPieces; ++k) {
+        const AdamPieceRange &q = pieces[k];
+        if (q.W == nullptr || q.dst_r == nullptr || q.rows <= 0 || q.cols <= 0) continue;
+        if (!aligned16(q.dst_r) || (q.dst_t != nullptr && !aligned16(q.dst_t))) continue;
+        const int64_t begin = q.W - A.p, end = begin + q.rows * q.cols;
+        if (q.W < A.p || end > A.n || begin < prev_end) continue;
+        int seg = -1;
+        bool ok = true;
+        for (int s = 0; s < A.segs.n; ++s) {
+            if (A.segs.end[s] <= begin || A.segs.begin[s] >= end) continue;
+            ok = ok && A.segs.begin[s] == begin && A.segs.end[s] == end && A.segs.ded_first[s] < 0;
+            seg = s;
+        }
+        if (!ok) continue;
+        const int64_t ldd_r = b3_kpad(q.cols), ldd_t = b3_kpad(q.rows);
+        const int64_t gx = ceil_div(ldd_r, 64), gy = ceil_div(q.dst_t ? ldd_t : q.rows, 64);
+        if (blocks + gx * gy >= (1LL << 30)) continue;
+        const int j = pc.n++;
+        pc.first[j] = (int)blocks; pc.gx[j] = (int)gx; pc.seg[j] = seg;
+        pc.begin[j] = begin; pc.rows[j] = q.rows; pc.cols[j] = q.cols;
+        pc.ldd_r[j] = ldd_r; pc.ldd_t[j] = ldd_t; pc.dst_r[j] = q.dst_r; pc.dst_t[j] = q.dst_t;
+        pc.skip_lo[j] = ceil_div(begin, 1024);
+        pc.skip_hi[j] = end / 1024 > pc.skip_lo[j] ? end / 1024 : pc.skip_lo[j];
+        blocks += gx * gy;
+        prev_end = end;
+        if (taken) *taken |= 1u << k;
+    }
+    pc.n_blocks = (int)blocks;
+    if (A.n == 0 && A.row_nll == nullptr) return GIST_OK;
+    int64_t n_arena = adam_arena_blocks(A.n);
+    for (int s = 0; s < pc.n; ++s) n_arena -= pc.skip_hi[s] - pc.skip_lo[s];
+    const int64_t grid = blocks + n_arena + A.segs.n_ded + (A.row_nll ? 1 : 0);
+    hipLaunchKernelGGL(adam_segments_kernel, dim3((unsigned)grid), dim3(256), 0, st, A);
+    return launch_status("gist_adam_segments_f32");
+}
 }
 
 extern "C" int gist_adam_segments_f32(float *param, float *grad, float *exp_avg, float *exp_avg_sq,
@@ -1231,10 +1287,8 @@
                                             eps, weight_decay, step, segments, n_segments, row_loss, n_loss_rows,
                                             loss_count, loss, &A);
     if (rc != GIST_OK) return rc;
-    if (n == 0 && row_loss == nullptr) return GIST_OK;
-    const int64_t blocks = gist::adam_arena_blocks(n) + A.segs.n_ded + (row_loss ? 1 : 0);
-    hipLaunchKernelGGL(gist::adam_segments_kernel, dim3((unsigned)blocks), dim3(256), 0, gist::as_stream(stream), A);
-    return gist::launch_status("gist_adam_segments_f32");
+    gist::weight_pieces_forget(nullptr);
+    return gist::adam_segments_launch(A, nullptr, 0, gist::as_stream(stream));
 }
 
 extern "C" int gist_grad_segments_finish_f32(float *grad, int64_t n, const gist_grad_segment *segments,
diff --git a/gist_amd/csrc/step.hip b/gist_amd/csrc/step.hip
--- a/gist_amd/csrc/step.hip
+++ b/gist_amd/csrc/step.hip
@@ -1,7 +1,9 @@
 #include <math.h>
 
+#include <mutex>
 #include <new>
 
+#include "adam_body.h"
 #include "common.h"
 #include "class_dw_body.h"
 
@@ -226,6 +228,70 @@
 }
 
 namespace {
+struct PiecesRecord {
+    const void *ws; const float *params; int64_t n_params; int mode;
+    unsigned layers;
+    const float *W[GIST_MAX_LAYERS]; int64_t n_in[GIST_MAX_LAYERS], n_out[GIST_MAX_LAYERS];
+    const uint16_t *Ws[GIST_MAX_LAYERS], *WsT[GIST_MAX_LAYERS];
+};
+constexpr int kPiecesRecords = 16;
+std::mutex g_pieces_mu;
+PiecesRecord g_pieces[kPiecesRecords];
+int g_pieces_n = 0;
+
+void pieces_forget_ws(const void *ws) {
+    std::lock_guard<std::mutex> lk(g_pieces_mu);
+    int w = 0;
+    for (int i = 0; i < g_pieces_n; ++i)
+        if (g_pieces[i].ws != ws) g_pieces[w++] = g_pieces[i];
+    g_pieces_n = w;
+}
+
+unsigned pieces_current(const gist_step_plan *p, const B3Step &b3, int mode) {
+    std::lock_guard<std::mutex> lk(g_pieces_mu);
+    for (int i = 0; i < g_pieces_n; ++i) {
+        const PiecesRecord &r = g_pieces[i];
+        if (r.ws != p->h3_workspace || r.params != p->params || r.n_params != p->n_params || r.mode != mode) continue;
+        unsigned cur = 0;
+        for (int k = 0; k < p->n_layers; ++k)
+            if (((r.layers >> k) & 1) && b3.layer[k].on && r.W[k] == p->layer[k].W && r.n_in[k] == p->layer[k].n_in &&
+                r.n_out[k] == p->layer[k].n_out && r.Ws[k] == b3.layer[k].Ws && r.WsT[k] == b3.layer[k].WsT)
+                cur |= 1u << k;
+        return cur;
+    }
+    return 0;
+}
+
+void pieces_remember(const gist_step_plan *p, const B3Step &b3, int mode, unsigned layers) {
+    if (layers == 0) return;
+    std::lock_guard<std::mutex> lk(g_pieces_mu);
+    int w = 0;
+    for (int i = 0; i < g_pieces_n; ++i)
+        if (g_pieces[i].ws != p->h3_workspace && g_pieces[i].params != p->params) g_pieces[w++] = g_pieces[i];
+    g_pieces_n = w;
+    if (g_pieces_n == kPiecesRecords) {
+        for (int i = 1; i < kPiecesRecords; ++i) g_pieces[i - 1] = g_pieces[i];
+        --g_pieces_n;
+    }
+    PiecesRecord &r = g_pieces[g_pieces_n++];
+    r = PiecesRecord{};
+    r.ws = p->h3_workspace; r.params = p->params; r.n_params = p->n_params; r.mode = mode; r.layers = layers;
+    for (int k = 0; k < p->n_layers; ++k) {
+        r.W[k] = p->layer[k].W; r.n_in[k] = p->layer[k].n_in; r.n_out[k] = p->layer[k].n_out;
+        r.Ws[k] = b3.layer[k].Ws; r.WsT[k] = b3.layer[k].WsT;
+    }
+}
+}
+
+void gist::weight_pieces_forget(const float *params) {
+    std::lock_guard<std::mutex> lk(g_pieces_mu);
+    int w = 0;
+    for (int i = 0; i < g_pieces_n; ++i)
+        if (params != nullptr && g_pieces[i].params != params) g_pieces[w++] = g_pieces[i];
+    g_pieces_n = w;
+}
+
+namespace {
 constexpr int64_t kLnbMaxUnits = 256;
 struct FusedLayout {
     float *dw_slabs[GIST_MAX_LAYERS]; int64_t dw_bytes[GIST_MAX_LAYERS];
@@ -442,11 +508,14 @@
                                             blocked ? p->row_blocks : nullptr);
     }
 
+    if (!(flags & GIST_STEP_PARAMS_UNCHANGED)) weight_pieces_forget(p->params);
+    if (h3.any && do_fwd) pieces_forget_ws(p->h3_workspace);
+    const unsigned w_cur = b3.any && (flags & GIST_STEP_PARAMS_UNCHANGED) ? pieces_current(p, b3, gemm_mode) : 0u;
     if (b3.any && do_fwd) {
         Scope sc(p->timer, 3, 0, 0, 0, st);
         for (int k = 0; k < L1; ++k) {
             const B3Layer &hl = b3.layer[k];
-            if (!hl.on) continue;
+            if (!hl.on || ((w_cur >> k) & 1)) continue;
             const gist_layer_desc &l = p->layer[k];
             B3Dual d{};
             d.src = l.W; d.ld = 2 * l.n_in; d.rows = l.n_out; d.cols = 2 * l.n_in;
@@ -875,6 +944,7 @@
         return GIST_OK;
     }
     if (!do_opt) return GIST_OK;
+    weight_pieces_forget(p->params);
     if (!do_bwd) n_segs = 0;
     const float *opt_row_loss = do_bwd || !split_phases ? p->row_loss : nullptr;
     if (defer && (flags & GIST_STEP_EXTRACT_NEXT) && next_parts_ok(p, fuse) && p->n_params <= kPrefetchMaxParams) {
@@ -897,6 +967,26 @@
         GIST_TRY(gist_adam_segments_extract_f32(p->params, p->grads, p->exp_avg, p->exp_avg_sq, p->n_params, lr, beta1,
                                                 beta2, eps, weight_decay, adam_step, segs, n_segs, opt_row_loss, n, n,
                                                 p->loss, &x, s));
+    } else if (defer && b3.any && !split_phases) {
+        AdamArgs A;
+        GIST_TRY(adam_segments_args("gist_adam_segments_f32", p->params, p->grads, p->exp_avg, p->exp_avg_sq, p->n_params,
+                                    lr, beta1, beta2, eps, weight_decay, adam_step, segs, n_segs, opt_row_loss, n, n,
+                                    p->loss, &A));
+        AdamPieceRange pr[kAdamMaxPieces];
+        int layer_of[kAdamMaxPieces], n_pr = 0;
+        for (int k = 0; k < L1 && n_pr < kAdamMaxPieces; ++k) {
+            const B3Layer &hl = b3.layer[k];
+            if (!hl.on) continue;
+            const gist_layer_desc &l = p->layer[k];
+            pr[n_pr] = AdamPieceRange{l.W, l.n_out, 2 * l.n_in, hl.Ws, hl.WsT};
+            layer_of[n_pr++] = k;
+        }
+        unsigned taken = 0;
+        GIST_TRY(adam_segments_launch(A, pr, n_pr, st, &taken));
+        unsigned layers = 0;
+        for (int j = 0; j < n_pr; ++j)
+            if ((taken >> j) & 1) layers |= 1u << layer_of[j];
+        pieces_remember(p, b3, gemm_mode, layers);
     } else if (defer)
         GIST_TRY(gist_adam_segments_f32(p->params, p->grads, p->exp_avg, p->exp_avg_sq, p->n_params, lr, beta1,
                                         beta2, eps, weight_decay, adam_step, segs, n_segs, opt_row_loss, n, n,
diff --git a/gist_amd/csrc/subgraph.hip b/gist_amd/csrc/subgraph.hip
--- a/gist_amd/csrc/subgraph.hip
+++ b/gist_amd/csrc/subgraph.hip
@@ -786,6 +786,7 @@
 extern "C" int gist_block_gather_f32(const float *src, int64_t lds_, const int32_t *row_idx,
                                      const int32_t *col_idx, int64_t n_rows, int64_t n_cols,
                                      float *dst, int64_t ldd, gist_stream_t stream) {
+    weight_pieces_forget(nullptr);
     return block_move("gist_block_gather_f32", false, src, lds_, row_idx, col_idx, n_rows, n_cols,
                       dst, ldd, stream);
 }
@@ -793,6 +794,7 @@
 extern "C" int gist_block_scatter_f32(const float *src, int64_t lds_, const int32_t *row_idx,
                                       const int32_t *col_idx, int64_t n_rows, int64_t n_cols,
                                       float *dst, int64_t ldd, gist_stream_t stream) {
+    weight_pieces_forget(nullptr);
     return block_move("gist_block_scatter_f32", true, src, lds_, row_idx, col_idx, n_rows, n_cols,
                       dst, ldd, stream);
 }
@@ -802,6 +804,7 @@
     GIST_REQUIRE(n_src > 0 && n >= 0, "gist_mean_rows_f32: bad size");
     if (n == 0) return GIST_OK;
     GIST_REQUIRE(src && out, "gist_mean_rows_f32: null pointer");
+    weight_pieces_forget(nullptr);
     hipLaunchKernelGGL(mean_rows_kernel, dim3((unsigned)ceil_div(n, 256)), dim3(256), 0,
                        as_stream(stream), src, stride, (int)n_src, n, out);
     return launch_status("gist_mean_rows_f32");
@@ -991,6 +994,7 @@
     const int64_t blocks = 3 * gx + ceil_div((int64_t)A.segs.n_ded, 4) + (row_loss ? 1 : 0) +
                            ceil_div(gist::adam_arena_blocks(n), 4);
     GIST_REQUIRE(blocks < (1LL << 31), "gist_adam_segments_extract_f32: grid too large");
+    gist::weight_pieces_forget(nullptr);
     hipLaunchKernelGGL(adam_extract_kernel, dim3((unsigned)blocks), dim3(64 * kPartsWaves), 0, as_stream(stream), a, (int)gx, A);
     return launch_status("gist_adam_segments_extract_f32");
 }
diff --git a/gist_amd/engine.py b/gist_amd/engine.py
--- a/gist_amd/engine.py
+++ b/gist_amd/engine.py
@@ -176,6 +176,7 @@
         self._logit_slabs_n = 1
         self.plan = None
         self._spmm_prep = None
+        self._params_seen = None
         self._plan_keep = None
 
     def attach_batcher(self, batcher):
@@ -248,6 +249,7 @@
                 self._fused_ws = torch.empty(int(nb), dtype=torch.uint8, device=self.device)
                 P.fused_workspace, P.fused_workspace_bytes = self._fused_ws.data_ptr(), int(nb)
         self.plan = P
+        self._params_seen = None
         self._plan_keep = (batcher, g, self._ws, self._ws2, self._h3_ws, self._fused_ws,
                            self._col_partials)
         return P
@@ -331,8 +333,9 @@
             elif given:
                 flags |= _lib.GIST_STEP_DLOGITS_GIVEN
             rc = L.gist_sage_step(ctypes.byref(P), ids_ptr, b.n, off, lr, betas[0], betas[1], eps, weight_decay,
-                                  max(adam_step if adam_step is not None else self.arena.step, 1), flags | phase,
-                                  hip._stream())
+                                  max(adam_step if adam_step is not None else self.arena.step, 1),
+                                  flags | phase | self._params_flag(), hip._stream())
+            self._params_seen = self.arena.params._version
             _lib.check(rc, 'gist_sage_step')
             if phase == _lib.GIST_STEP_PHASE_OPTIMIZER and batcher is not None:
                 batcher.prefetched = nxt
@@ -385,7 +388,8 @@
             self._phase_ctx = (b, off, flags, ids_ptr)
         rc = L.gist_sage_step(ctypes.byref(P), ids_ptr, b.n, off, lr, betas[0], betas[1],
                               eps, weight_decay, max(adam_step if adam_step is not None else self.arena.step, 1),
-                              flags | phase, hip._stream())
+                              flags | phase | self._params_flag(), hip._stream())
+        self._params_seen = self.arena.params._version
         _lib.check(rc, 'gist_sage_step')
         if batcher is not None:
             batcher.prefetched = nxt
@@ -393,6 +397,11 @@
             b.z0_dropped = True
         b.ready = True
         return self.loss
+
+    def _params_flag(self):
+        from . import _lib
+        seen = self._params_seen
+        return _lib.GIST_STEP_PARAMS_UNCHANGED if seen is not None and seen == self.arena.params._version else 0
 
     def _plan_next(self, b, batcher, flags):
         import ctypes
diff --git a/include/gist_hip.h b/include/gist_hip.h
--- a/include/gist_hip.h
+++ b/include/gist_hip.h
@@ -408,6 +408,7 @@
 #define GIST_STEP_PHASE_BACKWARD 32
 #define GIST_STEP_PHASE_OPTIMIZER 64
 #define GIST_STEP_DLOGITS_GIVEN 128
+#define GIST_STEP_PARAMS_UNCHANGED 256
 
 int gist_sage_step(const gist_step_plan *plan, const int32_t *ids, int64_t n,
                    uint64_t drop_offset, float lr, float beta1, float beta2, float eps,
```

Measured after the change: 5.341 (median of 6 runs). Within noise of the previous version (+0.3%).
